# lmxyy/sige

Measured on AMD Instinct MI355X. Metric: DDPM-256 U-Net sparse (SIGE) forwards/s, higher is better.
Workload: dtype f32; 1 GPU; DDPM 256x256 church U-Net (ch128, mult 1-1-2-2-4-4, 113.7M params, random init), 1.2% square edit, one edited image per GPU, hipGraph replay, NHWC activations, in-place scatter ...; batch_per_gpu=1, resolution=256, parallelism=dp1

## Files before the change

### include/sige_hip.h

```cpp
#ifndef SIGE_HIP_H
#define SIGE_HIP_H

#include <stddef.h>
#include <stdint.h>

#ifdef __cplusplus
extern "C" {
#endif

#define SIGE_HIP_VERSION 310

enum {
    SIGE_HIP_OK = 0,
    SIGE_HIP_EINVAL = -1,
    SIGE_HIP_EUNSUPPORTED = -2,
    SIGE_HIP_ELAUNCH = -3,
    SIGE_HIP_ENODEVICE = -4
};

enum { SIGE_HIP_ACT_IDENTITY = 0, SIGE_HIP_ACT_SWISH = 1,
       SIGE_HIP_ACT_RELU = 2, SIGE_HIP_ACT_LEAKY = 3 , SIGE_HIP_ACT_TANH = 4 };

enum {
    SIGE_HIP_TUNE_CONV_TILE_MT = 0,
// ... 92 lines not shown

int sige_hip_change_tiles_i32(const int32_t *indices, const int32_t *count, int capacity, int bH, int bW,
                              int strideH, int strideW, int offsetH, int offsetW, int outH, int outW,
                              int Hp, int Wp, int tileH, int tileW, int padH, int padW, int depth,
                              int32_t *lists, int32_t *counts, void *stream);

size_t sige_hip_block_conv_packed_size(int Cout, int Cin, int kH, int kW, int R, int S,
                                       int strideH, int strideW, int groups);
int sige_hip_block_conv_pack_f32(const float *w, int Cout, int Cin, int kH, int kW,
                                 float *packed, void *stream);
int sige_hip_block_conv_f32(const float *x, int T, int Cin, int R, int S,
                            const float *packed, const float *bias, int Cout, int kH, int kW,
                            int strideH, int strideW, float *out, void *stream);
int sige_hip_block_conv_direct_f32(const float *x, int T, int Cin, int R, int S,
                                   const float *w, const float *bias, int Cout, int kH, int kW,
                                   int strideH, int strideW, int dilationH, int dilationW, int groups,
                                   float *out, void *stream);
int sige_hip_spade_modulate_nhwc_f32(
        const float *x_full, const float *x_tiles, const int32_t *map_x, int Nx, int Rx, int Sx,
        const float *scale, int scaleB, int scaleC, const float *shift, int shiftB, int shiftC,
        const float *gb_tiles, const float *gb_full, const int32_t *map_g, int Ng, int Rg, int Sg,
        int B, int C, int H, int W, int bH, int bW, const int32_t *active_indices, int N,
        int leaky, float slope, float *out, void *stream);

size_t sige_hip_block_conv_packed_size_f16c(int Cout, int Cin, int kH, int kW, int R, int S,
                                            int strideH, int strideW, int groups);
int sige_hip_block_conv_pack_f16c(const float *w, int Cout, int Cin, int kH, int kW,
                                  float *packed, void *stream);

int sige_hip_conv_pair_begin(void);
int sige_hip_conv_pair_end(void);
int64_t sige_hip_conv_pairs_fused(void);
int sige_hip_conv_side_begin(int max_side_workgroups_per_host);
int sige_hip_conv_side_flush(void);
int64_t sige_hip_conv_side_workgroups(int flushed);
int sige_hip_release_graph_tickets(void);

int sige_hip_gather_conv_f32(const float *x, int B, int Cin, int H, int W, int bH, int bW,
                             const int32_t *active_indices, int N,
                             const float *scale, int scaleB, int scaleC, int scaleH, int scaleW,
                             const float *shift, int shiftB, int shiftC, int shiftH, int shiftW,
                             int activation,
                             const float *packed, const float *bias, int Cout, int kH, int kW,
                             int strideH, int strideW, float *out, void *stream);
int sige_hip_scatter_gather_conv_f32(const float *x, const float *y, int B, int Cin, int H, int W,
                                     int Rx, int Sx, int bH, int bW,
                                     const int32_t *active_indices, int N, const int32_t *scatter_map,
                                     const float *scale, int scaleB, int scaleC, int scaleH, int scaleW,
                                     const float *shift, int shiftB, int shiftC, int shiftH, int shiftW,
                                     int activation,
                                     const float *packed, const float *bias, int Cout, int kH, int kW,
                                     int strideH, int strideW, float *out, void *stream);

int sige_hip_gather_conv_nchw_f32(const float *x, const float *x2, int B, int C1, int C2, int H, int W,
                                  int bH, int bW, const int32_t *active_indices, int N,
                                  const float *scale, int scaleB, int scaleC,
                                  const float *shift, int shiftB, int shiftC,
                                  int activation,
                                  const float *packed, const float *bias, int Cout, int kH, int kW,
                                  int strideH, int strideW, int offsetH, int offsetW,
                                  const float *residual, int Ho, int Wo, float *out, void *stream);

int sige_hip_block_conv_nhwc(int compute, const float *x, int T, int Cin, int R, int S,
                             const float *packed, const float *bias, int Cout, int kH, int kW,
                             int strideH, int strideW, float *out, void *stream);
int sige_hip_block_conv_nhwc_keyed(int compute, const float *x, const int32_t *count_key, int B, int N, int Cin, int R, int S,
                                   const float *packed, const float *bias, int Cout, int kH, int kW,
                                   int strideH, int strideW, float *out, void *stream);
int sige_hip_gather_conv_nhwc(int compute, const float *x, const float *x2, int B, int C1, int C2, int H, int W,
                              int bH, int bW, const int32_t *active_indices, int N,
                              const float *scale, int scaleB, int scaleC,
                              const float *shift, int shiftB, int shiftC,
                              int activation,
                              const float *packed, const float *bias, int Cout, int kH, int kW,
                              int strideH, int strideW,
                              int to_full, int offsetH, int offsetW, const float *residual, int Ho, int Wo,
                              float *workspace, size_t workspace_floats,
                              const float *out_scale, const float *out_shift, int out_activation,
                              int upsample2x,
                              float *twin0, const float *twin0_scale, const float *twin0_shift,
                              float *twin1, const float *twin1_scale, const float *twin1_shift,
                              const float *packed_tile3, int min_blocks,
                              float *out, void *stream);
int sige_hip_conv_ksplit_hint(int T, int Cin, int Cout, int kH, int kW, int strideH, int strideW);
int sige_hip_scatter_gather_conv_nhwc(int compute, const float *x, const void *y, int y_f16, int B, int Cin, int H, int W,
                                      int Rx, int Sx, int bH, int bW,
                                      const int32_t *active_indices, int N, const int32_t *scatter_map,
                                      const float *scale, int scaleB, int scaleC,
                                      const float *shift, int shiftB, int shiftC,
                                      int activation,
                                      const float *packed, const float *bias, int Cout, int kH, int kW,
                                      int strideH, int strideW, float *out, void *stream);

int sige_hip_scatter_gather_conv_scatter_nhwc(
        int compute, const float *x, const void *y, int y_f16, int B, int Cin, int H, int W, int Rx, int Sx, int bH, int bW,
        const int32_t *active_indices, int N, const int32_t *scatter_map,
        const float *scale, int scaleB, int scaleC, const float *shift, int shiftB, int shiftC, int activation,
        const float *packed, const float *bias, int Cout, int kH, int kW,
        int offsetH, int offsetW, const void *residual, int residual_f16,
        const float *x1, const int32_t *table1, int gH1, int gW1, int N1, int R1, int S1,
        float *twin0, const float *twin0_scale, const float *twin0_shift,
        float *twin1, const float *twin1_scale, const float *twin1_shift,
        const float *packed_tile3, int min_blocks,
        float *out, void *stream);

int sige_hip_gather_nhwc_f32(const float *x, int B, int C, int H, int W, int bH, int bW,
                             const int32_t *active_indices, int N,
                             const float *scale, int scaleB, int scaleC,
                             const float *shift, int shiftB, int shiftC,
                             int activation, float *out, void *stream);
int sige_hip_scatter_gather_nhwc_f32(const float *x, const float *y, int B, int C, int H, int W,
                                     int Rx, int Sx, int bH, int bW,
                                     const int32_t *active_indices, int N, const int32_t *scatter_map,
                                     const float *scale, int scaleB, int scaleC,
                                     const float *shift, int shiftB, int shiftC,
                                     int activation, float *out, void *stream);
int sige_hip_scatter_nhwc_f32(const float *x, const float *y, int B, int C, int H, int W, int R, int S,
                              int offsetH, int offsetW, int strideH, int strideW,
                              const int32_t *active_indices, const int32_t *table, int gH, int gW, int N,
                              const float *residual, int in_place, float *out, void *stream);
int sige_hip_scatter_with_block_residual_nhwc_f32(
        const float *x0, const float *y0, const float *x1, const float *y1,
        int B, int C, int H, int W, int R0, int S0, int R1, int S1,
        int offsetH, int offsetW, int strideH, int strideW,
        const int32_t *active_indices0, const int32_t *table0, int gH0, int gW0, int N0,
        const int32_t *active_indices1, const int32_t *table1, int gH1, int gW1, int N1,
        int in_place, float *out, void *stream);

enum { SIGE_HIP_RESAMPLE_DOWN = 0, SIGE_HIP_RESAMPLE_UP = 1 };
int sige_hip_resample_tiles_nhwc_f32(const float *x, int B, int C, int H, int W, int mode,
                                     const int32_t *active_indices, int N, int bH, int bW,
                                     const float *scale, const float *shift, float *tiles,
                                     int offsetH, int offsetW, int strideH, int strideW, int rH, int rW,
                                     float *res, void *stream);

int sige_hip_tile_conv3_supported(int C1, int C2, int Cout);
int sige_hip_tile_conv3_nhwc(
        int compute, int source, const float *x, const void *x2, int y_f16, int B, int C1, int C2, int H, int W, int upsample2x,
        const int32_t *active_indices, int N, const int32_t *scatter_map, int Rx, int Sx,
        const float *scale, const float *shift, int affineB, int activation,
        const float *packed, const float *bias, int Cout,
        int to_full, int offsetH, int offsetW, int Ho, int Wo, const void *residual, int residual_f16,
        const float *x1, const int32_t *table1, int gH1, int gW1, int N1, int R1, int S1,
        const float *out_scale, const float *out_shift, int out_activation,
        float *twin0, const float *twin_scale0, const float *twin_shift0,
        float *twin1, const float *twin_scale1, const float *twin_shift1,
        float *out, void *stream);

int sige_hip_add_layer_norm_tokens_f32(const float *x, const float *delta, const float *bias, const float *gamma,
                                       const float *beta, int64_t T, int C, float eps, float *sum_out, float *out, void *stream);
int sige_hip_geglu_tokens_f32(const float *x, int64_t T, int D, float *out, void *stream);
int sige_hip_add_bias_tokens_f32(const float *x, const float *delta, const float *bias, int64_t T, int C, float *out, void *stream);

size_t sige_hip_token_linear_packed_size(int N, int K, int geglu);
int sige_hip_token_linear_supported(int64_t M, int N, int K, int layer_norm, int geglu, int parts);
int sige_hip_token_linear_pack(const float *w, int N, int K, int geglu, float *packed, void *stream);
int sige_hip_token_linear_f32(const float *x, int64_t M, int K, const float *ln_gamma, const float *ln_beta, float ln_eps,
                              const float *packed, const float *bias, int N, int geglu, const float *residual, int parts,
                              float *out0, float *out1, float *out2, void *stream);

int sige_hip_conv3x3_small_cout_nhwc_f32(const float *x, int B, int C, int H, int W,
                                         const float *scale, int scaleB, int scaleC,
                                         const float *shift, int shiftB, int shiftC, int activation,
                                         const float *weight, const float *bias, int Cout,
                                         float *out, void *stream);

// ... 158 lines not shown
```

### sige_amd/build.py

```python
import os
import subprocess
import sys

PKG = os.path.dirname(os.path.abspath(__file__))
REPO = os.path.dirname(PKG)
CSRC = os.path.join(PKG, "csrc")
LIB_DIR = os.path.join(PKG, "lib")
LIB = os.path.join(LIB_DIR, "libsige_hip.so")
SOURCES = ["api.hip", "plan.hip", "gather.hip", "scatter.hip", "reduce_mask.hip", "mask_pipeline.hip", "block_conv.hip", "conv_k3s1.hip", "conv_k1.hip",
           "conv_k3s2.hip", "conv_k3s1_nhwc.hip", "conv_k1_nhwc.hip", "conv_k3s2_nhwc.hip", "conv_k3s1_nhwc_w8.hip", "conv_k1_nhwc_w8.hip", "conv_k3s1_nhwc_h.hip", "conv_k1_nhwc_h.hip", "conv_k3s1_nhwc_x.hip", "conv_k1_nhwc_x.hip", "conv_k3s1_nhwc_c16.hip", "conv_k3s1_nhwc_h_c16.hip", "conv_k3s1_nhwc_x_c16.hip", "conv_pair_nhwc_x_t4.hip", "conv_pair_nhwc_x_f4.hip",
           "conv_pair_nhwc_t4.hip", "conv_pair_nhwc_t8.hip", "conv_pair_nhwc_f4.hip", "conv_pair_nhwc_f8.hip", "conv_pair_nhwc_h_t4.hip", "conv_pair_nhwc_h_f4.hip", "conv_wide.hip", "conv_wide_k3_p8.hip", "conv_wide_k3_f32.hip", "conv_wide_k1_p8.hip", "conv_wide_pair_f32.hip", "conv_wide_pair_x3.hip", "conv_wide_pair_f16.hip", "group_norm.hip", "attention.hip", "attention_fused.hip", "attention_tokens.hip", "nhwc_ops.hip", "conv_out.hip", "conv_in.hip", "spade_ops.hip", "conv_tile3.hip", "conv_tile3_f32.hip", "token_ops.hip", "conv_tile3_f16.hip", "token_linear.hip", "resample_tiles.hip", "attention_wide.hip", "conv_side_nhwc_f4.hip", "conv_latent_head.hip", "spade_separable.hip"]
FLAGS = ["--offload-arch=gfx950", "-O3", "-std=c++17", "-fPIC", "-ffp-contract=off", "-Wno-unused-result"]


def source_hash() -> str:
    import hashlib

    h = hashlib.sha256(" ".join(FLAGS).encode())
    for f in sorted(os.listdir(CSRC)):
        if f.endswith((".hip", ".hpp", ".h")):
            h.update(f.encode())
            h.update(open(os.path.join(CSRC, f), "rb").read())
    h.update(open(os.path.join(REPO, "include", "sige_hip.h"), "rb").read())
    return h.hexdigest()[:16]


def _hipcc() -> str:
    for cand in (os.environ.get("HIPCC"), "/opt/rocm/bin/hipcc", "hipcc"):
        if cand and (os.path.isabs(cand) and os.path.isfile(cand) or not os.path.isabs(cand)):
            return cand
    return "hipcc"


def needs_build() -> bool:
    if not os.path.isfile(LIB):
        return True
    t = os.path.getmtime(LIB)
    deps = [os.path.join(CSRC, f) for f in os.listdir(CSRC)] + [os.path.join(REPO, "include", "sige_hip.h")]
    return any(os.path.getmtime(d) > t for d in deps)


def _stale(obj: str, src: str, headers) -> bool:
    if not os.path.isfile(obj):
        return True
    t = os.path.getmtime(obj)
    return any(os.path.getmtime(d) > t for d in [src, *headers])


TUNING_UNITS = ("api.hip", "block_conv.hip", "gather.hip", "conv_wide.hip", "attention_tokens.hip", "conv_out.hip", "conv_tile3.hip", "token_linear.hip")
TUNING_LIB = os.path.join(LIB_DIR, "libsige_hip_tuning.so")


def _compile_cmd(src: str, obj: str, defs=()):
    return [_hipcc(), *FLAGS, "-DSIGE_TU_ID=%d" % SOURCES.index(src), *defs, "-I" + os.path.join(REPO, "include"), "-I" + CSRC, "-c",
            os.path.join(CSRC, src), "-o", obj]


def _headers():
    headers = [os.path.join(CSRC, f) for f in os.listdir(CSRC) if f.endswith((".hpp", ".h"))]
    headers.append(os.path.join(REPO, "include", "sige_hip.h"))
    return headers


def _headers_of(src: str, headers):
    return (headers if src.startswith("conv_wide") else [h for h in headers if not h.endswith("conv_wide.hpp")] if src.startswith(("conv_k", "conv_pair", "conv_side", "conv_tile3", "block_conv", "token_linear"))
            else [h for h in headers if not h.endswith(("conv_mfma.hpp", "conv_wide.hpp", "conv_tile3.hpp"))])


def _run_all(procs):
    for cmd, p in procs:
        if p.wait() != 0:
            raise RuntimeError("hipcc failed: " + " ".join(cmd))


def build_tuning(force: bool = False, verbose: bool = True) -> str:
    build(force=force, verbose=verbose)
    if not force and os.path.isfile(TUNING_LIB):
        t = os.path.getmtime(TUNING_LIB)
        deps = [os.path.join(CSRC, f) for f in os.listdir(CSRC)] + [os.path.join(REPO, "include", "sige_hip.h"), LIB]
        if all(os.path.getmtime(d) <= t for d in deps):
            return TUNING_LIB
    tdir = os.path.join(LIB_DIR, "tuning")
    os.makedirs(tdir, exist_ok=True)
    headers = _headers()
    objs, procs = [], []
    for src in SOURCES:
        if src in TUNING_UNITS:
            obj = os.path.join(tdir, src.replace(".hip", ".o"))
            if force or _stale(obj, os.path.join(CSRC, src), _headers_of(src, headers)):
                cmd = _compile_cmd(src, obj, ["-DSIGE_HIP_TUNING"])
                if verbose:
                    print(" ".join(cmd), flush=True)
                procs.append((cmd, subprocess.Popen(cmd)))
        else:
# ... 71 lines not shown
```

### sige_amd/csrc/block_conv.hip

```cpp
#include <deque>
#include <mutex>

#include "conv_mfma.hpp"
#include "conv_tile3.hpp"

namespace sige {

template <int KK, int MT>
__global__ void pack_weights_kernel(const float *__restrict__ w, int Cout, int Cin, float *__restrict__ packed,
                                    long total) {
    constexpr int NL = 64 / MT, CW = (KK == 1 ? 16 : 4) * NL, CC = 4 * CW, L = (CW / NL) * KK, F = L / 4;
    const int nchunks = ((Cin + CC - 1) / CC + 1) & ~1;
    for (long i = (long)blockIdx.x * blockDim.x + threadIdx.x; i < total; i += (long)gridDim.x * blockDim.x) {
        long r = i;
        const int e = r % 4; r /= 4;
        const int j = r % MT; r /= MT;
        const int kq = r % NL; r /= NL;
        const int f = r % F; r /= F;
        const int wave = r % 4; r /= 4;
        const int chunk = r % nchunks; r /= nchunks;
        const int ng = (int)r;
        const int u = 4 * f + e, q = u / KK, tap = u % KK;
        const int ci = chunk * CC + wave * CW + NL * q + kq;
        const int co = MT * ng + j;
// ... 93 lines not shown
        const int g = co / cog;
        float acc = bias ? bias[co] : 0.0f;
        for (int ci = 0; ci < cig; ++ci) {
            const float *xp = x + (((size_t)t * Cin + g * cig + ci) * R + oy * strH) * S + ox * strW;
            const float *wq = w + ((size_t)co * cig + ci) * kH * kW;
            for (int ky = 0; ky < kH; ++ky)
                for (int kx = 0; kx < kW; ++kx) acc = fmaf(xp[ky * dilH * S + kx * dilW], wq[ky * kW + kx], acc);
        }
        out[i] = acc;
    }
}

static int mfma_kind(int kH, int kW, int R, int S, int strH, int strW, int groups) {
    if (groups != 1 || kH != kW || R != S || strH != strW) return 0;
    if (kH == 3 && strH == 1 && R == 6) return 1;
    if (kH == 1 && strH == 1 && R == 4) return 2;
    if (kH == 3 && strH == 2 && R == 5) return 3;
    return 0;
}

#define SIGE_CONV_DECLARE(G, NB, LAY, W)                                                                 \
    template <> void launch_conv_geo<G, NB, SRC_TILES, DST_TILES, LAY, W>(ConvArgs, int, hipStream_t);          \
    template <> void launch_conv_geo<G, NB, SRC_GATHER, DST_TILES, LAY, W>(ConvArgs, int, hipStream_t);         \
    template <> void launch_conv_geo<G, NB, SRC_GATHER, DST_NCHW, LAY, W>(ConvArgs, int, hipStream_t);          \
    template <> void launch_conv_geo<G, NB, SRC_SCATTER_GATHER, DST_TILES, LAY, W>(ConvArgs, int, hipStream_t);
#define SIGE_CONV_DECLARE_LAYOUTS(G, NB) SIGE_CONV_DECLARE(G, NB, LAYOUT_NCHW, 4) SIGE_CONV_DECLARE(G, NB, LAYOUT_NHWC, 4)
using K31_16 = ConvGeo<3, 1, 6, 16>;
using K31_32 = ConvGeo<3, 1, 6, 32>;
using K11_16 = ConvGeo<1, 1, 4, 16>;
using K11_32 = ConvGeo<1, 1, 4, 32>;
using K32_16 = ConvGeo<3, 2, 5, 16>;
using K32_32 = ConvGeo<3, 2, 5, 32>;
SIGE_CONV_DECLARE_LAYOUTS(K31_16, 1)
SIGE_CONV_DECLARE_LAYOUTS(K31_16, 2)
SIGE_CONV_DECLARE_LAYOUTS(K31_32, 1)
SIGE_CONV_DECLARE_LAYOUTS(K31_32, 2)
SIGE_CONV_DECLARE_LAYOUTS(K11_16, 1)
SIGE_CONV_DECLARE_LAYOUTS(K11_16, 2)
SIGE_CONV_DECLARE_LAYOUTS(K11_32, 1)
SIGE_CONV_DECLARE_LAYOUTS(K11_32, 2)
SIGE_CONV_DECLARE_LAYOUTS(K32_16, 1)
SIGE_CONV_DECLARE_LAYOUTS(K32_32, 1)
#define SIGE_CONV_DECLARE_SG_FULL(G, NB, W) \
    template <> void launch_conv_geo<G, NB, SRC_SCATTER_GATHER, DST_NCHW, LAYOUT_NHWC, W>(ConvArgs, int, hipStream_t);
SIGE_CONV_DECLARE_SG_FULL(K31_16, 1, 4) SIGE_CONV_DECLARE_SG_FULL(K31_16, 2, 4)
SIGE_CONV_DECLARE_SG_FULL(K31_32, 1, 4) SIGE_CONV_DECLARE_SG_FULL(K31_32, 2, 4)
SIGE_CONV_DECLARE_SG_FULL(K31_16, 1, 8) SIGE_CONV_DECLARE_SG_FULL(K31_16, 2, 8)
SIGE_CONV_DECLARE_SG_FULL(K31_32, 1, 8) SIGE_CONV_DECLARE_SG_FULL(K31_32, 2, 8)
SIGE_CONV_DECLARE(K31_16, 1, LAYOUT_NHWC, 8)
SIGE_CONV_DECLARE(K31_16, 2, LAYOUT_NHWC, 8)
SIGE_CONV_DECLARE(K31_32, 1, LAYOUT_NHWC, 8)
SIGE_CONV_DECLARE(K31_32, 2, LAYOUT_NHWC, 8)
SIGE_CONV_DECLARE(K11_16, 1, LAYOUT_NHWC, 8)
SIGE_CONV_DECLARE(K11_16, 2, LAYOUT_NHWC, 8)
SIGE_CONV_DECLARE(K11_32, 1, LAYOUT_NHWC, 8)
SIGE_CONV_DECLARE(K11_32, 2, LAYOUT_NHWC, 8)

using H31_16 = ConvGeoH<3, 1, 6, 16>;
using H31_32 = ConvGeoH<3, 1, 6, 32>;
using H11_16 = ConvGeoH<1, 1, 4, 16>;
using H11_32 = ConvGeoH<1, 1, 4, 32>;
SIGE_CONV_DECLARE(H31_16, 1, LAYOUT_NHWC, 4) SIGE_CONV_DECLARE(H31_16, 2, LAYOUT_NHWC, 4)
SIGE_CONV_DECLARE(H31_32, 1, LAYOUT_NHWC, 4) SIGE_CONV_DECLARE(H31_32, 2, LAYOUT_NHWC, 4)
SIGE_CONV_DECLARE(H11_16, 1, LAYOUT_NHWC, 4) SIGE_CONV_DECLARE(H11_16, 2, LAYOUT_NHWC, 4)
SIGE_CONV_DECLARE(H11_32, 1, LAYOUT_NHWC, 4) SIGE_CONV_DECLARE(H11_32, 2, LAYOUT_NHWC, 4)
SIGE_CONV_DECLARE_SG_FULL(H31_16, 1, 4) SIGE_CONV_DECLARE_SG_FULL(H31_16, 2, 4)
SIGE_CONV_DECLARE_SG_FULL(H31_32, 1, 4) SIGE_CONV_DECLARE_SG_FULL(H31_32, 2, 4)

using X31_16 = ConvGeoX<3, 1, 6, 16>;
using X31_32 = ConvGeoX<3, 1, 6, 32>;
using X11_16 = ConvGeoX<1, 1, 4, 16>;
using X11_32 = ConvGeoX<1, 1, 4, 32>;
SIGE_CONV_DECLARE(X31_16, 1, LAYOUT_NHWC, 4) SIGE_CONV_DECLARE(X31_32, 1, LAYOUT_NHWC, 4)
SIGE_CONV_DECLARE(X11_16, 1, LAYOUT_NHWC, 4) SIGE_CONV_DECLARE(X11_32, 1, LAYOUT_NHWC, 4)
SIGE_CONV_DECLARE_SG_FULL(X31_16, 1, 4) SIGE_CONV_DECLARE_SG_FULL(X31_32, 1, 4)

#define SIGE_CONV_DECLARE_C16(G, NB)                                                        \
    template <> void launch_conv_c16<G, NB, DST_TILES>(ConvArgs, int, hipStream_t);         \
    template <> void launch_conv_c16<G, NB, DST_NCHW>(ConvArgs, int, hipStream_t);
SIGE_CONV_DECLARE_C16(K31_16, 1) SIGE_CONV_DECLARE_C16(K31_16, 2) SIGE_CONV_DECLARE_C16(K31_32, 1) SIGE_CONV_DECLARE_C16(K31_32, 2)
SIGE_CONV_DECLARE_C16(H31_16, 1) SIGE_CONV_DECLARE_C16(H31_16, 2) SIGE_CONV_DECLARE_C16(H31_32, 1) SIGE_CONV_DECLARE_C16(H31_32, 2)
SIGE_CONV_DECLARE_C16(X31_16, 1) SIGE_CONV_DECLARE_C16(X31_32, 1)

__global__ __launch_bounds__(256) void splitk_reduce_nhwc_kernel(const float *__restrict__ ws, int S, size_t stride, size_t n4, int C,
                                                                const float *__restrict__ bias, const float *__restrict__ residual,
                                                                const float *__restrict__ oscale, const float *__restrict__ oshift, int oact,
                                                                float *__restrict__ out) {
    for (size_t i = (size_t)blockIdx.x * 256 + threadIdx.x; i < n4; i += (size_t)gridDim.x * 256) {
        const float4 zero = make_float4(0.f, 0.f, 0.f, 0.f);
        const int c = (int)((4 * i) % C);
        float4 b = zero, r = zero, os = zero, oh = zero;
        if (bias) b = *reinterpret_cast<const float4 *>(bias + c);
        if (residual) r = *reinterpret_cast<const float4 *>(residual + 4 * i);
        if (oscale) {
            os = *reinterpret_cast<const float4 *>(oscale + c);
            oh = *reinterpret_cast<const float4 *>(oshift + c);
        }
        float4 p[8];
#pragma unroll
        for (int s = 0; s < 8; ++s) p[s] = *reinterpret_cast<const float4 *>(ws + (size_t)(s < S ? s : S - 1) * stride + 4 * i);
        float4 v = p[0];
#pragma unroll
        for (int s = 1; s < 8; ++s)
            if (s < S) { v.x += p[s].x; v.y += p[s].y; v.z += p[s].z; v.w += p[s].w; }
        if (bias) { v.x += b.x; v.y += b.y; v.z += b.z; v.w += b.w; }
        if (residual) { v.x += r.x; v.y += r.y; v.z += r.z; v.w += r.w; }
        if (oscale) {
            v.x = os.x * v.x; v.y = os.y * v.y; v.z = os.z * v.z; v.w = os.w * v.w;
            v.x = oh.x + v.x; v.y = oh.y + v.y; v.z = oh.z + v.z; v.w = oh.w + v.w;
            if (oact == SIGE_HIP_ACT_SWISH) { v.x = swish(v.x); v.y = swish(v.y); v.z = swish(v.z); v.w = swish(v.w); }
        }
        *reinterpret_cast<float4 *>(out + 4 * i) = v;
    }
}

static int ksplit_for(long blocks, int nchunks, int cap) {
    const int force = tuning(SIGE_HIP_TUNE_CONV_KSPLIT);
    if (cap <= 1 || (blocks >= 224 && !force)) return 1;
    int s = force ? force : (int)((224 + blocks - 1) / blocks);
    s = s < nchunks / 2 ? s : nchunks / 2;
    s = s < 8 ? s : 8;
    s = s < cap ? s : cap;
    return s < 1 ? 1 : s;
}

__device__ int32_t g_zero_idx[2] = {0, 0};

#ifdef SIGE_CONV_PROBE
static unsigned long long *g_probe_buf = nullptr;
static unsigned long long *conv_probe_buffer() {
    if (!g_probe_buf && hipMalloc(&g_probe_buf, 8 * 4096 * sizeof(unsigned long long)) != hipSuccess) g_probe_buf = nullptr;
    return g_probe_buf;
}
extern "C" int sige_hip_conv_probe_read(unsigned long long *host, int workgroups) {
    if (!g_probe_buf || workgroups > 4096) return SIGE_HIP_EINVAL;
    return hipMemcpy(host, g_probe_buf, (size_t)workgroups * 8 * sizeof(unsigned long long), hipMemcpyDeviceToHost) == hipSuccess
               ? SIGE_HIP_OK : SIGE_HIP_ELAUNCH;
}
extern "C" int sige_hip_conv_probe_clear(void) {
    if (!conv_probe_buffer()) return SIGE_HIP_ELAUNCH;
    return hipMemset(g_probe_buf, 0, 8 * 4096 * sizeof(unsigned long long)) == hipSuccess ? SIGE_HIP_OK : SIGE_HIP_ELAUNCH;
}
#endif

struct HeldConv {
    bool active = false;
    ConvArgs a;
    int mode = 0, dst = 0, prec = 0;
    hipStream_t st = nullptr;
    int (*launch)(ConvArgs, int, hipStream_t) = nullptr;
};
static thread_local HeldConv g_held;
static thread_local bool g_pairing = false;
static std::atomic<long> g_pairs_fused{0};

static int flush_held() {
    if (!g_held.active) return SIGE_HIP_OK;
    const HeldConv h = g_held;
    g_held.active = false;
    const bool p = g_pairing;
    g_pairing = false;
    const int rc = h.launch(h.a, h.mode, h.st);
    note_launches(1);
    g_pairing = p;
    return rc;
}
// ... 305 lines not shown
            if (rc1 != SIGE_HIP_OK) {
                const int rc = flush_held();
                return rc != SIGE_HIP_OK ? rc : SIGE_HIP_EUNSUPPORTED;
            }
        }
    }
    if (a.ksplit > 1) {
        a.out = a.ws;
        a.fout = final_out;
    }
    const int mt = p.mt, nb = p.nb, waves = p.waves;
    bool done = false;
    if constexpr (kPairFirst) {
        if (may_pair) {
            done = launch_pair<DST, PREC>(a, p, mode, g_held.a, st);
            if (done) g_held.active = false;
            else {
                const int rc = flush_held();
                if (rc != SIGE_HIP_OK) return rc;
            }
        }
    }
    if constexpr (kSideGeo) {
        if (!done && !g_side.empty() && mt == 16 && nb == 1 && waves == 4 && a.ksplit == 1 && (mode == MODE_RAW || mode == MODE_AFFINE_SWISH)) {
            SideConv &sc = g_side.front();
            const int na = conv_grid_x(a);
            int take = sc.total - sc.next;
            take = take < sc.budget ? take : sc.budget;
            take = take < kSideChipWorkgroups - na ? take : kSideChipWorkgroups - na;
            if (take > 0) {
                if (sc.nb == 2) launch_conv_side<K31_16, 1, K31_16, 2, DST_NCHW, 4>(a, sc.a, mode, na, sc.next, take, st);
                else launch_conv_side<K31_16, 1, K31_16, 1, DST_NCHW, 4>(a, sc.a, mode, na, sc.next, take, st);
                sc.next += take;
                g_side_hosted.fetch_add(take, std::memory_order_relaxed);
                if (sc.next >= sc.total) g_side.pop_front();
                done = true;
            }
        }
    }
    if constexpr (SRC == SRC_SCATTER_GATHER && LAY == LAYOUT_NHWC && KH == 3 && STR == 1) {
        if (!done && a.y_f16) {
            if (waves != 4) return SIGE_HIP_EUNSUPPORTED;
            if constexpr (kHasNB2) {
                if (mt == 32 && nb == 2) { launch_conv_c16<G32, 2, DST>(a, mode, st); done = true; }
                else if (nb == 2) { launch_conv_c16<G16, 2, DST>(a, mode, st); done = true; }
            }
            if (!done) {
                if (mt == 32) launch_conv_c16<G32, 1, DST>(a, mode, st);
                else launch_conv_c16<G16, 1, DST>(a, mode, st);
                done = true;
            }
        }
    } else {
        if (a.y_f16) return SIGE_HIP_EUNSUPPORTED;
    }
    constexpr bool kHasW8 = LAY == LAYOUT_NHWC && STR == 1 && PREC == 0;
    if constexpr (kHasW8) {
        if (!done && waves == 8) {
            if (mt == 32 && nb == 2) launch_conv_geo<G32, 2, SRC, DST, LAY, 8>(a, mode, st);
            else if (mt == 32) launch_conv_geo<G32, 1, SRC, DST, LAY, 8>(a, mode, st);
            else if (nb == 2) launch_conv_geo<G16, 2, SRC, DST, LAY, 8>(a, mode, st);
            else launch_conv_geo<G16, 1, SRC, DST, LAY, 8>(a, mode, st);
            done = true;
        }
    }
    if constexpr (kHasNB2) {
        if (!done && mt == 32 && nb == 2) { launch_conv_geo<G32, 2, SRC, DST, LAY, 4>(a, mode, st); done = true; }
        else if (!done && nb == 2) { launch_conv_geo<G16, 2, SRC, DST, LAY, 4>(a, mode, st); done = true; }
    }
    if (!done) {
        if (mt == 32) launch_conv_geo<G32, 1, SRC, DST, LAY, 4>(a, mode, st);
        else launch_conv_geo<G16, 1, SRC, DST, LAY, 4>(a, mode, st);
    }
    if (a.ksplit > 1 && !a.counters) {
        const size_t n4 = a.split_stride / 4;
        const int grid = (int)((n4 + 255) / 256 < 2048 ? (n4 + 255) / 256 : 2048);
        splitk_reduce_nhwc_kernel<<<grid, 256, 0, st>>>(a.ws, a.ksplit, a.split_stride, n4, a.Cout, a.bias, a.residual,
                                                       a.oscale, a.oshift, a.oact, final_out);
        note_launches(1);
    }
    return SIGE_HIP_OK;
}

template <int SRC, int DST = DST_TILES, int LAY = LAYOUT_NCHW, int PREC = 0>
static int launch_conv(const ConvArgs &a, int mode, int kH, int kW, int R, int S, int strH, int strW, hipStream_t st) {
    int rc;
    switch (mfma_kind(kH, kW, R, S, strH, strW, 1)) {
        case 1: rc = launch_kind<3, 1, 6, SRC, DST, LAY, PREC>(a, mode, st); break;
        case 2: rc = launch_kind<1, 1, 4, SRC, DST, LAY, PREC>(a, mode, st); break;
        case 3:
            if constexpr (PREC != 0) return SIGE_HIP_EUNSUPPORTED;
            else rc = launch_kind<3, 2, 5, SRC, DST, LAY, PREC>(a, mode, st);
            break;
        default: return SIGE_HIP_EUNSUPPORTED;
    }
    return rc != SIGE_HIP_OK ? rc : launch_status();
}

static int staging_mode(const float *scale, int sB, int sC, const float *shift, int tB, int tC, int activation,
                        int B, int C, int *aff_sb, int *aff_sc) {
    *aff_sb = *aff_sc = 0;
    if (!scale && !shift) return activation == SIGE_HIP_ACT_IDENTITY ? MODE_RAW : -1;
    if (!scale || !shift || sB != tB || sC != tC) return -1;
    if (!((sB == 1 || sB == B) && (sC == 1 || sC == C))) return -1;
    *aff_sb = sB > 1 ? sC : 0;
    *aff_sc = sC > 1 ? 1 : 0;
    return activation == SIGE_HIP_ACT_SWISH ? MODE_AFFINE_SWISH : MODE_AFFINE;
}

}

using namespace sige;

extern "C" int sige_hip_conv_pair_begin(void) {
    SIGE_PLAN_HOOK0(sige_hip_conv_pair_begin);
    const int rc = flush_held();
    g_pairing = true;
    return rc;
}

extern "C" int sige_hip_conv_pair_end(void) {
    SIGE_PLAN_HOOK0(sige_hip_conv_pair_end);
    g_pairing = false;
    g_side_armed = 0;
    const int rc = flush_held();
    if (rc != SIGE_HIP_OK) (void)flush_side();
    return rc != SIGE_HIP_OK ? rc : launch_status(0);
}

extern "C" int64_t sige_hip_conv_pairs_fused(void) { return (int64_t)g_pairs_fused.load(std::memory_order_relaxed); }

extern "C" int sige_hip_conv_side_begin(int max_side_workgroups_per_host) {
    SIGE_PLAN_HOOK_NOSTREAM(sige_hip_conv_side_begin, max_side_workgroups_per_host);
    if (max_side_workgroups_per_host <= 0) return SIGE_HIP_EINVAL;
    g_side_armed = max_side_workgroups_per_host;
    return SIGE_HIP_OK;
}

extern "C" int sige_hip_conv_side_flush(void) {
    SIGE_PLAN_HOOK0(sige_hip_conv_side_flush);
    g_side_armed = 0;
    return flush_side();
}

extern "C" int64_t sige_hip_conv_side_workgroups(int flushed) {
    return (int64_t)(flushed ? g_side_flushed : g_side_hosted).load(std::memory_order_relaxed);
}

extern "C" size_t sige_hip_block_conv_packed_size(int Cout, int Cin, int kH, int kW, int R, int S,
                                                  int strideH, int strideW, int groups) {
    if (Cout <= 0 || Cin <= 0) return 0;
    if (!mfma_kind(kH, kW, R, S, strideH, strideW, groups)) return 0;
    return packed_floats(Cout, Cin, kH * kW, 32) + packed_floats(Cout, Cin, kH * kW, 16);
}

extern "C" int sige_hip_block_conv_pack_f32(const float *w, int Cout, int Cin, int kH, int kW,
                                            float *packed, void *stream) {
    if (!w || !packed || Cout <= 0 || Cin <= 0) return SIGE_HIP_EINVAL;
    if (kH != kW || (kH != 1 && kH != 3)) return SIGE_HIP_EUNSUPPORTED;
    const int KK = kH * kW;
    hipStream_t st = as_stream(stream);
    const long n32 = (long)packed_floats(Cout, Cin, KK, 32), n16 = (long)packed_floats(Cout, Cin, KK, 16);
    auto blocks = [](long n) { return (int)((n + 255) / 256 < 4096 ? (n + 255) / 256 : 4096); };
    if (KK == 9) {
        pack_weights_kernel<9, 32><<<blocks(n32), 256, 0, st>>>(w, Cout, Cin, packed, n32);
        pack_weights_kernel<9, 16><<<blocks(n16), 256, 0, st>>>(w, Cout, Cin, packed + n32, n16);
    } else {
        pack_weights_kernel<1, 32><<<blocks(n32), 256, 0, st>>>(w, Cout, Cin, packed, n32);
        pack_weights_kernel<1, 16><<<blocks(n16), 256, 0, st>>>(w, Cout, Cin, packed + n32, n16);
    }
    return launch_status(2);
}

extern "C" size_t sige_hip_block_conv_packed_size_f16c(int Cout, int Cin, int kH, int kW, int R, int S,
                                                       int strideH, int strideW, int groups) {
    if (Cout <= 0 || Cin <= 0) return 0;
    const int kind = mfma_kind(kH, kW, R, S, strideH, strideW, groups);
    if (kind != 1 && kind != 2) return 0;
    return packed_units_h(Cout, Cin, kH * kW, 32) + packed_units_h(Cout, Cin, kH * kW, 16);
}

extern "C" int sige_hip_block_conv_pack_f16c(const float *w, int Cout, int Cin, int kH, int kW,
                                             float *packed, void *stream) {
    if (!w || !packed || Cout <= 0 || Cin <= 0) return SIGE_HIP_EINVAL;
    if (kH != kW || (kH != 1 && kH != 3)) return SIGE_HIP_EUNSUPPORTED;
    const int KK = kH * kW;
    hipStream_t st = as_stream(stream);
    const long n32 = 2 * (long)packed_units_h(Cout, Cin, KK, 32), n16 = 2 * (long)packed_units_h(Cout, Cin, KK, 16);
    auto blocks = [](long n) { return (int)((n + 255) / 256 < 4096 ? (n + 255) / 256 : 4096); };
    _Float16 *ph = reinterpret_cast<_Float16 *>(packed);
    if (KK == 9) {
        pack_weights_h_kernel<9, 32><<<blocks(n32), 256, 0, st>>>(w, Cout, Cin, ph, n32);
        pack_weights_h_kernel<9, 16><<<blocks(n16), 256, 0, st>>>(w, Cout, Cin, ph + n32, n16);
    } else {
        pack_weights_h_kernel<1, 32><<<blocks(n32), 256, 0, st>>>(w, Cout, Cin, ph, n32);
        pack_weights_h_kernel<1, 16><<<blocks(n16), 256, 0, st>>>(w, Cout, Cin, ph + n32, n16);
    }
    return launch_status(2);
}

extern "C" size_t sige_hip_block_conv_packed_size_f16x3(int Cout, int Cin, int kH, int kW, int R, int S,
                                                        int strideH, int strideW, int groups) {
    if (Cout <= 0 || Cin <= 0) return 0;
    const int kind = mfma_kind(kH, kW, R, S, strideH, strideW, groups);
    if (kind != 1 && kind != 2) return 0;
    return packed_units_x(Cout, Cin, kH * kW, 32) + packed_units_x(Cout, Cin, kH * kW, 16) + kX3Header;
}

extern "C" int sige_hip_block_conv_pack_f16x3(const float *w, int Cout, int Cin, int kH, int kW,
                                              float *packed, void *stream) {
    if (!w || !packed || Cout <= 0 || Cin <= 0) return SIGE_HIP_EINVAL;
    if (kH != kW || (kH != 1 && kH != 3)) return SIGE_HIP_EUNSUPPORTED;
    const int KK = kH * kW;
    hipStream_t st = as_stream(stream);
    const size_t u32 = packed_units_x(Cout, Cin, KK, 32), u16 = packed_units_x(Cout, Cin, KK, 16);
    const long n32 = 2 * (long)u32, n16 = 2 * (long)u16;
    float *header = packed + u32 + u16;
    if (hipMemsetAsync(header, 0, kX3Header * sizeof(float), st) != hipSuccess) return SIGE_HIP_ELAUNCH;
    const long nw = (long)Cout * Cin * KK;
    wmax_bits_kernel<<<(int)((nw + 255) / 256 < 1024 ? (nw + 255) / 256 : 1024), 256, 0, st>>>(w, nw, reinterpret_cast<unsigned *>(header));
    auto blocks = [](long n) { return (int)((n + 255) / 256 < 4096 ? (n + 255) / 256 : 4096); };
    _Float16 *ph = reinterpret_cast<_Float16 *>(packed);
    if (KK == 9) {
        pack_weights_x_kernel<9, 32><<<blocks(n32), 256, 0, st>>>(w, Cout, Cin, ph, n32, header);
        pack_weights_x_kernel<9, 16><<<blocks(n16), 256, 0, st>>>(w, Cout, Cin, ph + n32, n16, header);
    } else {
        pack_weights_x_kernel<1, 32><<<blocks(n32), 256, 0, st>>>(w, Cout, Cin, ph, n32, header);
        pack_weights_x_kernel<1, 16><<<blocks(n16), 256, 0, st>>>(w, Cout, Cin, ph + n32, n16, header);
    }
    return launch_status(3);
}

extern "C" int sige_hip_block_conv_f32(const float *x, int T, int Cin, int R, int S,
                                       const float *packed, const float *bias, int Cout, int kH, int kW,
                                       int strideH, int strideW, float *out, void *stream) {
    SIGE_PLAN_HOOK_FIXED(sige_hip_block_conv_f32, x, T, Cin, R, S, packed, bias, Cout, kH, kW, strideH, strideW, out, stream);
    if (T < 0 || Cin <= 0 || Cout <= 0) return SIGE_HIP_EINVAL;
    if (T == 0) return SIGE_HIP_OK;
    if (!x || !packed || !out) return SIGE_HIP_EINVAL;
    if (reinterpret_cast<uintptr_t>(out) & 15 || reinterpret_cast<uintptr_t>(packed) & 15) return SIGE_HIP_EINVAL;
    if ((long)T * Cin * R * S >= (1L << 29)) return SIGE_HIP_EUNSUPPORTED;
    ConvArgs a{};
    a.x = x; a.packed = packed; a.bias = bias; a.out = out;
    a.T = T; a.Cin = Cin; a.Cout = Cout;
    if (reinterpret_cast<uintptr_t>(x) & 15 || ((long)Cin * R * S) % 4) {
        void *zero_idx = nullptr;
        if (hipGetSymbolAddress(&zero_idx, HIP_SYMBOL(g_zero_idx)) != hipSuccess) return SIGE_HIP_ELAUNCH;
        a.x2 = x; a.Csplit = Cin; a.idx = static_cast<const int32_t *>(zero_idx);
        a.B = T; a.N = 1; a.H = R; a.W = S;
        return launch_conv<SRC_GATHER>(a, MODE_RAW, kH, kW, R, S, strideH, strideW, as_stream(stream));
    }
    return launch_conv<SRC_TILES>(a, 0, kH, kW, R, S, strideH, strideW, as_stream(stream));
}

// ... 77 lines not shown
        !channel_affine(shift, shiftB, shiftC, shiftH, shiftW, B, Cin))
        return SIGE_HIP_EUNSUPPORTED;
    if ((long)B * Cin * H * W >= (1L << 29) || (long)B * N * Cin * Rx * Sx >= (1L << 29)) return SIGE_HIP_EUNSUPPORTED;
    if ((long)B * N == 0) return SIGE_HIP_OK;
    if (!x || !y || !packed || !out || !active_indices || !scatter_map) return SIGE_HIP_EINVAL;
    if (reinterpret_cast<uintptr_t>(out) & 15 || reinterpret_cast<uintptr_t>(packed) & 15) return SIGE_HIP_EINVAL;
    ConvArgs a{};
    a.x = x; a.y = y; a.idx = active_indices; a.map = scatter_map; a.packed = packed; a.bias = bias; a.out = out;
    a.T = B * N; a.Cin = Cin; a.Cout = Cout; a.B = B; a.N = N; a.H = H; a.W = W;
    if (stacked_shift(H) != 0) return SIGE_HIP_EUNSUPPORTED;
    a.RxSx = Rx * Sx; a.Sx = Sx;
    a.scale = scale; a.shift = shift;
    const int mode = staging_mode(scale, scaleB, scaleC, shift, shiftB, shiftC, activation, B, Cin, &a.aff_sb, &a.aff_sc);
    if (mode < 0) return SIGE_HIP_EUNSUPPORTED;
    return launch_conv<SRC_SCATTER_GATHER>(a, mode, kH, kW, bH, bW, strideH, strideW, as_stream(stream));
}

static bool nhwc_ok(int Cin, int C1, int Cout, const void *p0, const void *p1, const void *p2, const void *p3) {
    auto al = [](const void *p) { return (reinterpret_cast<uintptr_t>(p) & 15) == 0; };
    return Cin % 4 == 0 && C1 % 4 == 0 && Cout % 4 == 0 && al(p0) && al(p1) && al(p2) && al(p3);
}

extern "C" int sige_hip_conv_ksplit_hint(int T, int Cin, int Cout, int kH, int kW, int strideH, int strideW) {
    if (T <= 0 || Cin <= 0 || Cout <= 0) return 1;
    const int px = (kH == 3 && strideH == 2) ? 4 : 16;
    const long blocks16 = (long)ceil_div(T, 16 / px) * ceil_div(Cout, 16);
    if (blocks16 >= 224 && !tuning(SIGE_HIP_TUNE_CONV_KSPLIT)) return 1;
    return 8;
}

#define SIGE_BY_COMPUTE(compute, impl, ...)         \
    ((compute) == 0   ? impl<0>(__VA_ARGS__)        \
     : (compute) == 1 ? impl<1>(__VA_ARGS__)        \
     : (compute) == 2 ? impl<2>(__VA_ARGS__)        \
                      : SIGE_HIP_EINVAL)

template <int PREC>
static int block_conv_nhwc_impl(const float *x, int T, int Cin, int R, int S,
                                const float *packed, const float *bias, int Cout, int kH, int kW,
                                int strideH, int strideW, float *out, void *stream) {
    if (T < 0 || Cin <= 0 || Cout <= 0) return SIGE_HIP_EINVAL;
    if (T == 0) return SIGE_HIP_OK;
    if (!x || !packed || !out) return SIGE_HIP_EINVAL;
    if (!nhwc_ok(Cin, Cin, Cout, x, packed, out, bias)) return SIGE_HIP_EUNSUPPORTED;
    if ((long)T * Cin * R * S >= (1L << 29)) return SIGE_HIP_EUNSUPPORTED;
    ConvArgs a{};
    a.x = x; a.packed = packed; a.bias = bias; a.out = out;
    a.T = T; a.Cin = Cin; a.Cout = Cout;
    return launch_conv<SRC_TILES, DST_TILES, LAYOUT_NHWC, PREC>(a, 0, kH, kW, R, S, strideH, strideW, as_stream(stream));
}

extern "C" int sige_hip_block_conv_nhwc(int compute, const float *x, int T, int Cin, int R, int S,
                                        const float *packed, const float *bias, int Cout, int kH, int kW,
                                        int strideH, int strideW, float *out, void *stream) {
    SIGE_PLAN_HOOK_FIXED(sige_hip_block_conv_nhwc, compute, x, T, Cin, R, S, packed, bias, Cout, kH, kW, strideH, strideW, out, stream);
    return SIGE_BY_COMPUTE(compute, block_conv_nhwc_impl, x, T, Cin, R, S, packed, bias, Cout, kH, kW, strideH, strideW, out, stream);
}

extern "C" int sige_hip_block_conv_nhwc_keyed(int compute, const float *x, const int32_t *count_key, int B, int N, int Cin, int R, int S,
                                              const float *packed, const float *bias, int Cout, int kH, int kW,
                                              int strideH, int strideW, float *out, void *stream) {
    SIGE_PLAN_HOOK_N(sige_hip_block_conv_nhwc_keyed, (sige::CountOf<2, 4>), compute, x, count_key, B, N, Cin, R, S, packed, bias, Cout, kH, kW, strideH, strideW, out, stream);
    if (B < 0 || N < 0 || !count_key || (long)B * N > 0x7fffffffL) return SIGE_HIP_EINVAL;
    const int T = B * N;
    return SIGE_BY_COMPUTE(compute, block_conv_nhwc_impl, x, T, Cin, R, S, packed, bias, Cout, kH, kW, strideH, strideW, out, stream);
}

template <int PREC>
static int gather_conv_nhwc_impl(const float *x, const float *x2, int B, int C1, int C2, int H, int W,
                                             int bH, int bW, const int32_t *active_indices, int N,
                                             const float *scale, int scaleB, int scaleC,
                                             const float *shift, int shiftB, int shiftC,
                                             int activation,
                                             const float *packed, const float *bias, int Cout, int kH, int kW,
                                             int strideH, int strideW,
                                             int to_full, int offsetH, int offsetW, const float *residual, int Ho, int Wo,
                                             float *workspace, size_t workspace_floats,
                                             const float *out_scale, const float *out_shift, int out_activation,
                                             int upsample2x,
                                             float *twin0, const float *twin0_scale, const float *twin0_shift,
                                             float *twin1, const float *twin1_scale, const float *twin1_shift,
                                             float *out, void *stream) {
    const int Cin = C1 + C2;
    if (upsample2x && ((H | W) & 1)) return SIGE_HIP_EINVAL;
    if (B < 0 || C1 <= 0 || C2 < 0 || Cout <= 0 || H <= 0 || W <= 0 || N < 0) return SIGE_HIP_EINVAL;
    if (to_full && (Ho <= 0 || Wo <= 0)) return SIGE_HIP_EINVAL;
    if (activation != SIGE_HIP_ACT_IDENTITY && activation != SIGE_HIP_ACT_SWISH) return SIGE_HIP_EUNSUPPORTED;
    if ((long)B * Cin * H * W >= (1L << 29)) return SIGE_HIP_EUNSUPPORTED;
    if ((long)B * N == 0) return SIGE_HIP_OK;
    if (!x || (C2 && !x2) || !packed || !out || !active_indices) return SIGE_HIP_EINVAL;
    if (C2 && B != 1) return SIGE_HIP_EUNSUPPORTED;
    if (!nhwc_ok(Cin, C1, Cout, x, C2 ? x2 : x, out, bias) || (reinterpret_cast<uintptr_t>(packed) & 15) ||
        (reinterpret_cast<uintptr_t>(residual) & 15))
        return SIGE_HIP_EUNSUPPORTED;
    ConvArgs a{};
    a.x = x; a.x2 = C2 ? x2 : x; a.Csplit = C1; a.idx = active_indices; a.packed = packed; a.bias = bias; a.out = out;
    a.T = B * N; a.Cin = Cin; a.Cout = Cout; a.B = B; a.N = N; a.H = H; a.W = W;
    a.hp_shift = stacked_shift(H);
    if (a.hp_shift < 0 || (a.hp_shift && B != 1)) return SIGE_HIP_EUNSUPPORTED;
    a.scale = scale; a.shift = shift;
    const int mode = staging_mode(scale, scaleB, scaleC, shift, shiftB, shiftC, activation, B, Cin, &a.aff_sb, &a.aff_sc);
    if (mode < 0) return SIGE_HIP_EUNSUPPORTED;
    if ((out_scale == nullptr) != (out_shift == nullptr)) return SIGE_HIP_EINVAL;
    if (out_activation != SIGE_HIP_ACT_IDENTITY && out_activation != SIGE_HIP_ACT_SWISH) return SIGE_HIP_EUNSUPPORTED;
    if ((reinterpret_cast<uintptr_t>(out_scale) | reinterpret_cast<uintptr_t>(out_shift)) & 15) return SIGE_HIP_EUNSUPPORTED;
    a.oscale = out_scale; a.oshift = out_shift; a.oact = out_activation;
    a.up = upsample2x ? 1 : 0;
    {
        const int Ro = (bH - kH) / strideH + 1, So = (bW - kW) / strideW + 1;
        a.split_stride = to_full ? (size_t)B * Ho * Wo * Cout : (size_t)B * N * Ro * So * Cout;
        a.ws = workspace;
        a.ksplit_max = (workspace && a.split_stride && !(reinterpret_cast<uintptr_t>(workspace) & 15))
                           ? (int)(workspace_floats / a.split_stride < 8 ? workspace_floats / a.split_stride : 8) : 1;
        if (to_full && (long)N * Ro * So < (long)Ho * Wo) a.ksplit_max = 1;
    }
    if ((twin0 || twin1) && !to_full) return SIGE_HIP_EINVAL;
    if ((twin0 && (!twin0_scale || !twin0_shift)) || (twin1 && (!twin1_scale || !twin1_shift))) return SIGE_HIP_EINVAL;
    if ((reinterpret_cast<uintptr_t>(twin0) | reinterpret_cast<uintptr_t>(twin1) | reinterpret_cast<uintptr_t>(twin0_scale) |
         reinterpret_cast<uintptr_t>(twin0_shift) | reinterpret_cast<uintptr_t>(twin1_scale) | reinterpret_cast<uintptr_t>(twin1_shift)) & 15)
        return SIGE_HIP_EUNSUPPORTED;
    a.twin0 = twin0; a.tscale0 = twin0_scale; a.tshift0 = twin0_shift;
    a.twin1 = twin1; a.tscale1 = twin1_scale; a.tshift1 = twin1_shift;
    if (to_full) {
        a.residual = residual; a.Ho = Ho; a.Wo = Wo; a.offH = offsetH; a.offW = offsetW; a.strH = strideH; a.strW = strideW;
        return launch_conv<SRC_GATHER, DST_NCHW, LAYOUT_NHWC, PREC>(a, mode, kH, kW, bH, bW, strideH, strideW, as_stream(stream));
    }
    return launch_conv<SRC_GATHER, DST_TILES, LAYOUT_NHWC, PREC>(a, mode, kH, kW, bH, bW, strideH, strideW, as_stream(stream));
}

constexpr int kTile3F16PairMin = 256;

constexpr int kTile3F16SparseMin = 128;

static bool tile3_takes(const float *packed_tile3, int min_blocks, int B, int N, int C1, int C2, int Cout, int kH, int kW, int bH, int bW,
                        int strideH, int strideW, hipStream_t st, bool f16 = false, int H = 0, int W = 0) {
    if (!packed_tile3 || min_blocks <= 0) return false;
    if (kH != 3 || kW != 3 || bH != 6 || bW != 6 || strideH != 1 || strideW != 1) return false;
    if (!sige_hip_tile_conv3_supported(C1, C2, Cout)) return false;
    const long blocks = (long)((B * (long)N + 1) / 2) * (Cout / 64);
    int need = min_blocks;
    if (f16 && H > 0 && (long)N * 16 < (long)H * W) {
        int sm = tuning(SIGE_HIP_TUNE_TILE3_F16_SPARSE_MIN);
        if (sm < 0) sm = kTile3F16SparseMin;
        if (sm > 0 && sm < need) need = sm;
    }
    if (blocks < need) return false;
    if (g_held.active && g_held.st == st) {
        if (!f16) return false;
        int pm = tuning(SIGE_HIP_TUNE_TILE3_F16_PAIR_MIN);
        if (pm < 0) pm = kTile3F16PairMin;
        if (pm == 0 || blocks < pm) return false;
    }
    return true;
}

extern "C" int sige_hip_gather_conv_nhwc(int compute, const float *x, const float *x2, int B, int C1, int C2, int H, int W,
                                         int bH, int bW, const int32_t *active_indices, int N,
                                         const float *scale, int scaleB, int scaleC,
                                         const float *shift, int shiftB, int shiftC,
                                         int activation,
                                         const float *packed, const float *bias, int Cout, int kH, int kW,
                                         int strideH, int strideW,
                                         int to_full, int offsetH, int offsetW, const float *residual, int Ho, int Wo,
                                         float *workspace, size_t workspace_floats,
                                         const float *out_scale, const float *out_shift, int out_activation,
                                         int upsample2x,
                                         float *twin0, const float *twin0_scale, const float *twin0_shift,
                                         float *twin1, const float *twin1_scale, const float *twin1_shift,
                                         const float *packed_tile3, int min_blocks,
                                         float *out, void *stream) {
    SIGE_PLAN_HOOK_N(sige_hip_gather_conv_nhwc, (sige::CountOf<10, 11>), compute, x, x2, B, C1, C2, H, W, bH, bW, active_indices, N, scale, scaleB, scaleC, shift, shiftB, shiftC, activation, packed, bias, Cout, kH, kW, strideH, strideW, to_full, offsetH, offsetW, residual, Ho, Wo, workspace, workspace_floats, out_scale, out_shift, out_activation, upsample2x, twin0, twin0_scale, twin0_shift, twin1, twin1_scale, twin1_shift, packed_tile3, min_blocks, out, stream);
    const int Cin = C1 + C2;
    const bool f16 = compute == 1;
    const bool aff_ok = (!scale && !shift) || (scale && shift && scaleC == Cin && shiftC == Cin && scaleB == shiftB && (scaleB == 1 || scaleB == B));
    if ((compute == 0 || f16) && B > 0 && N > 0 && aff_ok && !(g_side_armed > 0 && compute == 0 && to_full) &&
        tile3_takes(packed_tile3, min_blocks, B, N, C1, C2, Cout, kH, kW, bH, bW, strideH, strideW, as_stream(stream), f16, f16 ? H : 0, f16 ? W : 0)) {
        const int rc = tile_conv3_launch(T3_GATHER, x, x2, B, C1, C2, H, W, upsample2x, active_indices, N, nullptr, 0, 0, scale, shift,
                                         scale ? scaleB : 0, activation, packed_tile3, bias, Cout, to_full, offsetH, offsetW, Ho, Wo,
                                         to_full ? residual : nullptr, nullptr, nullptr, 0, 0, 0, 0, 0, out_scale, out_shift, out_activation,
                                         twin0, twin0_scale, twin0_shift, twin1, twin1_scale, twin1_shift, out, stream, f16 ? WIDE_F16 : WIDE_F32, 0, 0);
        if (rc != SIGE_HIP_EUNSUPPORTED) { g_side_armed = 0; return rc; }
    }
    const int rc = SIGE_BY_COMPUTE(compute, gather_conv_nhwc_impl, x, x2, B, C1, C2, H, W, bH, bW, active_indices, N, scale, scaleB, scaleC, shift, shiftB,
                                   shiftC, activation, packed, bias, Cout, kH, kW, strideH, strideW, to_full, offsetH, offsetW, residual, Ho, Wo,
                                   workspace, workspace_floats, out_scale, out_shift, out_activation, upsample2x, twin0, twin0_scale, twin0_shift,
                                   twin1, twin1_scale, twin1_shift, out, stream);
    g_side_armed = 0;
    return rc;
}

template <int PREC>
static int scatter_gather_conv_nhwc_impl(const float *x, const void *y, int y_f16, int B, int Cin, int H, int W,
                                                     int Rx, int Sx, int bH, int bW,
                                                     const int32_t *active_indices, int N, const int32_t *scatter_map,
                                                     const float *scale, int scaleB, int scaleC,
                                                     const float *shift, int shiftB, int shiftC,
                                                     int activation,
                                                     const float *packed, const float *bias, int Cout, int kH, int kW,
                                                     int strideH, int strideW, float *out, void *stream) {
    if (B < 0 || Cin <= 0 || Cout <= 0 || H <= 0 || W <= 0 || N < 0 || Rx <= 0 || Sx <= 0) return SIGE_HIP_EINVAL;
    if (activation != SIGE_HIP_ACT_IDENTITY && activation != SIGE_HIP_ACT_SWISH) return SIGE_HIP_EUNSUPPORTED;
    if ((long)B * Cin * H * W >= (1L << 29) || (long)B * N * Cin * Rx * Sx >= (1L << 29)) return SIGE_HIP_EUNSUPPORTED;
    if ((long)B * N == 0) return SIGE_HIP_OK;
    if (!x || !y || !packed || !out || !active_indices || !scatter_map) return SIGE_HIP_EINVAL;
    if (!nhwc_ok(Cin, Cin, Cout, x, y, out, bias) || (reinterpret_cast<uintptr_t>(packed) & 15)) return SIGE_HIP_EUNSUPPORTED;
    if (y_f16 && (kH != 3 || kW != 3 || strideH != 1 || strideW != 1)) return SIGE_HIP_EUNSUPPORTED;
    ConvArgs a{};
    a.y_f16 = y_f16 ? 1 : 0;
    a.x = x; a.y = static_cast<const float *>(y); a.idx = active_indices; a.map = scatter_map; a.packed = packed; a.bias = bias; a.out = out;
    a.T = B * N; a.Cin = Cin; a.Cout = Cout; a.B = B; a.N = N; a.H = H; a.W = W;
    a.hp_shift = stacked_shift(H);
    if (a.hp_shift < 0 || (a.hp_shift && B != 1)) return SIGE_HIP_EUNSUPPORTED;
    a.RxSx = Rx * Sx; a.Sx = Sx;
    a.scale = scale; a.shift = shift;
    const int mode = staging_mode(scale, scaleB, scaleC, shift, shiftB, shiftC, activation, B, Cin, &a.aff_sb, &a.aff_sc);
    if (mode < 0) return SIGE_HIP_EUNSUPPORTED;
    return launch_conv<SRC_SCATTER_GATHER, DST_TILES, LAYOUT_NHWC, PREC>(a, mode, kH, kW, bH, bW, strideH, strideW, as_stream(stream));
}

extern "C" int sige_hip_scatter_gather_conv_nhwc(int compute, const float *x, const void *y, int y_f16, int B, int Cin, int H, int W,
                                                 int Rx, int Sx, int bH, int bW,
                                                 const int32_t *active_indices, int N, const int32_t *scatter_map,
                                                 const float *scale, int scaleB, int scaleC,
                                                 const float *shift, int shiftB, int shiftC,
                                                 int activation,
                                                 const float *packed, const float *bias, int Cout, int kH, int kW,
                                                 int strideH, int strideW, float *out, void *stream) {
    SIGE_PLAN_HOOK_N(sige_hip_scatter_gather_conv_nhwc, (sige::CountOf<12, 13>), compute, x, y, y_f16, B, Cin, H, W, Rx, Sx, bH, bW, active_indices, N, scatter_map, scale, scaleB, scaleC, shift, shiftB, shiftC, activation, packed, bias, Cout, kH, kW, strideH, strideW, out, stream);
    return SIGE_BY_COMPUTE(compute, scatter_gather_conv_nhwc_impl, x, y, y_f16, B, Cin, H, W, Rx, Sx, bH, bW, active_indices, N, scatter_map, scale, scaleB,
                           scaleC, shift, shiftB, shiftC, activation, packed, bias, Cout, kH, kW, strideH, strideW, out, stream);
}

template <int PREC>
static int scatter_gather_conv_scatter_nhwc_impl(
        const float *x, const void *y, int y_f16, int B, int Cin, int H, int W, int Rx, int Sx, int bH, int bW,
        const int32_t *active_indices, int N, const int32_t *scatter_map,
        const float *scale, int scaleB, int scaleC, const float *shift, int shiftB, int shiftC, int activation,
        const float *packed, const float *bias, int Cout, int kH, int kW,
        int offsetH, int offsetW, const void *residual, int residual_f16,
        const float *x1, const int32_t *table1, int gH1, int gW1, int N1, int R1, int S1,
        float *twin0, const float *twin0_scale, const float *twin0_shift,
        float *twin1, const float *twin1_scale, const float *twin1_shift,
        float *out, void *stream) {
    if (B < 0 || Cin <= 0 || Cout <= 0 || H <= 0 || W <= 0 || N < 0 || Rx <= 0 || Sx <= 0) return SIGE_HIP_EINVAL;
    if (kH != 3 || kW != 3 || bH != 6 || bW != 6) return SIGE_HIP_EUNSUPPORTED;
    if (activation != SIGE_HIP_ACT_IDENTITY && activation != SIGE_HIP_ACT_SWISH) return SIGE_HIP_EUNSUPPORTED;
    if ((long)B * Cin * H * W >= (1L << 29) || (long)B * N * Cin * Rx * Sx >= (1L << 29)) return SIGE_HIP_EUNSUPPORTED;
    if ((long)B * N == 0) return SIGE_HIP_OK;
    if (!x || !y || !packed || !out || !active_indices || !scatter_map) return SIGE_HIP_EINVAL;
    if (x1 && (!residual || !table1 || R1 <= 0 || S1 <= 0 || gH1 < (H + R1 - 1) / R1 || gW1 < (W + S1 - 1) / S1)) return SIGE_HIP_EINVAL;
    if (!nhwc_ok(Cin, Cin, Cout, x, y, out, bias) || (reinterpret_cast<uintptr_t>(packed) & 15) ||
        (reinterpret_cast<uintptr_t>(residual) & 15) || (reinterpret_cast<uintptr_t>(x1) & 15))
        return SIGE_HIP_EUNSUPPORTED;
    if (residual_f16 && !residual) return SIGE_HIP_EINVAL;
    ConvArgs a{};
    a.y_f16 = y_f16 ? 1 : 0; a.res_f16 = residual_f16 ? 1 : 0;
    a.x = x; a.y = static_cast<const float *>(y); a.idx = active_indices; a.map = scatter_map; a.packed = packed; a.bias = bias; a.out = out;
    a.T = B * N; a.Cin = Cin; a.Cout = Cout; a.B = B; a.N = N; a.H = H; a.W = W;
// ... 71 lines not shown
```

### sige_amd/csrc/conv_mfma.hpp

```cpp
#pragma once
#include <type_traits>

#include "common.hpp"

namespace sige {

typedef float f32x16 __attribute__((ext_vector_type(16)));
typedef float f32x4 __attribute__((ext_vector_type(4)));
typedef _Float16 f16x8 __attribute__((ext_vector_type(8)));
typedef _Float16 f16x4 __attribute__((ext_vector_type(4)));

enum { SRC_TILES = 0, SRC_GATHER = 1, SRC_SCATTER_GATHER = 2 };
enum { DST_TILES = 0, DST_NCHW = 1 };

template <int MT_> struct Mfma;
template <> struct Mfma<32> {
    using acc_t = f32x16;
    static constexpr int REGS = 16;
    __device__ static __forceinline__ acc_t op(float a, float b, acc_t c) {
        return __builtin_amdgcn_mfma_f32_32x32x2f32(a, b, c, 0, 0, 0);
    }
};
template <> struct Mfma<16> {
    using acc_t = f32x4;
// ... 35 lines not shown
    static constexpr int F = L / 4;
    static constexpr int TILE_FLOATS = CC * RS;
    static constexpr int BUF = TPB * TILE_FLOATS;
    static constexpr int RED = MT_ + 4;
    static_assert(L % 4 == 0, "wave slice must be a whole number of float4 weight loads");
    static_assert(MT_ % PX == 0 && TPB >= 1, "tile pixels must divide the M block");
};

template <int KH, int STR, int R_, int MT_>
struct ConvGeoH {
    static constexpr bool F16 = true, X3 = false;
    static constexpr int K = KH, S = STR, R = R_, MT = MT_;
    static constexpr int KK = KH * KH;
    static constexpr int RS = R_ * R_;
    static constexpr int RO = (R_ - KH) / STR + 1;
    static constexpr int PX = RO * RO;
    static constexpr int NL = 64 / MT_;
    static constexpr int KP = 8;
    static constexpr int SLAB = NL * KP;
    static constexpr int NSLAB = KK == 1 ? 2 : 1;
    static constexpr int TPB = MT_ / PX;
    static constexpr int CW = NSLAB * SLAB;
    static constexpr int CC = 4 * CW;
    static constexpr int L = NSLAB * KK;
    static constexpr int F = L;
    static constexpr int TILE_FLOATS = CC * RS;
    static constexpr int BUF = TPB * TILE_FLOATS;
    static constexpr int RED = MT_ + 4;
    static_assert(MT_ % PX == 0 && TPB >= 1, "tile pixels must divide the M block");
};

template <int KH, int STR, int R_, int MT_>
struct ConvGeoX : ConvGeoH<KH, STR, R_, MT_> {
    static constexpr bool X3 = true;
    static constexpr int F = 2 * ConvGeoH<KH, STR, R_, MT_>::L;
};

__host__ __device__ constexpr int cmax(int a, int b) { return a > b ? a : b; }

template <int I, int N, typename F>
__device__ __forceinline__ void static_for(F &&f) {
    if constexpr (I < N) {
        f(std::integral_constant<int, I>{});
        static_for<I + 1, N>(f);
    }
}

struct ConvArgs {
    const float *x;
    const float *y;
    const int32_t *idx;
    const int32_t *map;
    const float *packed;
    const float *bias;
    float *out;
    int T, Cin, Cout, nchunks;
    int nblk;
    int B, N, H, W;
    int RxSx, Sx;
    const float *scale, *shift;
    int aff_sb, aff_sc;
    const float *x2;
    int Csplit;
    const float *residual;
    int Ho, Wo, offH, offW, strH, strW;
    int mbk, ngk, ng_fast;
    int ksplit, chunks_per_split;
    size_t split_stride;
    const float *oscale, *oshift;
    int oact;
    const float *x1;
    const int32_t *table1;
    int gW1, N1, R1, S1;
    int up;
    float *ws;
    int ksplit_max;
    int32_t *counters;
    float *fout;
    float *twin0, *twin1;
    const float *tscale0, *tshift0, *tscale1, *tshift1;
    const float *wscale_ptr;
    int y_f16, res_f16;
    int hp_shift;
#ifdef SIGE_CONV_PROBE
    unsigned long long *probe;
#endif
};

#ifdef SIGE_CONV_PROBE
#define SIGE_PROBE(k)                                                                                       \
    do {                                                                                                    \
        if (a.probe && threadIdx.x == 0 && blockIdx.y == 0 && blockIdx.x < 4096)                            \
            a.probe[blockIdx.x * 8 + (k)] = __builtin_amdgcn_s_memtime();                                   \
    } while (0)
#else
#define SIGE_PROBE(k)
#endif
#if defined(SIGE_CONV_PROBE) && defined(SIGE_ABL)
#define SIGE_ABL_HAS(bit) (((SIGE_ABL) & (bit)) != 0)
#else
#define SIGE_ABL_HAS(bit) false
#endif

__device__ __forceinline__ float swish_fast(float z) {
    const float e = __builtin_amdgcn_exp2f(z * -1.44269504088896341f);
    return z * __builtin_amdgcn_rcpf(1.0f + e);
}

enum { MODE_RAW = 0, MODE_AFFINE_SWISH = 1, MODE_AFFINE = 2 };

using rsrc_t = __amdgpu_buffer_rsrc_t;
constexpr unsigned kOOB = 0x80000000u;

__device__ __forceinline__ rsrc_t make_rsrc(const float *base, long elem_off, long total_elems) {
    const int off = __builtin_amdgcn_readfirstlane((int)elem_off);
    int bytes = __builtin_amdgcn_readfirstlane((int)((total_elems - elem_off) * 4));
    bytes = bytes < 0 ? 0 : bytes;
    return __builtin_amdgcn_make_buffer_rsrc(const_cast<float *>(base) + off, 0, bytes, 0x00020000);
}
__device__ __forceinline__ float buf_f32(rsrc_t r, unsigned byte_off) {
    return __builtin_bit_cast(float, __builtin_amdgcn_raw_buffer_load_b32(r, (int)byte_off, 0, 0));
}
__device__ __forceinline__ float4 buf_f32x4(rsrc_t r, unsigned byte_off, int soff) {
    const f32x4 v = __builtin_bit_cast(f32x4, __builtin_amdgcn_raw_buffer_load_b128(r, (int)byte_off, soff, 0));
    return make_float4(v[0], v[1], v[2], v[3]);
}

__device__ __forceinline__ rsrc_t make_rsrc_h(const float *base_as_halves, long elem_off, long total_elems) {
    const int off = __builtin_amdgcn_readfirstlane((int)elem_off);
    int bytes = __builtin_amdgcn_readfirstlane((int)((total_elems - elem_off) * 2));
    bytes = bytes < 0 ? 0 : bytes;
    return __builtin_amdgcn_make_buffer_rsrc(reinterpret_cast<_Float16 *>(const_cast<float *>(base_as_halves)) + off, 0, bytes, 0x00020000);
}
typedef unsigned u32x2 __attribute__((ext_vector_type(2)));
__device__ __forceinline__ float4 buf_h4(rsrc_t r, unsigned byte_off, int soff) {
    const f16x4 h = __builtin_bit_cast(f16x4, __builtin_amdgcn_raw_buffer_load_b64(r, (int)byte_off, soff, 0));
    return make_float4((float)h[0], (float)h[1], (float)h[2], (float)h[3]);
}
__device__ __forceinline__ float4 ld_f32x4_or_h4(const float *base, size_t elem, bool halves) {
    if (halves) {
        const f16x4 h = *reinterpret_cast<const f16x4 *>(reinterpret_cast<const _Float16 *>(base) + elem);
        return make_float4((float)h[0], (float)h[1], (float)h[2], (float)h[3]);
    }
    return *reinterpret_cast<const float4 *>(base + elem);
}

__device__ __forceinline__ float4 ld_raw_f32x4_or_h4(const float *base, size_t elem, bool halves) {
    if (halves) {
        const float2 h = *reinterpret_cast<const float2 *>(reinterpret_cast<const _Float16 *>(base) + elem);
        return make_float4(h.x, h.y, 0.f, 0.f);
    }
    return *reinterpret_cast<const float4 *>(base + elem);
}
__device__ __forceinline__ float4 cvt_raw_f32x4_or_h4(float4 raw, bool halves) {
    if (halves) {
        const float2 r2 = make_float2(raw.x, raw.y);
        const f16x4 h = __builtin_bit_cast(f16x4, r2);
        return make_float4((float)h[0], (float)h[1], (float)h[2], (float)h[3]);
    }
    return raw;
}

enum { LAYOUT_NCHW = 0, LAYOUT_NHWC = 1 };

__device__ __forceinline__ void coherent_store(float *p, float4 v) {
    unsigned long long *q = reinterpret_cast<unsigned long long *>(p);
    const unsigned long long lo = (unsigned long long)__builtin_bit_cast(unsigned, v.x) | ((unsigned long long)__builtin_bit_cast(unsigned, v.y) << 32);
    const unsigned long long hi = (unsigned long long)__builtin_bit_cast(unsigned, v.z) | ((unsigned long long)__builtin_bit_cast(unsigned, v.w) << 32);
    __hip_atomic_store(q, lo, __ATOMIC_RELAXED, __HIP_MEMORY_SCOPE_AGENT);
    __hip_atomic_store(q + 1, hi, __ATOMIC_RELAXED, __HIP_MEMORY_SCOPE_AGENT);
}
__device__ __forceinline__ float4 coherent_load(const float *p) {
    unsigned long long *q = reinterpret_cast<unsigned long long *>(const_cast<float *>(p));
    const unsigned long long lo = __hip_atomic_load(q, __ATOMIC_RELAXED, __HIP_MEMORY_SCOPE_AGENT);
    const unsigned long long hi = __hip_atomic_load(q + 1, __ATOMIC_RELAXED, __HIP_MEMORY_SCOPE_AGENT);
    return make_float4(__builtin_bit_cast(float, (unsigned)lo), __builtin_bit_cast(float, (unsigned)(lo >> 32)),
                       __builtin_bit_cast(float, (unsigned)hi), __builtin_bit_cast(float, (unsigned)(hi >> 32)));
}

template <typename G, int NB, int MODE, int LAYOUT, int W>
__host__ __device__ constexpr int conv_lds_floats() {
    constexpr int CCk = W * G::CW;
    constexpr bool NHWC = LAYOUT == LAYOUT_NHWC;
    constexpr int LDC = G::F16 ? (G::X3 ? 2 * CCk + 8 : CCk + 8) : CCk + 4;
    constexpr int STAGE = NHWC ? (G::F16 ? G::TPB * G::RS * LDC / 2 : G::TPB * G::RS * LDC) : G::TPB * CCk * G::RS;
    constexpr int TABF = MODE != MODE_RAW ? 2 * (CCk + 4) : 0;
    return cmax(2 * STAGE + 2 * TABF, W * NB * G::MT * (G::MT + 4));
}

template <typename G, int NB, int SRC, int MODE, int DST, int LAYOUT, int W, bool Y16 = false>
__device__ __forceinline__ void conv_mfma_body(const ConvArgs &a, const int bx, const int by, float *const smem) {
    static_assert(!Y16 || (SRC == SRC_SCATTER_GATHER && LAYOUT == LAYOUT_NHWC), "fp16-stored cache: the channels-last scatter_gather source");
    constexpr unsigned YB = Y16 ? 2u : 4u;
    constexpr bool F16 = G::F16;
    using M = std::conditional_t<F16, MfmaH<G::MT>, Mfma<G::MT>>;
    static_assert(!F16 || LAYOUT == LAYOUT_NHWC, "the f16-compute kernels are channels-last");
    constexpr int NT = 64 * W;
    constexpr int CCk = W * G::CW;
    constexpr int TILEF = CCk * G::RS;
    constexpr int BUFk = G::TPB * TILEF;
    constexpr bool NHWC = LAYOUT == LAYOUT_NHWC;
    constexpr bool VEC = NHWC || SRC == SRC_TILES;
#ifndef SIGE_CONV_NACC32
#define SIGE_CONV_NACC32 1
#endif
    constexpr int NACC = NB == 1 ? ((G::MT == 16 || F16) ? 2 : SIGE_CONV_NACC32) : 1;
    constexpr bool AFF = MODE != MODE_RAW;
    constexpr bool X3 = G::X3;
    constexpr int LDC = F16 ? (X3 ? 2 * CCk + 8 : CCk + 8) : CCk + 4;
    constexpr int STAGE = NHWC ? (F16 ? G::TPB * G::RS * LDC / 2 : G::TPB * G::RS * LDC) : BUFk;
    constexpr int TROW = CCk + 4;
    constexpr int TABF = AFF ? 2 * TROW : 0;
    constexpr int RP = G::MT + 4;
    constexpr int LDS_FLOATS = cmax(2 * STAGE + 2 * TABF, W * NB * G::MT * RP);
    static_assert(LDS_FLOATS == conv_lds_floats<G, NB, MODE, LAYOUT, W>(), "conv_lds_floats() out of step with the body");
    float *const tab = smem + 2 * STAGE;

    SIGE_PROBE(0);
    const int tid = threadIdx.x;
    const int wave = __builtin_amdgcn_readfirstlane(tid >> 6);
    const int lane = tid & 63;
    const int kq = lane / G::MT, j = lane % G::MT;
    int mb, ng;
    if (a.ng_fast == 1) { ng = bx % a.ngk; mb = bx / a.ngk; }
    else if (a.ng_fast == 2) {
        const int jj = bx >> 3;
        mb = (bx & 7) + 8 * (jj / a.ngk);
        ng = jj % a.ngk;
        if (mb >= a.mbk) return;
    } else { mb = bx % a.mbk; ng = bx / a.mbk; }
    SIGE_PROBE(6);
    const int Cin = a.Cin;
    const int HW = (SRC == SRC_GATHER) ? (a.H >> a.up) * (a.W >> a.up) : a.H * a.W;
    const int split = by;
    const int first = split * a.chunks_per_split;
    const int last = min(a.nchunks, first + a.chunks_per_split) - 1;

    const int ngtot = (a.Cout + G::MT - 1) / G::MT;
    const long packed_floats_total = (long)ngtot * a.nblk * G::F * 64 * 4;
    int gsel[NB];
#pragma unroll
    for (int nb = 0; nb < NB; ++nb) gsel[nb] = min(ng * NB + nb, ngtot - 1);
    rsrc_t r_b[NB];
    auto set_b_chunk = [&](int chunk) {
#pragma unroll
        for (int nb = 0; nb < NB; ++nb)
            r_b[nb] = make_rsrc(a.packed, ((long)gsel[nb] * a.nblk + chunk * W + wave) * G::F * 64 * 4, packed_floats_total);
    };
    float4 bset[2][NB][G::F];
    auto b_load = [&](float4 &dst, int nb, int f) { dst = buf_f32x4(r_b[nb], lane * 16, f * 1024); };

    auto b_prologue = [&]() {
        set_b_chunk(first);
#pragma unroll
        for (int nb = 0; nb < NB; ++nb)
#pragma unroll
            for (int f = 0; f < G::F; ++f) b_load(bset[0][nb][f], nb, f);
        set_b_chunk(min(first + 1, last));
#pragma unroll
        for (int nb = 0; nb < NB; ++nb)
#pragma unroll
            for (int f = 0; f < G::F; ++f) b_load(bset[1][nb][f], nb, f);
    };
    if (!NHWC) b_prologue();

    constexpr int UNITS = VEC ? (NHWC ? G::TPB * G::RS * CCk / 4 : BUFk / 4) : BUFk;
    constexpr int NS = (UNITS + NT - 1) / NT;
    constexpr bool TWO = SRC == SRC_SCATTER_GATHER || (NHWC && SRC == SRC_GATHER);
    float st_z[2][VEC ? 1 : NS], st_z2[2][(!VEC && TWO) ? NS : 1];
    float4 st_q[2][VEC ? NS : 1], st_q2[2][(VEC && SRC == SRC_SCATTER_GATHER) ? NS : 1];
    unsigned s_off[NS], s_off2[TWO ? NS : 1];
    int s_tab[AFF ? NS : 1];
    int s_dst[NS];
    int s_cl[VEC ? NS : 1];

    const int trow = tid % CCk;
    const int tab_b0 = AFF ? ((mb * G::TPB) / a.N) * a.aff_sb : 0;
    auto tab_fetch = [&](int chunk, float &sc, float &sh) {
        const int c = chunk * CCk + trow;
        const int cc = c < Cin ? c : 0;
        const float vs = a.scale[tab_b0 + cc * a.aff_sc], vh = a.shift[tab_b0 + cc * a.aff_sc];
        sc = c < Cin ? vs : 0.f;
        sh = c < Cin ? vh : 0.f;
    };
    float t_sc = 0.f, t_sh = 0.f, t_sc1 = 0.f, t_sh1 = 0.f;

    constexpr int UNITS_NB = G::MT * G::MT / 4;
    constexpr int OUT_UNITS = NB * UNITS_NB;
    constexpr int EU = (OUT_UNITS + NT - 1) / NT;
    constexpr bool EPRE = NHWC && DST != DST_TILES && (W == 4 || NB == 1);
    int e_h[EPRE ? EU : 1], e_w[EPRE ? EU : 1];
    size_t e_q[EPRE ? EU : 1];
    bool e_in[EPRE ? EU : 1];
    float4 e_res[EPRE ? EU : 1];
    constexpr bool EPV = NHWC && (W == 4 || NB == 1);
    float4 e_bias[EPV ? EU : 1], e_os[EPV ? EU : 1], e_oh[EPV ? EU : 1];
    const bool e_first_pass = a.ksplit <= 1 || a.counters != nullptr;
    float wsc = 1.0f;
    if constexpr (X3) wsc = *a.wscale_ptr;

    auto epre_setup = [&]() {
        if constexpr (EPRE)
            static_for<0, EU>([&](auto k_tag) {
                constexpr int k = decltype(k_tag)::value;
                const int o = tid + k * NT;
                const int nb = o / UNITS_NB, o1 = o - nb * UNITS_NB;
                const int n4 = o1 % (G::MT / 4), m = o1 / (G::MT / 4);
                const int pxo = m % G::PX;
                const int t = mb * G::TPB + m / G::PX, co = (ng * NB + nb) * G::MT + 4 * n4;
                const int b = min(t, a.T - 1) / a.N;
                const int h = (a.offH + e_h[k]) / a.strH + pxo / G::RO, w = (a.offW + e_w[k]) / a.strW + pxo % G::RO;
                const bool in = o < OUT_UNITS && t < a.T && co < a.Cout && h >= 0 && h < a.Ho && w >= 0 && w < a.Wo;
                e_h[k] = h; e_w[k] = w; e_in[k] = in;
                e_q[k] = in ? (((size_t)b * a.Ho + h) * a.Wo + w) * a.Cout + co : 0;
                e_res[k] = make_float4(0.f, 0.f, 0.f, 0.f);
                if (e_first_pass && a.residual) e_res[k] = ld_raw_f32x4_or_h4(a.residual, e_q[k], a.res_f16 != 0);
            });
    };
    if constexpr (NHWC) {
        constexpr int UPT = G::RS * CCk / 4, UPP = CCk / 4;
        int z_t[NS], z_p[NS], z_c[NS], z_h[NS], z_w[NS], z_b[NS];
        bool z_live[NS];
        static_for<0, NS>([&](auto i_tag) {
            constexpr int i = decltype(i_tag)::value;
            const int v = tid + NT * i;
            const int t_l = v / UPT;
            const int p = (v - t_l * UPT) / UPP;
            const int c_l = ((v - t_l * UPT) - p * UPP) * 4;
            s_dst[i] = (t_l * G::RS + p) * LDC + c_l;
            s_cl[i] = c_l;
            z_c[i] = c_l; z_p[i] = p;
            z_t[i] = mb * G::TPB + t_l;
            z_live[i] = v < UNITS && z_t[i] < a.T;
        });
        if (SRC != SRC_TILES) {
            static_for<0, NS>([&](auto i_tag) {
                constexpr int i = decltype(i_tag)::value;
                const int tt = min(z_t[i], a.T - 1);
                const int b = tt / a.N, n = tt - b * a.N;
                const int2 o = *reinterpret_cast<const int2 *>(a.idx + 2 * n);
                z_b[i] = b; z_h[i] = o.x + z_p[i] / G::R; z_w[i] = o.y + z_p[i] % G::R;
            });
        }
        if constexpr (EPRE) {
            static_for<0, EU>([&](auto k_tag) {
                constexpr int k = decltype(k_tag)::value;
                const int o = tid + k * NT;
                const int nb = o / UNITS_NB, o1 = o - nb * UNITS_NB;
                const int m = o1 / (G::MT / 4);
                const int tt = min(mb * G::TPB + m / G::PX, a.T - 1);
                const int n = tt - (tt / a.N) * a.N;
                const int2 og = *reinterpret_cast<const int2 *>(a.idx + 2 * n);
                e_h[k] = og.x; e_w[k] = og.y;
            });
        }
        if constexpr (EPV) static_for<0, EU>([&](auto k_tag) {
            constexpr int k = decltype(k_tag)::value;
            const int o = tid + k * NT;
            const int nb = o / UNITS_NB, o1 = o - nb * UNITS_NB;
            const int co = (ng * NB + nb) * G::MT + 4 * (o1 % (G::MT / 4));
            const int cs = (o < OUT_UNITS && co < a.Cout) ? co : 0;
            e_bias[k] = e_os[k] = e_oh[k] = make_float4(0.f, 0.f, 0.f, 0.f);
            if (e_first_pass) {
                if (a.bias) e_bias[k] = *reinterpret_cast<const float4 *>(a.bias + cs);
                if (a.oscale) {
                    e_os[k] = *reinterpret_cast<const float4 *>(a.oscale + cs);
                    e_oh[k] = *reinterpret_cast<const float4 *>(a.oshift + cs);
                }
            }
        });
        if (AFF) {
            tab_fetch(first, t_sc, t_sh);
            tab_fetch(min(first + 1, last), t_sc1, t_sh1);
        }
        SIGE_PROBE(7);
        b_prologue();
        int z_hw[NS], z_m0[NS], z_m1[NS], z_m2[NS];
        static_for<0, NS>([&](auto i_tag) {
            constexpr int i = decltype(i_tag)::value;
            unsigned off = kOOB, off2 = kOOB;
            const int t = z_t[i], c_l = z_c[i];
            if (SRC == SRC_TILES) {
                off = z_live[i] ? (unsigned)((t * G::RS + z_p[i]) * Cin + c_l) * 4u : kOOB;
            } else {
                const int h = z_h[i], w = z_w[i], b = z_b[i];
                int hlo = 0, hhi = a.H;
                if (a.hp_shift) {
                    hlo = ((h - z_p[i] / G::R + 2) >> a.hp_shift) << a.hp_shift;
                    hhi = hlo + (1 << a.hp_shift);
                }
                const bool in = z_live[i] && h >= hlo && h < hhi && w >= 0 && w < a.W;
                z_live[i] = in;
                const int hw = (SRC == SRC_GATHER) ? (h >> a.up) * (a.W >> a.up) + (w >> a.up) : h * a.W + w;
                if (SRC == SRC_GATHER) {
                    off = in ? (unsigned)((b * HW + hw) * a.Csplit + c_l) * 4u : kOOB;
                    off2 = in ? (unsigned)(hw * (Cin - a.Csplit) + c_l) * 4u : kOOB;
                } else {
                    const int hwc = in ? hw : 0;
                    z_hw[i] = hwc;
                    const int32_t *m = a.map + 3 * (size_t)hwc;
                    z_m0[i] = m[0]; z_m1[i] = m[1]; z_m2[i] = m[2];
                }
            }
            if (SRC != SRC_SCATTER_GATHER) {
                s_off[i] = off;
                if (TWO) s_off2[i] = (off == kOOB ? 0u : off2 - off);
                if (AFF) s_tab[i] = (off != kOOB || off2 != kOOB) ? c_l : CCk;
            }
        });
        if constexpr (SRC == SRC_SCATTER_GATHER) {
            static_for<0, NS>([&](auto i_tag) {
                constexpr int i = decltype(i_tag)::value;
                const int blk = z_m0[i], c_l = z_c[i], b = z_b[i];
                const bool in = z_live[i];
                const unsigned off = (in && blk >= 0)
                    ? (unsigned)(((b * a.N + blk) * a.RxSx + z_m1[i] * a.Sx + z_m2[i]) * Cin + c_l) * 4u : kOOB;
                const unsigned off2 = (in && blk < 0) ? (unsigned)((b * HW + z_hw[i]) * Cin + c_l) * YB : kOOB;
                s_off[i] = off;
                s_off2[i] = off2;
                if (AFF) s_tab[i] = in ? c_l : CCk;
            });
        }
    } else {
    static_for<0, NS>([&](auto i_tag) {
        constexpr int i = decltype(i_tag)::value;
        const int v = tid + NT * i;
        int t_l, c_l, p;
        if (NHWC) {
            constexpr int UPT = G::RS * CCk / 4, UPP = CCk / 4;
            t_l = v / UPT;
            p = (v - t_l * UPT) / UPP;
            c_l = ((v - t_l * UPT) - p * UPP) * 4;
            s_dst[i] = (t_l * G::RS + p) * LDC + c_l;
        } else if (VEC) {
            constexpr int U4 = TILEF / 4;
            t_l = v / U4;
            const int e = (v - t_l * U4) * 4;
            c_l = e / G::RS; p = e - c_l * G::RS;
            s_dst[i] = 4 * v;
        } else {
            t_l = v / TILEF;
            c_l = (v - t_l * TILEF) / G::RS;
            p = (v - t_l * TILEF) - c_l * G::RS;
            s_dst[i] = v;
        }
        if (VEC) s_cl[i] = c_l;
        const int t = mb * G::TPB + t_l;
        unsigned off = kOOB, off2 = kOOB;
        if (v < UNITS && t < a.T) {
            if (SRC == SRC_TILES) {
                off = NHWC ? (unsigned)((t * G::RS + p) * Cin + c_l) * 4u : (unsigned)(t * Cin * G::RS + (v % (TILEF / 4)) * 4) * 4u;
            } else {
                const int b = t / a.N;
                const int n = t - b * a.N;
                const int h = a.idx[2 * n] + p / G::R, w = a.idx[2 * n + 1] + p % G::R;
                if (h >= 0 && h < a.H && w >= 0 && w < a.W) {
                    const int hw = (SRC == SRC_GATHER) ? (h >> a.up) * (a.W >> a.up) + (w >> a.up) : h * a.W + w;
                    if (SRC == SRC_GATHER) {
                        if (NHWC) {
                            off = (unsigned)((b * HW + hw) * a.Csplit + c_l) * 4u;
                            off2 = (unsigned)(hw * (Cin - a.Csplit) + c_l) * 4u;
                        } else {
                            off = (unsigned)((b * Cin + c_l) * HW + hw) * 4u;
                        }
                    } else {
                        const int32_t *m = a.map + 3 * (size_t)hw;
                        const int blk = m[0];
                        if (NHWC) {
                            if (blk >= 0) off = (unsigned)(((b * a.N + blk) * a.RxSx + m[1] * a.Sx + m[2]) * Cin + c_l) * 4u;
                            else off2 = (unsigned)((b * HW + hw) * Cin + c_l) * 4u;
                        } else {
                            if (blk >= 0) off = (unsigned)(((b * a.N + blk) * Cin + c_l) * a.RxSx + m[1] * a.Sx + m[2]) * 4u;
                            else off2 = (unsigned)((b * Cin + c_l) * HW + hw) * 4u;
                        }
                    }
                }
// ... 364 lines not shown
                        pv[sidx] = coherent_load(a.out + (size_t)(sidx < a.ksplit ? sidx : a.ksplit - 1) * a.split_stride + u.addr);
                    float4 s = pv[0];
#pragma unroll
                    for (int sidx = 1; sidx < 8; ++sidx)
                        if (sidx < a.ksplit) { s.x += pv[sidx].x; s.y += pv[sidx].y; s.z += pv[sidx].z; s.w += pv[sidx].w; }
                    emit(k_tag, u, s, a.fout);
                });
            }
        }
        SIGE_PROBE(5);
        return;
    }
    const float *const biasp = split_k ? nullptr : a.bias;
    const float *const resp = split_k ? nullptr : a.residual;
    constexpr int P4 = G::PX / 4;
#pragma unroll
    for (int o = tid; o < OUT_UNITS; o += NT) {
        const int nb = o / UNITS_NB, o1 = o - nb * UNITS_NB;
        const int p4 = o1 % P4;
        const int co_l = (o1 / P4) % G::MT;
        const int t_l = o1 / (P4 * G::MT);
        const int rrow = t_l * G::PX + p4 * 4;
        const float *r0 = red + (nb * G::MT + co_l) * RP + rrow;
        float4 s = *reinterpret_cast<const float4 *>(r0);
#pragma unroll
        for (int w = 1; w < W; ++w) {
            const float4 v = *reinterpret_cast<const float4 *>(r0 + w * NB * G::MT * RP);
            s.x += v.x; s.y += v.y; s.z += v.z; s.w += v.w;
        }
        const int t = mb * G::TPB + t_l, co = (ng * NB + nb) * G::MT + co_l;
        if (t < a.T && co < a.Cout) {
            const float bb = biasp ? biasp[co] : 0.0f;
            s.x += bb; s.y += bb; s.z += bb; s.w += bb;
            if (DST == DST_TILES) {
                *reinterpret_cast<float4 *>(outp + ((size_t)t * a.Cout + co) * G::PX + p4 * 4) = s;
            } else {
                const int b = t / a.N, n = t - b * a.N;
                const int h0 = (a.offH + a.idx[2 * n]) / a.strH, w0 = (a.offW + a.idx[2 * n + 1]) / a.strW;
                const size_t plane = ((size_t)b * a.Cout + co) * a.Ho * a.Wo;
                const float sv[4] = {s.x, s.y, s.z, s.w};
                if (G::RO == 4) {
                    const int h = h0 + p4;
                    if (h >= 0 && h < a.Ho) {
                        const size_t q = plane + (size_t)h * a.Wo + w0;
                        if (w0 >= 0 && w0 + 3 < a.Wo && ((q & 3) == 0)) {
                            float4 ov = s;
                            if (resp) {
                                const float4 rr = *reinterpret_cast<const float4 *>(resp + q);
                                ov.x += rr.x; ov.y += rr.y; ov.z += rr.z; ov.w += rr.w;
                            }
                            *reinterpret_cast<float4 *>(outp + q) = ov;
                        } else {
#pragma unroll
                            for (int i = 0; i < 4; ++i)
                                if (w0 + i >= 0 && w0 + i < a.Wo)
                                    outp[q + i] = sv[i] + (resp ? resp[q + i] : 0.0f);
                        }
                    }
                } else {
#pragma unroll
                    for (int i = 0; i < 4; ++i) {
                        const int pp = p4 * 4 + i;
                        const int h = h0 + pp / G::RO, w = w0 + pp % G::RO;
                        if (h >= 0 && h < a.Ho && w >= 0 && w < a.Wo) {
                            const size_t q = plane + (size_t)h * a.Wo + w;
                            outp[q] = sv[i] + (resp ? resp[q] : 0.0f);
                        }
                    }
                }
            }
        }
    }
}

inline int conv_grid_x(const ConvArgs &a) { return a.ng_fast == 2 ? 8 * ((a.mbk + 7) / 8) * a.ngk : a.mbk * a.ngk; }

template <typename G, int NB, int SRC, int MODE, int DST, int LAYOUT = LAYOUT_NCHW, int W = 4, bool Y16 = false>
__global__ __launch_bounds__(64 * W) void conv_mfma_kernel(const ConvArgs a) {
    kernarg_touch<sizeof(ConvArgs)>();
    __shared__ __attribute__((aligned(16))) float smem[conv_lds_floats<G, NB, MODE, LAYOUT, W>()];
    conv_mfma_body<G, NB, SRC, MODE, DST, LAYOUT, W, Y16>(a, blockIdx.x, blockIdx.y, smem);
}

template <typename GA, int NBA, typename GB, int DST, int W, int MODEA>
__global__ __launch_bounds__(64 * W) void conv_pair_kernel(const ConvArgs a, const ConvArgs b, const int na) {
    kernarg_touch<2 * sizeof(ConvArgs)>();
    constexpr int LA = conv_lds_floats<GA, NBA, MODEA, LAYOUT_NHWC, W>();
    constexpr int LB = conv_lds_floats<GB, 1, MODE_RAW, LAYOUT_NHWC, W>();
    __shared__ __attribute__((aligned(16))) float smem[cmax(LA, LB)];
    if ((int)blockIdx.x < na)
        conv_mfma_body<GA, NBA, SRC_GATHER, MODEA, DST, LAYOUT_NHWC, W>(a, blockIdx.x, blockIdx.y, smem);
    else if (blockIdx.y == 0)
        conv_mfma_body<GB, 1, SRC_GATHER, MODE_RAW, DST, LAYOUT_NHWC, W>(b, blockIdx.x - na, 0, smem);
}

template <typename GA, int NBA, typename GB, int DST, int W>
void launch_conv_pair(ConvArgs a, ConvArgs b, int mode_a, hipStream_t st);

#define SIGE_CONV_PAIR_INSTANTIATE(GA, NBA, GB, DST, W)                                                   \
    template <> void launch_conv_pair<GA, NBA, GB, DST, W>(ConvArgs a, ConvArgs b, int mode_a, hipStream_t st) { \
        const int na = conv_grid_x(a);                                                                    \
        const dim3 grid(na + conv_grid_x(b), a.ksplit);                                                   \
        if (mode_a == MODE_RAW) conv_pair_kernel<GA, NBA, GB, DST, W, MODE_RAW><<<grid, 64 * W, 0, st>>>(a, b, na); \
        else conv_pair_kernel<GA, NBA, GB, DST, W, MODE_AFFINE_SWISH><<<grid, 64 * W, 0, st>>>(a, b, na);  \
    }


template <typename GA, int NBA, typename GB, int NBB, int DST, int W, int MODEA>
__global__ __launch_bounds__(64 * W) void conv_side_kernel(const ConvArgs a, const ConvArgs b, const int na, const int b_off) {
    kernarg_touch<2 * sizeof(ConvArgs)>();
    constexpr int LA = conv_lds_floats<GA, NBA, MODEA, LAYOUT_NHWC, W>();
    constexpr int LB = conv_lds_floats<GB, NBB, MODE_RAW, LAYOUT_NHWC, W>();
    __shared__ __attribute__((aligned(16))) float smem[cmax(LA, LB)];
    if ((int)blockIdx.x < na)
        conv_mfma_body<GA, NBA, SRC_GATHER, MODEA, DST, LAYOUT_NHWC, W>(a, blockIdx.x, blockIdx.y, smem);
    else if (blockIdx.y == 0)
        conv_mfma_body<GB, NBB, SRC_GATHER, MODE_RAW, DST, LAYOUT_NHWC, W>(b, b_off + (int)blockIdx.x - na, 0, smem);
}

template <typename GA, int NBA, typename GB, int NBB, int DST, int W>
void launch_conv_side(ConvArgs a, ConvArgs b, int mode_a, int na, int b_off, int nb_blocks, hipStream_t st);

#define SIGE_CONV_SIDE_INSTANTIATE(GA, NBA, GB, NBB, DST, W)                                              \
    template <> void launch_conv_side<GA, NBA, GB, NBB, DST, W>(ConvArgs a, ConvArgs b, int mode_a, int na, int b_off, \
                                                                int nb_blocks, hipStream_t st) {          \
        const dim3 grid(na + nb_blocks, na ? a.ksplit : 1);                                               \
        if (mode_a == MODE_RAW) conv_side_kernel<GA, NBA, GB, NBB, DST, W, MODE_RAW><<<grid, 64 * W, 0, st>>>(a, b, na, b_off); \
        else conv_side_kernel<GA, NBA, GB, NBB, DST, W, MODE_AFFINE_SWISH><<<grid, 64 * W, 0, st>>>(a, b, na, b_off); \
    }

template <typename G, int NB, int SRC, int DST, int LAYOUT, int W>
void launch_conv_geo(ConvArgs a, int mode, hipStream_t st);

#define SIGE_CONV_LAUNCH3(G, NB, SRC, DST, LAY, W)                                                        \
    template <> void launch_conv_geo<G, NB, SRC, DST, LAY, W>(ConvArgs a, int mode, hipStream_t st) {     \
        const dim3 grid(conv_grid_x(a), a.ksplit);                                                        \
        if (mode == MODE_AFFINE_SWISH) conv_mfma_kernel<G, NB, SRC, MODE_AFFINE_SWISH, DST, LAY, W><<<grid, 64 * W, 0, st>>>(a); \
        else if (mode == MODE_AFFINE) conv_mfma_kernel<G, NB, SRC, MODE_AFFINE, DST, LAY, W><<<grid, 64 * W, 0, st>>>(a);        \
        else conv_mfma_kernel<G, NB, SRC, MODE_RAW, DST, LAY, W><<<grid, 64 * W, 0, st>>>(a);             \
    }

#define SIGE_CONV_INSTANTIATE(G, NB, LAY, W)                                                              \
    template <> void launch_conv_geo<G, NB, SRC_TILES, DST_TILES, LAY, W>(ConvArgs a, int, hipStream_t st) { \
        conv_mfma_kernel<G, NB, SRC_TILES, MODE_RAW, DST_TILES, LAY, W><<<dim3(conv_grid_x(a), a.ksplit), 64 * W, 0, st>>>(a); \
    }                                                                                                     \
    SIGE_CONV_LAUNCH3(G, NB, SRC_GATHER, DST_TILES, LAY, W)                                               \
    SIGE_CONV_LAUNCH3(G, NB, SRC_GATHER, DST_NCHW, LAY, W)                                                \
    SIGE_CONV_LAUNCH3(G, NB, SRC_SCATTER_GATHER, DST_TILES, LAY, W)

template <typename G, int NB, int DST>
void launch_conv_c16(ConvArgs a, int mode, hipStream_t st);
#define SIGE_CONV_INSTANTIATE_C16_DST(G, NB, DST)                                                         \
    template <> void launch_conv_c16<G, NB, DST>(ConvArgs a, int mode, hipStream_t st) {                  \
        const dim3 grid(conv_grid_x(a), a.ksplit);                                                        \
        if (mode == MODE_AFFINE_SWISH) conv_mfma_kernel<G, NB, SRC_SCATTER_GATHER, MODE_AFFINE_SWISH, DST, LAYOUT_NHWC, 4, true><<<grid, 256, 0, st>>>(a); \
        else if (mode == MODE_AFFINE) conv_mfma_kernel<G, NB, SRC_SCATTER_GATHER, MODE_AFFINE, DST, LAYOUT_NHWC, 4, true><<<grid, 256, 0, st>>>(a);        \
        else conv_mfma_kernel<G, NB, SRC_SCATTER_GATHER, MODE_RAW, DST, LAYOUT_NHWC, 4, true><<<grid, 256, 0, st>>>(a);             \
    }
#define SIGE_CONV_INSTANTIATE_C16(G, NB) SIGE_CONV_INSTANTIATE_C16_DST(G, NB, DST_TILES) SIGE_CONV_INSTANTIATE_C16_DST(G, NB, DST_NCHW)

#define SIGE_CONV_INSTANTIATE_SG_FULL(G, NB, LAY, W) SIGE_CONV_LAUNCH3(G, NB, SRC_SCATTER_GATHER, DST_NCHW, LAY, W)

}
```

### sige_amd/hip.py

```python
import ctypes
import os
import threading
from typing import Optional, Tuple

import torch

_PKG = os.path.dirname(os.path.abspath(__file__))
LIB_PATH = os.environ.get("SIGE_HIP_LIB", os.path.join(_PKG, "lib", "libsige_hip.so"))

ACT = {"identity": 0, "swish": 1}
ACT_EXT = {"identity": 0, "relu": 2, "leaky": 3, "tanh": 4}

_c_int, _c_vp, _c_sz = ctypes.c_int, ctypes.c_void_p, ctypes.c_size_t
_lib = None

_BC = [_c_vp, _c_int, _c_int, _c_int, _c_int]

_SIGNATURES = {
    "sige_hip_version": (_c_int, []),
    "sige_hip_error_string": (ctypes.c_char_p, [_c_int]),
    "sige_hip_device_arch": (ctypes.c_char_p, []),
    "sige_hip_launch_count": (ctypes.c_int64, []),
    "sige_hip_last_launch_device": (_c_int, []),
    "sige_hip_preload": (_c_int, []),
    "sige_hip_gather_f32": (_c_int, [_c_vp] + [_c_int] * 6 + [_c_vp, _c_int] + _BC + _BC + [_c_int, _c_int, _c_vp, _c_vp]),
    "sige_hip_scatter_f32": (_c_int, [_c_vp, _c_vp] + [_c_int] * 10 + [_c_vp, _c_int] + _BC + [_c_vp, _c_vp]),
    "sige_hip_scatter_with_block_residual_f32": (
        _c_int, [_c_vp] * 4 + [_c_int] * 12 + [_c_vp, _c_int, _c_vp, _c_int, _c_vp, _c_vp]),
    "sige_hip_tile_table_i32": (_c_int, [_c_vp] + [_c_int] * 9 + [_c_vp, _c_vp]),
    "sige_hip_scatter_fused_f32": (_c_int, [_c_vp, _c_vp] + [_c_int] * 6 + [_c_vp, _c_int, _c_int, _c_int] + _BC + [_c_vp, _c_vp]),
    "sige_hip_scatter_with_block_residual_fused_f32": (
        _c_int, [_c_vp] * 4 + [_c_int] * 8 + [_c_vp, _c_int, _c_int, _c_int] * 2 + [_c_vp, _c_vp]),
    "sige_hip_scatter_map_i32": (_c_int, [_c_int] * 10 + [_c_vp, _c_int, _c_vp, _c_vp]),
    "sige_hip_scatter_gather_f32": (
        _c_int, [_c_vp, _c_vp] + [_c_int] * 8 + [_c_vp, _c_int, _c_vp] + _BC + _BC + [_c_int, _c_int, _c_vp, _c_vp]),
    "sige_hip_difference_mask_u8": (_c_int, [_c_vp, _c_vp] + [_c_int] * 3 + [ctypes.c_int64] * 3 + [ctypes.c_float, _c_vp, _c_vp]),
    "sige_hip_dilate_mask_u8": (_c_int, [_c_vp] + [_c_int] * 4 + [_c_vp, _c_vp]),
    "sige_hip_mask_pyramid_levels": (_c_int, [_c_int] * 4 + [_c_vp, _c_vp, _c_int]),
    "sige_hip_mask_pyramid_u8": (_c_int, [_c_vp] + [_c_int] * 6 + [ctypes.c_float] * 2 + [_c_vp, _c_sz, _c_vp, _c_vp]),
    "sige_hip_reduce_mask_capacity": (_c_int, [_c_int] * 6),
    "sige_hip_reduce_mask_i32": (_c_int, [_c_vp] + [_c_int] * 8 + [_c_vp, _c_int, _c_vp, _c_vp]),
    "sige_hip_demand_tiles_capacity": (_c_int, [_c_int] * 4),
    "sige_hip_demand_tiles_i32": (_c_int, [_c_vp, _c_vp] + [_c_int] * 13 + [_c_vp, _c_vp, _c_vp]),
    "sige_hip_change_tiles_i32": (_c_int, [_c_vp, _c_vp] + [_c_int] * 16 + [_c_vp, _c_vp, _c_vp]),
    "sige_hip_block_conv_packed_size": (_c_sz, [_c_int] * 9),
    "sige_hip_block_conv_packed_size_f16c": (_c_sz, [_c_int] * 9),
    "sige_hip_block_conv_pack_f16c": (_c_int, [_c_vp] + [_c_int] * 4 + [_c_vp, _c_vp]),
    "sige_hip_block_conv_pack_f32": (_c_int, [_c_vp] + [_c_int] * 4 + [_c_vp, _c_vp]),
    "sige_hip_block_conv_f32": (_c_int, [_c_vp] + [_c_int] * 4 + [_c_vp, _c_vp] + [_c_int] * 5 + [_c_vp, _c_vp]),
    "sige_hip_gather_conv_f32": (
        _c_int, [_c_vp] + [_c_int] * 6 + [_c_vp, _c_int] + _BC + _BC + [_c_int, _c_vp, _c_vp] + [_c_int] * 5 + [_c_vp, _c_vp]),
    "sige_hip_scatter_gather_conv_f32": (
        _c_int, [_c_vp, _c_vp] + [_c_int] * 8 + [_c_vp, _c_int, _c_vp] + _BC + _BC + [_c_int, _c_vp, _c_vp]
        + [_c_int] * 5 + [_c_vp, _c_vp]),
    "sige_hip_gather_conv_nchw_f32": (
        _c_int, [_c_vp, _c_vp] + [_c_int] * 7 + [_c_vp, _c_int] + [_c_vp, _c_int, _c_int] * 2 + [_c_int, _c_vp, _c_vp]
        + [_c_int] * 7 + [_c_vp, _c_int, _c_int, _c_vp, _c_vp]),
    "sige_hip_group_norm_affine_workspace": (_c_sz, [_c_int] * 5),
    "sige_hip_group_norm_affine_f32": (_c_int, [_c_vp] + [_c_int] * 5 + [ctypes.c_float] + [_c_vp] * 6),
    "sige_hip_block_conv_direct_f32": (_c_int, [_c_vp] + [_c_int] * 4 + [_c_vp, _c_vp] + [_c_int] * 8 + [_c_vp, _c_vp]),
    "sige_hip_conv_pair_begin": (_c_int, []),
    "sige_hip_conv_pair_end": (_c_int, []),
    "sige_hip_conv_pairs_fused": (ctypes.c_int64, []),
    "sige_hip_conv_side_begin": (_c_int, [_c_int]),
    "sige_hip_conv_side_flush": (_c_int, []),
    "sige_hip_conv_side_workgroups": (ctypes.c_int64, [_c_int]),
    "sige_hip_attention_workspace": (_c_sz, [_c_int] * 3),
    "sige_hip_attention_f32": (_c_int, [_c_vp, _c_int, _c_int, _c_int, ctypes.c_float, _c_vp, _c_vp, _c_vp]),
    "sige_hip_copy_f32": (_c_int, [_c_vp, _c_vp, _c_sz, _c_vp]),
    "sige_hip_block_conv_nhwc": (_c_int, [_c_int, _c_vp] + [_c_int] * 4 + [_c_vp, _c_vp] + [_c_int] * 5 + [_c_vp, _c_vp]),
    "sige_hip_block_conv_nhwc_keyed": (_c_int, [_c_int, _c_vp, _c_vp] + [_c_int] * 5 + [_c_vp, _c_vp] + [_c_int] * 5 + [_c_vp, _c_vp]),
    "sige_hip_gather_conv_nhwc": (
        _c_int, [_c_int, _c_vp, _c_vp] + [_c_int] * 7 + [_c_vp, _c_int] + [_c_vp, _c_int, _c_int] * 2 + [_c_int, _c_vp, _c_vp]
        + [_c_int] * 5 + [_c_int, _c_int, _c_int, _c_vp, _c_int, _c_int, _c_vp, _c_sz, _c_vp, _c_vp, _c_int, _c_int] + [_c_vp] * 6
        + [_c_vp, _c_int] + [_c_vp, _c_vp]),
    "sige_hip_scatter_gather_conv_nhwc": (
        _c_int, [_c_int, _c_vp, _c_vp, _c_int] + [_c_int] * 8 + [_c_vp, _c_int, _c_vp] + [_c_vp, _c_int, _c_int] * 2 + [_c_int, _c_vp, _c_vp]
        + [_c_int] * 5 + [_c_vp, _c_vp]),
    "sige_hip_scatter_gather_conv_scatter_nhwc": (
        _c_int, [_c_int, _c_vp, _c_vp, _c_int] + [_c_int] * 8 + [_c_vp, _c_int, _c_vp] + [_c_vp, _c_int, _c_int] * 2 + [_c_int, _c_vp, _c_vp]
        + [_c_int] * 3 + [_c_int, _c_int, _c_vp, _c_int] + [_c_vp, _c_vp] + [_c_int] * 5 + [_c_vp] * 6 + [_c_vp, _c_int] + [_c_vp, _c_vp]),
    "sige_hip_tile_conv3_nhwc": (
        _c_int, [_c_int, _c_int, _c_vp, _c_vp, _c_int] + [_c_int] * 6 + [_c_vp, _c_int, _c_vp, _c_int, _c_int] + [_c_vp, _c_vp, _c_int, _c_int]
        + [_c_vp, _c_vp, _c_int] + [_c_int] * 5 + [_c_vp, _c_int] + [_c_vp, _c_vp] + [_c_int] * 5 + [_c_vp, _c_vp, _c_int] + [_c_vp] * 6 + [_c_vp, _c_vp]),
    "sige_hip_conv_ksplit_hint": (_c_int, [_c_int] * 7),
    "sige_hip_gather_nhwc_f32": (
        _c_int, [_c_vp] + [_c_int] * 6 + [_c_vp, _c_int] + [_c_vp, _c_int, _c_int] * 2 + [_c_int, _c_vp, _c_vp]),
    "sige_hip_scatter_gather_nhwc_f32": (
        _c_int, [_c_vp, _c_vp] + [_c_int] * 8 + [_c_vp, _c_int, _c_vp] + [_c_vp, _c_int, _c_int] * 2 + [_c_int, _c_vp, _c_vp]),
    "sige_hip_resample_tiles_nhwc_f32": (
        _c_int, [_c_vp] + [_c_int] * 5 + [_c_vp, _c_int, _c_int, _c_int] + [_c_vp] * 3 + [_c_int] * 6 + [_c_vp, _c_vp]),
    "sige_hip_spade_modulate_nhwc_f32": (
        _c_int, [_c_vp, _c_vp, _c_vp, _c_int, _c_int, _c_int] + [_c_vp, _c_int, _c_int] * 2 + [_c_vp, _c_vp, _c_vp, _c_int, _c_int, _c_int]
        + [_c_int] * 6 + [_c_vp, _c_int, _c_int, ctypes.c_float, _c_vp, _c_vp]),
    "sige_hip_scatter_nhwc_f32": (
        _c_int, [_c_vp, _c_vp] + [_c_int] * 10 + [_c_vp, _c_vp, _c_int, _c_int, _c_int, _c_vp, _c_int, _c_vp, _c_vp]),
    "sige_hip_scatter_with_block_residual_nhwc_f32": (
        _c_int, [_c_vp] * 4 + [_c_int] * 12 + [_c_vp, _c_vp, _c_int, _c_int, _c_int] * 2 + [_c_int, _c_vp, _c_vp]),
    "sige_hip_group_norm_affine_nhwc_workspace": (_c_sz, [_c_int] * 5),
    "sige_hip_group_norm_affine_nhwc_f32": (_c_int, [_c_vp] + [_c_int] * 5 + [ctypes.c_float] + [_c_vp] * 6),
    "sige_hip_group_norm_affine_nhwc_bias_f32": (_c_int, [_c_vp] + [_c_int] * 5 + [ctypes.c_float] + [_c_vp] * 7),
    "sige_hip_conv3x3_small_cout_nhwc_f32": (
        _c_int, [_c_vp] + [_c_int] * 4 + [_c_vp, _c_int, _c_int] * 2 + [_c_int, _c_vp, _c_vp, _c_int, _c_vp, _c_vp]),
    "sige_hip_conv3x3_small_cin_nhwc_f32": (
        _c_int, [_c_vp] + [ctypes.c_int64] * 4 + [_c_int] * 4 + [_c_vp, _c_vp, _c_int, _c_vp, _c_vp]),
    "sige_hip_conv3x3_small_cin_tiles_nhwc_f32": (
        _c_int, [_c_vp] + [ctypes.c_int64] * 4 + [_c_int] * 4 + [_c_vp, _c_vp, _c_int, _c_vp, _c_int, _c_int, _c_int, _c_vp, _c_vp]),
    "sige_hip_attention_nhwc_f32": (_c_int, [_c_vp, _c_int, _c_int, _c_int, ctypes.c_float, _c_vp, _c_vp, _c_vp]),
    "sige_hip_attention_residual_nhwc_f32": (_c_int, [_c_vp, _c_int, _c_int, _c_int, ctypes.c_float, _c_vp] + [_c_vp] * 10),
    "sige_hip_attention_residual_qv_nhwc_f32": (_c_int, [_c_vp, _c_vp, _c_vp, _c_int, _c_int, _c_int, _c_int, ctypes.c_float, _c_vp] + [_c_vp] * 10),
    "sige_hip_attention_fused_workspace": (_c_sz, [_c_int] * 3),
    "sige_hip_attention_fused_nhwc_f32": (_c_int, [_c_vp, _c_int, _c_int, _c_int, ctypes.c_float, _c_vp, _c_vp, _c_vp]),
    "sige_hip_block_conv_packed_size_f16x3": (_c_sz, [_c_int] * 9),
    "sige_hip_block_conv_pack_f16x3": (_c_int, [_c_vp] + [_c_int] * 4 + [_c_vp, _c_vp]),
    "sige_hip_affine_act_nhwc_f32": (_c_int, [_c_vp] + [_c_int] * 4 + [_c_vp, _c_vp, _c_int, _c_int, _c_vp, _c_vp]),
    "sige_hip_wide_conv_supported": (_c_int, [_c_int] * 5),
    "sige_hip_wide_conv_packed_size": (_c_sz, [_c_int] * 5),
    "sige_hip_wide_conv_pack": (_c_int, [_c_vp] + [_c_int] * 6 + [_c_vp, _c_vp]),
    "sige_hip_wide_conv_workspace": (_c_sz, [_c_int] * 8),
    "sige_hip_wide_conv_nhwc": (
        _c_int, [_c_vp, _c_vp] + [_c_int] * 6 + [_c_vp, _c_vp, _c_int, _c_int] + [_c_vp, _c_int, _c_int, _c_vp, _c_int, _c_int, _c_int]
        + [_c_vp, _c_vp, _c_vp, _c_int] + [_c_vp] * 6 + [_c_vp, _c_sz, _c_vp, _c_vp, _c_vp]),
    "sige_hip_release_graph_tickets": (_c_int, []),
    "sige_hip_channel_stats_tiles": (_c_int, [_c_int, _c_int]),
    "sige_hip_channel_stats_nhwc_f32": (_c_int, [_c_vp] + [_c_int] * 4 + [_c_vp, _c_vp]),
    "sige_hip_group_norm_affine_from_stats_f32": (
        _c_int, [_c_vp, _c_int, _c_int, _c_int, _c_vp, _c_int, _c_int, _c_int, _c_int, _c_int, ctypes.c_float] + [_c_vp] * 6),
    "sige_hip_attention_tokens_supported": (_c_int, [_c_int] * 4),
    "sige_hip_attention_tokens_f32": (_c_int, [_c_vp] * 3 + [_c_int] * 5 + [ctypes.c_float, _c_vp, _c_vp]),
    "sige_hip_attention_wide_supported": (_c_int, [_c_int] * 4),
    "sige_hip_attention_wide_f32": (_c_int, [_c_vp, _c_int] * 3 + [_c_int] * 5 + [ctypes.c_float, _c_vp, _c_int, _c_vp]),
# ... 567 lines not shown
    m = _mask_u8(mask)
    H, W = m.shape
    out = torch.empty_like(m)
    _check(lib().sige_hip_dilate_mask_u8(m.data_ptr(), H, W, max(0, dilation[0]), max(0, dilation[1]), out.data_ptr(),
                                         _stream(m)), "dilate_mask")
    _plan_keep(out, m)
    return out.view(torch.bool)


def mask_pyramid(mask: torch.Tensor, min_res: Tuple[int, int], dilation: Tuple[int, int], threshold: float, eps: float):
    m = _mask_u8(mask)
    H, W = m.shape
    E = get_edit_batch()
    if H % E:
        raise RuntimeError("mask_pyramid: the mask's height is not a multiple of the edit batch %d" % E)
    Hp = H // E
    n = lib().sige_hip_mask_pyramid_levels(Hp, W, min_res[0], min_res[1], None, None, 0)
    hs, ws = (ctypes.c_int * n)(), (ctypes.c_int * n)()
    lib().sige_hip_mask_pyramid_levels(Hp, W, min_res[0], min_res[1], hs, ws, n)
    sizes = [(E * int(hs[i]), int(ws[i])) for i in range(n)]
    out = torch.empty(sum(h * w for h, w in sizes), dtype=torch.uint8, device=m.device)
    n_scratch = E * ((Hp // 2) * (W // 2) + (Hp // 4) * (W // 4) + (Hp * W + 3) // 4 + 8)
    scratch = torch.empty(n_scratch, dtype=torch.float32, device=m.device)
    _check(lib().sige_hip_mask_pyramid_u8(m.data_ptr(), H, W, min_res[0], min_res[1], max(0, dilation[0]), max(0, dilation[1]),
                                          float(threshold), float(eps), scratch.data_ptr(), n_scratch, out.data_ptr(),
                                          _stream(m)), "mask_pyramid")
    _plan_keep(out, scratch, m)
    pyramid, off = {}, 0
    for h, w in sizes:
        pyramid[(h, w)] = out[off:off + h * w].view(h, w).view(torch.bool)
        off += h * w
    return pyramid


def conv_packed_size(Cout, Cin, kH, kW, R, S, strH, strW, groups=1) -> int:
    return int(lib().sige_hip_block_conv_packed_size(Cout, Cin, kH, kW, R, S, strH, strW, groups))


class PackedWeights(torch.Tensor):
    compute = "f32"
    wshift = 0

    @classmethod
    def __torch_function__(cls, func, types, args=(), kwargs=None):
        out = super().__torch_function__(func, types, args, kwargs or {})
        if isinstance(out, PackedWeights):
            src = next((a for a in args if isinstance(a, PackedWeights)), None)
            if src is not None and src is not out:
                out.compute = src.__dict__.get("compute", "f32")
                out.wshift = src.__dict__.get("wshift", 0)
        return out


def conv_pack_weights(weight: torch.Tensor, R: int, S: int, stride: Tuple[int, int], compute: str = "f32") -> Optional[torch.Tensor]:
    w = _req(weight.detach(), torch.float32, "weight")
    Cout, Cin, kH, kW = w.shape
    if compute not in ("f32", "f16", "f16x3"):
        raise ValueError("compute must be 'f32', 'f16' or 'f16x3'")
    n = 0
    if compute == "f16":
        n = int(lib().sige_hip_block_conv_packed_size_f16c(Cout, Cin, kH, kW, R, S, stride[0], stride[1], 1))
        if n == 0:
            compute = "f32"
    if compute == "f16x3":
        n = int(lib().sige_hip_block_conv_packed_size_f16x3(Cout, Cin, kH, kW, R, S, stride[0], stride[1], 1))
        if n == 0:
            compute = "f32"
    if compute == "f32":
        n = conv_packed_size(Cout, Cin, kH, kW, R, S, stride[0], stride[1], 1)
    if n == 0:
        return None
    packed = torch.empty((n,), dtype=torch.float32, device=w.device).as_subclass(PackedWeights)
    packed.compute = compute
    fn = {"f16": lib().sige_hip_block_conv_pack_f16c, "f16x3": lib().sige_hip_block_conv_pack_f16x3,
          "f32": lib().sige_hip_block_conv_pack_f32}[compute]
    _check(fn(w.data_ptr(), Cout, Cin, kH, kW, packed.data_ptr(), _stream(w)), "conv_pack_weights")
    if compute in ("f32", "f16") and (kH, kW) == (3, 3) and (R, S) == (6, 6) and tuple(stride) == (1, 1) and Cin % 64 == 0 and Cout % 64 == 0:
        packed._tile3_src = w
        if TILE3 is not False and TILE3_MIN_BLOCKS is not None:
            _tile3_pack_now(packed)
    return packed


COMPUTE_DTYPES = ("f32", "f16", "f16x3")


_COMPUTE_ID = {"f32": 0, "f16": 1, "f16x3": 2}
_WIDE_PREC = {"f16": 0, "f16x3": 1, "f32": 2}


def _compute_id(packed) -> int:
    return _COMPUTE_ID[getattr(packed, "compute", "f32")]


def wide_conv_supported(C1: int, C2: int, Cout: int, kernel: Tuple[int, int]) -> bool:
    return bool(lib().sige_hip_wide_conv_supported(C1, C2, Cout, kernel[0], kernel[1]))


def wide_conv_pack_weights(weight: torch.Tensor, compute: str) -> Optional[torch.Tensor]:
    if compute not in _WIDE_PREC:
        raise ValueError("compute must be 'f16', 'f16x3' or 'f32'")
    w = _req(weight.detach(), torch.float32, "weight")
    Cout, Cin, kH, kW = w.shape
    prec = _WIDE_PREC[compute]
    x3 = compute == "f16x3"
    n = int(lib().sige_hip_wide_conv_packed_size(Cout, Cin, kH, kW, prec))
    if n == 0:
        return None
    wshift = 0
    if x3:
        import math

        m = float(w.abs().max())
        if m > 0 and math.isfinite(m):
            wshift = max(-40, min(40, 13 - math.frexp(m)[1] + 1))
    packed = torch.empty((n,), dtype=torch.float32, device=w.device).as_subclass(PackedWeights)
    packed.compute = compute + "w"
    packed.wshift = wshift
    _check(lib().sige_hip_wide_conv_pack(w.data_ptr(), Cout, Cin, kH, kW, prec, wshift, packed.data_ptr(), _stream(w)),
           "wide_conv_pack_weights")
    return packed


def wide_conv_force_ksplit(ksplit: int = 0):
    tuning_set("wide_ksplit", ksplit)


def wide_conv_cl(x, x2, scale, shift, activationName: str, packed, bias, Cout: int, kernel: Tuple[int, int],
                 residual=None, out_affine: Optional[tuple] = None, twins=None, upsample2x: bool = False,
                 out: Optional[torch.Tensor] = None, stats: bool = False):
    compute = getattr(packed, "compute", "f32")
    if compute not in ("f16w", "f16x3w", "f32w"):
        raise NotImplementedError("wide_conv_cl: weights must be packed with wide_conv_pack_weights")
    bias_keep = _vec(bias, "bias")
    x = _req_cl(x, "x")
    B, C1, H, W = x.shape
    if upsample2x:
        H, W = 2 * H, 2 * W
    C2 = 0
    if x2 is not None:
        x2 = _req_cl(x2, "x2")
        C2 = x2.shape[1]
        if tuple(x2.shape[2:]) != tuple(x.shape[2:]) or x2.shape[0] != B:
            raise RuntimeError("wide_conv_cl: x2 must match x in batch and resolution")
    if not wide_conv_supported(C1, C2, Cout, kernel):
        return None
    (sa, s_keep), (ta, t_keep) = _cvec(scale, "scale"), _cvec(shift, "shift")
    if (s_keep is None) != (t_keep is None):
        return None
    if s_keep is not None and (sa[1] != ta[1] or sa[2] != C1 + C2 or ta[2] != C1 + C2 or sa[1] not in (1, B)):
        return None
    if s_keep is None and activationName != "identity":
        return None
    if out is None:
        out = _empty_cl((B, Cout, H, W), x.device)
    elif tuple(out.shape) != (B, Cout, H, W) or not out.is_contiguous(memory_format=CL):
        raise RuntimeError("wide_conv_cl: `out` must be a channels-last [B,Cout,H,W] tensor")
    r = None
    if residual is not None:
        r = _req_cl(residual, "residual")
        if tuple(r.shape) != tuple(out.shape):
            raise RuntimeError("wide_conv_cl: residual %s != output %s" % (tuple(r.shape), tuple(out.shape)))
    if out_affine is not None:
        os_, oh_, oact = out_affine
        os_, oh_ = _req(os_.reshape(-1), torch.float32, "out_scale", 1), _req(oh_.reshape(-1), torch.float32, "out_shift", 1)
        if os_.numel() != Cout or oh_.numel() != Cout:
# ... 485 lines not shown
    if status == UNSUPPORTED:
        return None
    _check(status, "block_conv_cl")
    return tag_tiles(out, idx, B) if keyed else out


TILE3 = None
TILE3_MIN_BLOCKS = 512
TILE3_MIN_BLOCKS_F16 = 256


def _tile3_min_blocks(packed) -> int:
    return int(TILE3_MIN_BLOCKS_F16 if getattr(packed, "compute", "f32") == "f16" else TILE3_MIN_BLOCKS)


def _tile3_pack_now(packed):
    t3 = wide_conv_pack_weights(packed._tile3_src, "f16" if getattr(packed, "compute", "f32") == "f16" else "f32")
    packed.tile3 = False if t3 is None else t3
    packed._tile3_src = None
    return t3


def _tile3_packed(packed):
    if TILE3 is False or (TILE3 is None and TILE3_MIN_BLOCKS is None):
        return None
    t3 = getattr(packed, "tile3", None)
    if t3 is False:
        return None
    if t3 is None:
        src = getattr(packed, "_tile3_src", None)
        if src is None or torch.cuda.is_current_stream_capturing():
            return None
        t3 = _tile3_pack_now(packed)
    return t3


def _tile3_args(packed, t3r):
    return (None, 0) if t3r is None else (t3r.data_ptr(), _tile3_min_blocks(packed))


def _tile3_route(packed, T: int, C1: int, C2: int, Cout: int, kernel, stride, block):
    if TILE3 is not True:
        return None
    if tuple(kernel) != (3, 3) or tuple(stride) != (1, 1) or tuple(block) != (6, 6) or C1 % 64 or C2 % 64 or Cout % 64:
        return None
    return _tile3_packed(packed)


def tile_conv3_cl(source: int, x, x2, B, C1, C2, H, W, up, idx, smap, rx_sx, scale, shift, activationName, t3, bias, Cout,
                  full, residual, bargs, out_affine, targs, out, compute: int = 0):
    bias_keep = _vec(bias, "bias")
    sc = sh = None
    affB = 0
    if scale is not None:
        (sa, s_keep), (ta, t_keep) = _cvec(scale, "scale"), _cvec(shift, "shift")
        if sa[2] != C1 + C2 or ta[2] != C1 + C2 or sa[1] != ta[1]:
            return None
        sc, sh, affB = sa[0], ta[0], sa[1]
    if out_affine is not None:
        os_, oh_, oact = out_affine
        os_, oh_ = _req(os_.reshape(-1), torch.float32, "out_scale", 1), _req(oh_.reshape(-1), torch.float32, "out_shift", 1)
        if os_.numel() != Cout or oh_.numel() != Cout:
            raise RuntimeError("tile_conv3_cl: out_affine must have one entry per output channel")
        oargs = (os_.data_ptr(), oh_.data_ptr(), _act(oact))
    else:
        oargs = (None, None, 0)
    fargs = (0, 0, 0, 0, 0) if full is None else (1, *full)
    y16 = int(x2 is not None and x2.dtype == torch.float16)
    r16 = int(residual is not None and residual.dtype == torch.float16)
    status = lib().sige_hip_tile_conv3_nhwc(
        compute, source, x.data_ptr(), None if x2 is None else x2.data_ptr(), y16, B, C1, C2, H, W, int(bool(up)), idx.data_ptr(), idx.shape[0],
        None if smap is None else smap.data_ptr(), rx_sx[0], rx_sx[1], sc, sh, affB, _act(activationName),
        t3.data_ptr(), _p(bias_keep), Cout, *fargs, None if residual is None else residual.data_ptr(), r16, *bargs, *oargs, *targs,
        out.data_ptr(), _stream(x))
    if status == UNSUPPORTED:
        return None
    _check(status, "tile_conv3_cl")
    return out


def gather_conv_cl(x, x2, block: Tuple[int, int], activeIndices, scale, shift, activationName: str,
                   packed, bias, Cout: int, kernel: Tuple[int, int], stride: Tuple[int, int],
                   full: Optional[dict] = None, out_affine: Optional[tuple] = None, upsample2x: bool = False,
                   out: Optional[torch.Tensor] = None, twins=None):
    bias_keep = _vec(bias, "bias")
    x = _req_cl(x, "x")
    B, C1, H, W = x.shape
    if upsample2x:
        H, W = 2 * H, 2 * W
    C2 = 0
    if x2 is not None:
        x2 = _req_cl(x2, "x2")
        C2 = x2.shape[1]
    idx = _req(activeIndices, torch.int32, "activeIndices", 2)
    (sa, s_keep), (ta, t_keep) = _cvec(scale, "scale"), _cvec(shift, "shift")
    N = idx.shape[0]
    if full is None:
        Ro, So = (block[0] - kernel[0]) // stride[0] + 1, (block[1] - kernel[1]) // stride[1] + 1
        out = _empty_tiles_cl(B, idx, Cout, Ro, So, x.device)
        fargs = (0, 0, 0, None, 0, 0)
    else:
        Ho, Wo = full["out_res"]
        if out is None:
            out = _empty_cl((B, Cout, Ho, Wo), x.device)
        elif tuple(out.shape) != (B, Cout, Ho, Wo) or not out.is_contiguous(memory_format=CL):
            raise RuntimeError("gather_conv_cl: `out` must be a channels-last [B,Cout,Ho,Wo] tensor")
        r = full.get("residual")
        if r is not None:
            r = _req_cl(r, "residual")
            if tuple(r.shape) != tuple(out.shape):
                raise RuntimeError("gather_conv_cl: residual %s != output %s" % (tuple(r.shape), tuple(out.shape)))
        fargs = (1, full["offset"][0], full["offset"][1], None if r is None else r.data_ptr(), Ho, Wo)
    compute = _compute_id(packed)
    t3 = _tile3_route(packed, B * N, C1, C2, Cout, kernel, stride, block)
    if getattr(_side_state, "armed", False):
        t3 = None
    if t3 is not None and N > 0:
        if twins and full is None:
            raise RuntimeError("gather_conv_cl: twins need a full-tensor destination")
        targs3, twin_keep3 = _twin_args(twins if twins else None, out, Cout, "gather_conv_cl")
        got = tile_conv3_cl(1, x, x2, B, C1, C2, H, W, upsample2x, idx, None, (0, 0), scale, shift, activationName, t3, bias, Cout,
                            None if full is None else (full["offset"][0], full["offset"][1], Ho, Wo),
                            None if full is None else r, (None, None, 0, 0, 0, 0, 0), out_affine, targs3, out, compute=compute)
        if got is not None:
            return got if full is not None else tag_tiles(got, idx, B)
    ws, ws_n = None, 0
    ks = lib().sige_hip_conv_ksplit_hint(B * N, C1 + C2, Cout, kernel[0], kernel[1], stride[0], stride[1])
    if full is not None and N * ((block[0] - kernel[0]) // stride[0] + 1) * ((block[1] - kernel[1]) // stride[1] + 1) < Ho * Wo:
        ks = 1
    cap = _tile_capacity(idx)
    if cap is not None and full is None and KSPLIT:
        px = ((block[0] - kernel[0]) // stride[0] + 1) * ((block[1] - kernel[1]) // stride[1] + 1)
        t_split = min(B * cap, max(1, 16 // px) * (224 // max(1, -(-Cout // 16)) + 1))
        ws_n = 8 * t_split * px * Cout
        ws = torch.empty(ws_n, dtype=torch.float32, device=x.device)
    elif ks > 1 and KSPLIT:
        ws_n = ks * out.numel()
        ws = torch.empty(ws_n, dtype=torch.float32, device=x.device)
    fargs = fargs + (None if ws is None else ws.data_ptr(), ws_n)
    if out_affine is not None:
        os_, oh_, oact = out_affine
        os_, oh_ = _req(os_.reshape(-1), torch.float32, "out_scale", 1), _req(oh_.reshape(-1), torch.float32, "out_shift", 1)
        if os_.numel() != Cout or oh_.numel() != Cout:
            raise RuntimeError("gather_conv_cl: out_affine must have one entry per output channel")
        fargs = fargs + (os_.data_ptr(), oh_.data_ptr(), _act(oact))
    else:
        fargs = fargs + (None, None, 0)
    if twins and full is None:
        raise RuntimeError("gather_conv_cl: twins need a full-tensor destination")
    targs, twin_keep = _twin_args(twins if twins else None, out, Cout, "gather_conv_cl")
    fargs = fargs + (int(bool(upsample2x)), *targs)
    t3r = _tile3_packed(packed) if (TILE3 is None and compute in (0, 1)) else None
    status = lib().sige_hip_gather_conv_nhwc(
        compute, x.data_ptr(), None if x2 is None else x2.data_ptr(), B, C1, C2, H, W, block[0], block[1], idx.data_ptr(), N,
        *sa, *ta, _act(activationName), packed.data_ptr(), _p(bias_keep), Cout, kernel[0], kernel[1],
        stride[0], stride[1], *fargs, *_tile3_args(packed, t3r), out.data_ptr(), _stream(x))
    if status == UNSUPPORTED:
        return None
    _check(status, "gather_conv_cl")
    keep = getattr(_pair_state, "keep", None)
    if keep is not None:
        keep.append((x, x2, idx, s_keep, t_keep, packed, bias_keep, out, ws, out_affine, full, twin_keep))
    if getattr(_side_state, "armed", False):
        _side_state.armed = False
        _side_state.keep.append((x, x2, idx, s_keep, t_keep, packed, bias_keep, out, ws, out_affine, full, twin_keep))
    return out


def scatter_gather_conv_cl(x, y, block: Tuple[int, int], activeIndices, scatterMap, scale, shift, activationName: str,
                           packed, bias, Cout: int, kernel: Tuple[int, int], stride: Tuple[int, int]):
    bias_keep = _vec(bias, "bias")
    x, y = _req_cl(x, "x"), _req_cl_cache(y, "y")
    idx = _req(activeIndices, torch.int32, "activeIndices", 2)
    smap = _req(scatterMap, torch.int32, "scatterMap", 3)
    (sa, s_keep), (ta, t_keep) = _cvec(scale, "scale"), _cvec(shift, "shift")
    B, C, H, W = y.shape
    N = idx.shape[0]
    Ro, So = (block[0] - kernel[0]) // stride[0] + 1, (block[1] - kernel[1]) // stride[1] + 1
    out = _empty_tiles_cl(B, idx, Cout, Ro, So, y.device)
    status = lib().sige_hip_scatter_gather_conv_nhwc(
        _compute_id(packed), x.data_ptr(), y.data_ptr(), int(y.dtype == torch.float16), B, C, H, W, x.shape[2], x.shape[3],
        block[0], block[1], idx.data_ptr(), N, smap.data_ptr(), *sa, *ta, _act(activationName), packed.data_ptr(), _p(bias_keep),
        Cout, kernel[0], kernel[1], stride[0], stride[1], out.data_ptr(), _stream(y))
    if status == UNSUPPORTED:
        return None
    _check(status, "scatter_gather_conv_cl")
    return out


def scatter_gather_conv_scatter_cl(x, y, block, activeIndices, scatterMap, scale, shift, activationName: str,
                                   packed, bias, Cout: int, kernel, offset, out: torch.Tensor, residual=None,
                                   x1=None, table1=None, twins=None):
    bias_keep = _vec(bias, "bias")
    x, y = _req_cl(x, "x"), _req_cl_cache(y, "y")
    idx = _req(activeIndices, torch.int32, "activeIndices", 2)
    smap = _req(scatterMap, torch.int32, "scatterMap", 3)
    (sa, s_keep), (ta, t_keep) = _cvec(scale, "scale"), _cvec(shift, "shift")
    B, C, H, W = y.shape
    if tuple(out.shape) != (B, Cout, H, W) or not out.is_contiguous(memory_format=CL):
        raise RuntimeError("scatter_gather_conv_scatter_cl: `out` must be a channels-last [B,Cout,H,W] tensor")
    r = None if residual is None else (_req_cl_cache(residual, "residual") if x1 is not None else _req_cl(residual, "residual"))
    if r is not None and r.dtype == torch.float16 and y.dtype != torch.float16:
        return None
    if r is not None and tuple(r.shape) != tuple(out.shape):
        raise RuntimeError("scatter_gather_conv_scatter_cl: residual must be full size")
    if x1 is not None:
        x1 = _req_cl(x1, "x1")
        t1 = _req(table1, torch.int32, "table1", 2)
        bargs = (x1.data_ptr(), t1.data_ptr(), t1.shape[0], t1.shape[1], x1.shape[0] // B, x1.shape[2], x1.shape[3])
    else:
        bargs = (None, None, 0, 0, 0, 0, 0)
    targs, twin_keep = _twin_args(twins if twins else None, out, Cout, "scatter_gather_conv_scatter_cl")
    compute = _compute_id(packed)
    t3 = _tile3_route(packed, B * idx.shape[0], C, 0, Cout, kernel, (1, 1), block)
    f16c = compute == 1
    if (t3 is not None and idx.shape[0] > 0 and (f16c or (y.dtype == torch.float32 and (r is None or r.dtype == torch.float32)))
            and ((scale is None and shift is None and activationName == "identity") or (scale is not None and shift is not None))):
        got = tile_conv3_cl(2, x, y, B, C, 0, H, W, False, idx, smap, (x.shape[2], x.shape[3]), scale, shift, activationName, t3, bias, Cout,
                            (offset[0], offset[1], H, W), r, bargs, None, targs, out, compute=compute)
        if got is not None:
            return got
    t3r = _tile3_packed(packed) if (TILE3 is None and ((compute == 0 and y.dtype == torch.float32) or f16c)) else None
    status = lib().sige_hip_scatter_gather_conv_scatter_nhwc(
        compute, x.data_ptr(), y.data_ptr(), int(y.dtype == torch.float16), B, C, H, W, x.shape[2], x.shape[3], block[0], block[1],
        idx.data_ptr(), idx.shape[0], smap.data_ptr(), *sa, *ta, _act(activationName), packed.data_ptr(), _p(bias_keep), Cout,
        kernel[0], kernel[1], offset[0], offset[1], None if r is None else r.data_ptr(), int(r is not None and r.dtype == torch.float16),
        *bargs, *targs, *_tile3_args(packed, t3r), out.data_ptr(), _stream(y))
    if status == UNSUPPORTED:
        return None
    _check(status, "scatter_gather_conv_scatter_cl")
    return out


def gather_cl(x, bSizeH, bSizeW, activeIndices, scale=None, shift=None, activationName="identity"):
    x = _req_cl_cache(x, "x")
    idx = _req(activeIndices, torch.int32, "activeIndices", 2)
    (sa, s_keep), (ta, t_keep) = _cvec(scale, "scale"), _cvec(shift, "shift")
    B, C, H, W = x.shape
    N = idx.shape[0]
    out = _empty_tiles_cl(B, idx, C, bSizeH, bSizeW, x.device)
    fn = lib().sige_hip_gather_nhwc_f16 if x.dtype == torch.float16 else lib().sige_hip_gather_nhwc_f32
    _check(fn(x.data_ptr(), B, C, H, W, bSizeH, bSizeW, idx.data_ptr(), N, *sa, *ta, _act(activationName), out.data_ptr(), _stream(x)),
           "gather_cl")
    return tag_tiles(out, idx, B)

# ... 585 lines not shown
```

### sige_amd/nn/base.py

```python
from typing import Dict, List, Optional, Tuple

import torch
from torch import nn
from torch.nn import functional as F

from .. import runtime as _runtime
from . import deferred

MODES = ("full", "sparse", "profile")


class _RuntimeTable(dict):

    def __init__(self, function_name: str):
        super().__init__()
        self.function_name = function_name

    def __missing__(self, device_type: str):
        fn = _runtime.resolve(device_type, self.function_name)
        if fn is not None:
            self[device_type] = fn
        return fn


class SIGEModule(nn.Module):
    def __init__(self, call_super: bool = True):
        if call_super:
            super(SIGEModule, self).__init__()
        self.devices: List[str] = ["cpu", "cuda", "mps"]
        self.supported_dtypes = [torch.float32]
        self.mode: str = "full"
        self.runtime: Dict = {}
        self.mask: Optional[torch.Tensor] = None
        self.timestamp = None
        self.cache_id = 0
        self.sparse_update = False
        self.cache_dtype = "f32"

    def set_mask(self, masks: Dict, cache: Dict, timestamp: int):
        self.timestamp = timestamp

    def set_cache_id(self, cache_id: int):
        self.cache_id = cache_id

    def clear_cache(self):
        pass

    def set_sparse_update(self, sparse_update: bool):
        self.sparse_update = sparse_update

    def set_mode(self, mode: str):
        self.mode = mode

    def load_runtime(self, function_name: str, runtime_dict: Dict = None):
        table = _RuntimeTable(function_name)
        if runtime_dict is None:
            self.runtime = table
        return table

    def native(self, table: Dict, x: torch.Tensor):
        fn = table[x.device.type]
        if fn is None:
            raise RuntimeError(
                "[%s] no native backend for device type '%s': the sparse path runs on MI355X "
                "(torch-ROCm 'cuda' tensors) through libsige_hip.so only." % (type(self).__name__, x.device.type))
        return fn

    def check_dtype(self, *args):
        for x in args:
            if x is not None:
                assert isinstance(x, torch.Tensor)
                if x.dtype not in self.supported_dtypes:
                    raise NotImplementedError(
                        "[%s] does not support dtype [%s]!!! "
                        "Currently supported dtype %s." % (self.__class__.__name__, x.dtype, str(self.supported_dtypes))
                    )

    def check_dim(self, *args):
        for x in args:
            if x is not None:
                assert isinstance(x, torch.Tensor)
                if x.dim() != 4:
                    raise NotImplementedError(
                        "[%s] does not support input with dim [%d]!!!" % (self.__class__.__name__, x.dim())
                    )


class SIGEModuleWrapper:

    def __init__(self, module: SIGEModule):
        self.module = module


class SIGEConv2d(nn.Conv2d, SIGEModule):

    def __init__(self, *args, **kwargs):
        nn.Conv2d.__init__(self, *args, **kwargs)
        SIGEModule.__init__(self, call_super=False)
        self._packed = {}
        self._tiles_runtime = self.load_runtime("conv2d_tiles", {})
        self.compute_dtype = "f32"

    def _packed_weights(self, x: torch.Tensor, channels_last: bool = True):
        from .. import hip

        from .dense import TILE_X3_MIN_FLOP, _tile_compute

        compute = _tile_compute(self.compute_dtype) if channels_last else "f32"
        if compute == "f16x3":
            ro, so = (x.shape[2] - self.kernel_size[0]) // self.stride[0] + 1, (x.shape[3] - self.kernel_size[1]) // self.stride[1] + 1
            flop = 2.0 * x.shape[0] * ro * so * self.out_channels * self.in_channels * self.kernel_size[0] * self.kernel_size[1]
            if flop * (9 if tuple(self.kernel_size) == (1, 1) else 1) < TILE_X3_MIN_FLOP:
                compute = "f32"
        w = self.weight
        key = (w.data_ptr(), w._version, tuple(w.shape), x.shape[2], x.shape[3], w.device)
        entry = self._packed.get(compute)
        if entry is None or entry[0] != key:
            entry = (key, hip.conv_pack_weights(w, x.shape[2], x.shape[3], self.stride, compute))
            self._packed[compute] = entry
        return entry[1]

    def _block_conv(self, x: torch.Tensor, out_affine=None) -> torch.Tensor:
        from .. import hip

        if out_affine is not None:
            spec = x.spec if isinstance(x, deferred.DeferredTiles) else None
            packed = self._packed_weights(x) if self.groups == 1 and tuple(self.dilation) == (1, 1) else None
            if (packed is not None and spec is not None and spec["kind"] == "gather" and spec.get("cl", False)
                    and self.out_channels % 4 == 0):
                out = hip.gather_conv_cl(spec["x"], spec.get("x2"), spec["block"], spec["idx"], spec["scale"], spec["shift"],
                                         spec["act"], packed, self.bias, self.out_channels, self.kernel_size, self.stride,
                                         out_affine=out_affine, upsample2x=spec.get("up", False))
                if out is not None:
                    return out
            out = self._block_conv(x)
            os_, oh_, oact = out_affine
            out = out * os_.reshape(1, -1, 1, 1) + oh_.reshape(1, -1, 1, 1)
            return F.silu(out) if oact == "swish" else out

        plain = tuple(self.dilation) == (1, 1)
        spec = x.spec if isinstance(x, deferred.DeferredTiles) else None
        mfma = self.groups == 1 and plain
        if mfma and spec is not None:
            cl = spec.get("cl", False) and self.out_channels % 4 == 0
            packed = self._packed_weights(x, cl)
        if mfma and spec is not None and packed is not None:
            common = (packed, self.bias, self.out_channels, self.kernel_size, self.stride)
            if spec["kind"] == "gather":
                if cl:
                    out = hip.gather_conv_cl(spec["x"], spec.get("x2"), spec["block"], spec["idx"], spec["scale"],
                                             spec["shift"], spec["act"], *common, upsample2x=spec.get("up", False))
                elif spec.get("x2") is None and not spec.get("up", False):
                    out = hip.gather_conv(spec["x"], spec["block"], spec["idx"], spec["scale"], spec["shift"],
                                          spec["act"], *common)
                else:
                    out = None
            else:
                f = hip.scatter_gather_conv_cl if cl else hip.scatter_gather_conv
                out = f(spec["x"], spec["y"], spec["block"], spec["idx"], spec["map"], spec["scale"], spec["shift"],
                        spec["act"], *common)
            if out is not None:
                return out
        x = deferred.resolve(x)
        if mfma:
            if hip.is_cl(x) and x.shape[1] % 4 == 0 and self.out_channels % 4 == 0:
                packed = self._packed_weights(x, True)
                out = None if packed is None else hip.block_conv_cl(x, packed, self.bias, self.out_channels, self.kernel_size,
                                                                    self.stride)
                if out is not None:
                    return out
            packed = self._packed_weights(x, False)
            if packed is not None:
                return hip.block_conv(x, packed, self.bias, self.out_channels, self.kernel_size, self.stride)
        return hip.block_conv_direct(x, self.weight, self.bias, self.stride, self.groups, self.dilation)

    def forward(self, x: torch.Tensor, out_affine=None) -> torch.Tensor:
        if self.mode == "full":
            if x.is_cuda and self.compute_dtype != "f32":
                from .dense import full_conv2d

                output = full_conv2d(self, x)
            else:
                output = super(SIGEConv2d, self).forward(x)
        elif self.mode == "sparse":
            self.check_dtype(x)
            if x.is_cuda:
                output = self._block_conv(x, out_affine)
            else:
                conv = self.native(self._tiles_runtime, x)
                output = conv(deferred.resolve(x), self.weight, self.bias, self.stride, self.dilation, self.groups)
                if out_affine is not None:
                    os_, oh_, oact = out_affine
                    output = output * os_.reshape(1, -1, 1, 1) + oh_.reshape(1, -1, 1, 1)
                    output = F.silu(output) if oact == "swish" else output
        elif self.mode == "profile":
            output = F.conv2d(x, self.weight, self.bias, self.stride, (0, 0), self.dilation, self.groups)
        else:
            raise NotImplementedError("Unknown mode: %s" % self.mode)
        return output


class SIGEModel(nn.Module):
    def __init__(self, call_super: bool = True):
# ... 125 lines not shown
```

### sige_amd/nn/gather.py

```python
import warnings
from typing import Dict, Optional, Tuple, Union

import torch
from torch import nn

from ..utils import reduce_mask
from . import deferred
from .base import SIGEModule
from .utils import activation


class Gather(SIGEModule):
    def __init__(
        self,
        conv: nn.Conv2d,
        block_size: Union[int, Tuple[int, int]],
        offset: Optional[Union[int, Tuple[int, int]]] = None,
        activation_name: str = "identity",
        activation_first: bool = False,
        verbose: bool = False,
    ):
        super(Gather, self).__init__()
        if isinstance(block_size, int):
            block_size = (block_size, block_size)
        k, s = conv.kernel_size, conv.stride
        out_tile = tuple(max(block_size[i] - k[i], 0) // s[i] + 1 for i in (0, 1))
        fitted = tuple((out_tile[i] - 1) * s[i] + k[i] for i in (0, 1))
        if fitted != tuple(block_size):
            warnings.warn("Change the block size from (%d, %d) to (%d, %d)" % (*block_size, *fitted))

        self.model_stride = conv.stride
        self.kernel_size = conv.kernel_size
        self.block_size = fitted
        self.block_stride = (out_tile[0] * s[0], out_tile[1] * s[1])
        self.out_tile = out_tile
        if offset is None:
            self.offset = conv.padding
        else:
            self.offset = (offset, offset) if isinstance(offset, int) else offset
        self.activation_name = activation_name
        self.activation_first = activation_first
        self.verbose = verbose

        self.load_runtime("gather")

        self.input_res: Optional[Tuple[int, int]] = None
        self.active_indices: Optional[torch.Tensor] = None
        self._tables: Dict = {}

    def note_full_input(self, res):
        self.input_res = torch.Size(tuple(res))

    def forward(
        self, x: torch.Tensor, scale: Optional[torch.Tensor] = None, shift: Optional[torch.Tensor] = None,
        upsample2x: bool = False, preactivated: bool = False
    ) -> torch.Tensor:
        self.check_dtype(x, scale, shift)
        self.check_dim(x, scale, shift)
        if upsample2x:
            x = deferred.resolve(x)
            if not self.fuses_upsample(x, scale, shift):
                raise ValueError("Gather(upsample2x=True) needs the fused channels-last gather -> conv path "
                                 "(sparse mode, channels-last fp32 GPU tensor, per-channel affine); upsample in the model instead")
        if self.mode == "sparse":
            act_name = self.activation_name
            if preactivated:
                if scale is not None or shift is not None:
                    raise ValueError("Gather(preactivated=True) takes no scale / shift: the input already carries them")
                act_name = "identity"
            x2 = None
            if isinstance(x, deferred.LazyCat) and x.spec is not None:
                a, b = x.parts
                from .. import hip

                if (hip.cat_fusable(a.shape[0], a.shape[1], self.kernel_size) and a.shape[1] % 4 == 0 and b.shape[1] % 4 == 0
                        and deferred.defer_ok(a, scale, shift, self.activation_first, self.sparse_update, act_name)
                        and hip.is_cl(a) and hip.is_cl(b)):
                    x, x2 = a, b
            fn = self.native(self.runtime, x)
            x = deferred.resolve(x)
            cl = x2 is not None or deferred.channels_last_ok(x, scale, shift, self.activation_first)
            if not cl:
                x = x.contiguous()
            idx = self.indices_on(x.device)
            scale = None if scale is None else scale.contiguous()
            shift = None if shift is None else shift.contiguous()
            bh, bw = self.block_size
            act, first = act_name, self.activation_first

            def run():
                xx = x if x2 is None else torch.cat([x, x2], dim=1)
                if upsample2x:
                    xx = torch.nn.functional.interpolate(xx, scale_factor=2.0, mode="nearest")
                if cl:
                    from .. import hip

                    return hip.gather_cl(xx, bh, bw, idx, scale, shift, act)
                return fn(xx, bh, bw, idx, scale, shift, act, first)

            if deferred.defer_ok(x, scale, shift, first, self.sparse_update, act):
                channels = x.shape[1] + (0 if x2 is None else x2.shape[1])
                return deferred.DeferredTiles(
                    (x.shape[0] * idx.shape[0], channels, bh, bw), x.dtype, x.device, run,
                    dict(kind="gather", x=x, x2=x2, block=(bh, bw), idx=idx, scale=scale, shift=shift, act=act, cl=cl,
                         up=upsample2x))
            return run()
        if self.mode == "full":
            self.note_full_input(x.shape[2:])
            assert scale is None
            assert shift is None
            return x
        if self.mode == "profile":
            b, c = x.shape[:2]
            output = torch.full((b * self.active_indices.size(0), c, *self.block_size), fill_value=x[0, 0, 0, 0],
                                dtype=x.dtype, device=x.device)
            if scale is not None:
                output = output * scale[0, 0, 0, 0]
            if shift is not None:
                output = output + shift[0, 0, 0, 0]
            return activation(output, self.activation_name)
        raise NotImplementedError("Unknown mode: [%s]!!!" % self.mode)

    def set_mask(self, masks: Dict, cache: Dict, timestamp: int):
        if self.timestamp == timestamp:
            return
        super(Gather, self).set_mask(masks, cache, timestamp)
        assert self.input_res is not None
        res = tuple(self.input_res)
        self.mask = masks[res]
        key = self.index_key(res)
        if key not in cache:
            cache[key] = reduce_mask(self.mask, self.block_size, self.block_stride, self.offset, verbose=self.verbose)
        self.active_indices = cache[key]
        self._tables = cache.setdefault(("tile_tables", *key[1:], *self.model_stride, *self.out_tile), {})

    def fuses_upsample(self, x: torch.Tensor, scale=None, shift=None) -> bool:
        return (self.mode == "sparse" and not isinstance(x, deferred.LazyCat)
                and deferred.channels_last_ok(deferred.resolve(x), scale, shift, self.activation_first)
                and deferred.defer_ok(deferred.resolve(x), scale, shift, self.activation_first, self.sparse_update,
                                      self.activation_name))

    def index_key(self, res) -> tuple:
        return ("active_indices", *res, *self.block_size, *self.block_stride, *self.offset)

    def indices_on(self, device: torch.device) -> torch.Tensor:
        idx = self.active_indices
        if idx.device != device:
            idx = self._tables.get(("idx", device))
            if idx is None:
                idx = self.active_indices.to(device)
                self._tables[("idx", device)] = idx
        return idx if idx.is_contiguous() else idx.contiguous()

    def tile_table(self, out_res: Tuple[int, int], device: torch.device) -> torch.Tensor:
        key = ("table", tuple(out_res), device)
        table = self._tables.get(key)
        if table is None:
            from .. import hip

            table = hip.tile_table(self.indices_on(device), self.offset, self.model_stride, self.out_tile, out_res)
            self._tables[key] = table
        return table
```

### sige_amd/nn/scatter.py

```python
from typing import Optional

import torch

from . import deferred
from .base import SIGEModule, SIGEModuleWrapper
from .gather import Gather


def _fused_ok(x: torch.Tensor) -> bool:
    return x.is_cuda


def hip_is_cl(t: torch.Tensor) -> bool:
    from .. import hip

    return hip.is_cl(t)


def _cl_ok(cached: torch.Tensor, *others) -> bool:
    if not cached.is_cuda or cached.dtype not in (torch.float32, torch.float16):
        return False
    from .. import hip

    if not (hip.is_cl(cached) and cached.shape[1] % 4 == 0):
# ... 138 lines not shown
    def refresh_outputs(self, new_mask: bool = False):
        stamp = self.gather.module.timestamp if new_mask else None
        self._out_bufs.refresh(self.original_outputs, stamp)
        self.twins.refresh(self.original_outputs, stamp)

    def plan_tables(self):
        g: Gather = self.gather.module
        for cached in self.original_outputs.values():
            if cached.is_cuda and g.active_indices is not None:
                g.tile_table(cached.shape[2:], cached.device)

    def forward_fused(self, conv, tiles: torch.Tensor, residual: Optional[torch.Tensor] = None) -> torch.Tensor:
        if self.mode == "sparse" and self.inplace and not self.sparse_update:
            g: Gather = self.gather.module
            cached = self.original_outputs[self.cache_id]
            if _cl_ok(cached, residual) and isinstance(tiles, deferred.DeferredTiles) and tiles.spec is not None:
                out = self._out_bufs.get(self.cache_id, cached, g.timestamp)
                tw = self.twins.launch_args(self.cache_id, cached, g.timestamp)
                done = _fused_conv_into(conv, tiles, out, g, residual=residual, twins=[(b, sc, sh) for _, b, sc, sh in tw])
                if done is not None:
                    return tag_twins(done, {k: b for k, b, _, _ in tw})
        return self.forward(conv(tiles), residual)

    def forward(self, x: torch.Tensor, residual: Optional[torch.Tensor] = None) -> torch.Tensor:
        self.check_dtype(x, residual)
        self.check_dim(x, residual)
        if self.mode == "sparse":
            x = deferred.resolve(x)
            g: Gather = self.gather.module
            cached = self.original_outputs[self.cache_id]
            if _cl_ok(cached, residual):
                from .. import hip

                out = self._out_bufs.get(self.cache_id, cached, g.timestamp) if (self.inplace and not self.sparse_update) else None
                output = hip.scatter_cl(x, cached, g.offset, g.model_stride, g.indices_on(x.device),
                                        g.tile_table(cached.shape[2:], x.device), residual, out=out)
            elif _fused_ok(x):
                from .. import hip

                output = hip.scatter_fused(
                    x.contiguous(), deferred.from_cache(cached), g.tile_table(cached.shape[2:], x.device), g.active_indices.size(0),
                    None if residual is None else residual.contiguous())
            else:
                fn = self.native(self.runtime, x)
                output = fn(x.contiguous(), deferred.from_cache(cached).contiguous(), g.offset[0], g.offset[1],
                            g.model_stride[0], g.model_stride[1], g.indices_on(x.device),
                            None if residual is None else residual.contiguous())
            if self.sparse_update:
                cached.copy_(output)
                self._out_bufs.invalidate(self.cache_id)
                self.twins.invalidate(self.cache_id)
            return tag_twins(output, emulated_twins(output, twins_for(self.twins.regs, self.cache_id)) if EMULATE_TWINS else {})
        if self.mode == "full":
            output = x if residual is None else x + residual
            self.output_res = output.shape[2:]
            self.original_outputs[self.cache_id] = deferred.to_cache(output, self.cache_dtype)
            self._out_bufs.invalidate(self.cache_id)
            self.twins.invalidate(self.cache_id)
            return output
        if self.mode == "profile":
            c = x.shape[1]
            output = torch.full((self.original_outputs[self.cache_id].size(0), c, *self.output_res),
                                fill_value=x[0, 0, 0, 0], dtype=x.dtype, device=x.device)
            if residual is not None:
                output = output + residual
            return output
        raise NotImplementedError("Unknown mode: [%s]!!!" % self.mode)


def _fused_conv_into(conv, tiles, out, g: Gather, residual=None, x1=None, table1=None, twins=None):
    from .. import hip

    spec = tiles.spec if isinstance(tiles, deferred.DeferredTiles) else None
    if spec is None or not spec.get("cl", False) or conv.groups != 1 or tuple(conv.dilation) != (1, 1):
        return None
    if conv.out_channels % 4 or tuple(conv.stride) != tuple(g.model_stride):
        return None
    packed = conv._packed_weights(tiles, True)
    if packed is None:
        return None
    if spec["kind"] == "gather":
        if x1 is not None:
            return None
        return hip.gather_conv_cl(spec["x"], spec.get("x2"), spec["block"], spec["idx"], spec["scale"], spec["shift"], spec["act"],
                                  packed, conv.bias, conv.out_channels, conv.kernel_size, conv.stride,
                                  full=dict(offset=g.offset, out_res=tuple(out.shape[2:]), residual=residual),
                                  upsample2x=spec.get("up", False), out=out, twins=twins)
    if tuple(conv.kernel_size) != (3, 3) or tuple(conv.stride) != (1, 1):
        return None
    return hip.scatter_gather_conv_scatter_cl(spec["x"], spec["y"], spec["block"], spec["idx"], spec["map"], spec["scale"],
                                              spec["shift"], spec["act"], packed, conv.bias, conv.out_channels,
                                              conv.kernel_size, g.offset, out, residual=residual, x1=x1, table1=table1,
                                              twins=twins)


class ScatterWithBlockResidual(SIGEModule):

    def __init__(self, main_gather: Gather, shortcut_gather: Gather):
        super(ScatterWithBlockResidual, self).__init__()
        self.main_gather = SIGEModuleWrapper(main_gather)
        self.shortcut_gather = SIGEModuleWrapper(shortcut_gather)

        self.load_runtime("scatter_with_block_residual")
        self.scatter_runtime = None
        self.output_res = None
        self.original_outputs = {}
        self.original_residuals = {}
        self.inplace = False
        self._out_bufs = _OutputBuffers()
        self.twins = _TwinBuffers()

    def clear_cache(self):
        self.original_outputs = {}
        self.original_residuals = {}
        self._out_bufs.clear()
        self.twins.clear()

    def refresh_outputs(self, new_mask: bool = False):
        stamp = (self.main_gather.module.timestamp, self.shortcut_gather.module.timestamp) if new_mask else None
        self._out_bufs.refresh(self.original_outputs, stamp)
        self.twins.refresh(self.original_outputs, stamp)

    def plan_tables(self):
        for cached in self.original_outputs.values():
            if cached.is_cuda:
                for g in (self.main_gather.module, self.shortcut_gather.module):
                    if g.active_indices is not None:
                        g.tile_table(cached.shape[2:], cached.device)

    def forward_fused(self, conv, tiles: torch.Tensor, residual: torch.Tensor) -> torch.Tensor:
        if self.mode == "sparse" and self.inplace and not self.sparse_update:
            mg: Gather = self.main_gather.module
            sg: Gather = self.shortcut_gather.module
            y0 = self.original_outputs[self.cache_id]
            y1 = self.original_residuals[self.cache_id]
            if (_cl_ok(y0, y1) and hip_is_cl(y1) and isinstance(tiles, deferred.DeferredTiles) and tiles.spec is not None
                    and sg.active_indices.size(0) <= mg.active_indices.size(0)):
                out = self._out_bufs.get(self.cache_id, y0, (mg.timestamp, sg.timestamp))
                x1 = deferred.resolve(residual)
                tw = self.twins.launch_args(self.cache_id, y0, (mg.timestamp, sg.timestamp))
                done = _fused_conv_into(conv, tiles, out, mg, residual=y1, x1=x1, table1=sg.tile_table(y0.shape[2:], y0.device),
                                        twins=[(b, sc, sh) for _, b, sc, sh in tw])
                if done is not None:
                    return tag_twins(done, {k: b for k, b, _, _ in tw})
        return self.forward(conv(tiles), residual)

    def forward(self, x: torch.Tensor, residual: torch.Tensor, x_is_sum: bool = False) -> torch.Tensor:
        self.check_dtype(x, residual)
        self.check_dim(x, residual)
        assert not x_is_sum or self.mode == "full"
        if self.mode == "sparse":
            x, residual = deferred.resolve(x), deferred.resolve(residual)
            mg: Gather = self.main_gather.module
            sg: Gather = self.shortcut_gather.module
            y0 = self.original_outputs[self.cache_id]
            y1 = self.original_residuals[self.cache_id]
            res = y0.shape[2:]
            if _cl_ok(y0, y1) and hip_is_cl(y1):
                from .. import hip

                out = self._out_bufs.get(self.cache_id, y0, (mg.timestamp, sg.timestamp)) \
                    if (self.inplace and not self.sparse_update) else None
                output = hip.scatter_with_block_residual_cl(
                    x, y0, residual, y1, mg.offset, mg.model_stride, mg.indices_on(x.device), mg.tile_table(res, x.device),
                    sg.indices_on(x.device), sg.tile_table(res, x.device), out=out)
            elif _fused_ok(x):
                from .. import hip

                output = hip.scatter_with_block_residual_fused(
                    x.contiguous(), deferred.from_cache(y0), residual.contiguous(), deferred.from_cache(y1),
# ... 40 lines not shown
```

Baseline: 848.7 forward/s.

## Replace upsample+3x3 conv with four 2x2 phase convolutions on the low-res input

Adds a polyphase form of the nearest-upsample followed by a 3x3 convolution. The 3x3 weights are collapsed into four 2x2 kernels, one per output phase, and a new MFMA kernel variant (grid y = phase) reads the low-resolution input directly. This cuts the multiply-accumulates per output from 9 to 4 taps and avoids reading upsampled duplicates. In exchange it adds extra packed weight storage and a new kernel path. It falls back to the old path when the tile3 9-tap kernel would be chosen, or when the conditions (fp32, no affine, edit batch 1) are not met.

```diff
diff --git a/include/sige_hip.h b/include/sige_hip.h
--- a/include/sige_hip.h
+++ b/include/sige_hip.h
@@ -198,6 +198,8 @@
                               float *twin1, const float *twin1_scale, const float *twin1_shift,
                               const float *packed_tile3, int min_blocks,
                               float *out, void *stream);
+size_t sige_hip_upsample_phase_packed_size(int Cout, int Cin);
+int sige_hip_upsample_phase_pack_f32(const float *w_phases, int Cout, int Cin, float *packed, void *stream);
 int sige_hip_conv_ksplit_hint(int T, int Cin, int Cout, int kH, int kW, int strideH, int strideW);
 int sige_hip_scatter_gather_conv_nhwc(int compute, const float *x, const void *y, int y_f16, int B, int Cin, int H, int W,
                                       int Rx, int Sx, int bH, int bW,
diff --git a/sige_amd/build.py b/sige_amd/build.py
--- a/sige_amd/build.py
+++ b/sige_amd/build.py
@@ -9,7 +9,7 @@
 LIB = os.path.join(LIB_DIR, "libsige_hip.so")
 SOURCES = ["api.hip", "plan.hip", "gather.hip", "scatter.hip", "reduce_mask.hip", "mask_pipeline.hip", "block_conv.hip", "conv_k3s1.hip", "conv_k1.hip",
            "conv_k3s2.hip", "conv_k3s1_nhwc.hip", "conv_k1_nhwc.hip", "conv_k3s2_nhwc.hip", "conv_k3s1_nhwc_w8.hip", "conv_k1_nhwc_w8.hip", "conv_k3s1_nhwc_h.hip", "conv_k1_nhwc_h.hip", "conv_k3s1_nhwc_x.hip", "conv_k1_nhwc_x.hip", "conv_k3s1_nhwc_c16.hip", "conv_k3s1_nhwc_h_c16.hip", "conv_k3s1_nhwc_x_c16.hip", "conv_pair_nhwc_x_t4.hip", "conv_pair_nhwc_x_f4.hip",
-           "conv_pair_nhwc_t4.hip", "conv_pair_nhwc_t8.hip", "conv_pair_nhwc_f4.hip", "conv_pair_nhwc_f8.hip", "conv_pair_nhwc_h_t4.hip", "conv_pair_nhwc_h_f4.hip", "conv_wide.hip", "conv_wide_k3_p8.hip", "conv_wide_k3_f32.hip", "conv_wide_k1_p8.hip", "conv_wide_pair_f32.hip", "conv_wide_pair_x3.hip", "conv_wide_pair_f16.hip", "group_norm.hip", "attention.hip", "attention_fused.hip", "attention_tokens.hip", "nhwc_ops.hip", "conv_out.hip", "conv_in.hip", "spade_ops.hip", "conv_tile3.hip", "conv_tile3_f32.hip", "token_ops.hip", "conv_tile3_f16.hip", "token_linear.hip", "resample_tiles.hip", "attention_wide.hip", "conv_side_nhwc_f4.hip", "conv_latent_head.hip", "spade_separable.hip"]
+           "conv_pair_nhwc_t4.hip", "conv_pair_nhwc_t8.hip", "conv_pair_nhwc_f4.hip", "conv_pair_nhwc_f8.hip", "conv_pair_nhwc_h_t4.hip", "conv_pair_nhwc_h_f4.hip", "conv_wide.hip", "conv_wide_k3_p8.hip", "conv_wide_k3_f32.hip", "conv_wide_k1_p8.hip", "conv_wide_pair_f32.hip", "conv_wide_pair_x3.hip", "conv_wide_pair_f16.hip", "group_norm.hip", "attention.hip", "attention_fused.hip", "attention_tokens.hip", "nhwc_ops.hip", "conv_out.hip", "conv_in.hip", "spade_ops.hip", "conv_tile3.hip", "conv_tile3_f32.hip", "token_ops.hip", "conv_tile3_f16.hip", "token_linear.hip", "resample_tiles.hip", "attention_wide.hip", "conv_side_nhwc_f4.hip", "conv_latent_head.hip", "spade_separable.hip", "conv_up_phase_nhwc.hip"]
 FLAGS = ["--offload-arch=gfx950", "-O3", "-std=c++17", "-fPIC", "-ffp-contract=off", "-Wno-unused-result"]
 
 
diff --git a/sige_amd/csrc/block_conv.hip b/sige_amd/csrc/block_conv.hip
--- a/sige_amd/csrc/block_conv.hip
+++ b/sige_amd/csrc/block_conv.hip
@@ -199,6 +199,14 @@
 SIGE_CONV_DECLARE_C16(H31_16, 1) SIGE_CONV_DECLARE_C16(H31_16, 2) SIGE_CONV_DECLARE_C16(H31_32, 1) SIGE_CONV_DECLARE_C16(H31_32, 2)
 SIGE_CONV_DECLARE_C16(X31_16, 1) SIGE_CONV_DECLARE_C16(X31_32, 1)
 
+using P22_16 = ConvGeo<2, 1, 3, 16>;
+using P22_32 = ConvGeo<2, 1, 3, 32>;
+template <typename G, int NB>
+void launch_conv_phase(ConvArgs a, hipStream_t st);
+template <> void launch_conv_phase<P22_16, 1>(ConvArgs, hipStream_t);
+template <> void launch_conv_phase<P22_16, 2>(ConvArgs, hipStream_t);
+template <> void launch_conv_phase<P22_32, 1>(ConvArgs, hipStream_t);
+
 __global__ __launch_bounds__(256) void splitk_reduce_nhwc_kernel(const float *__restrict__ ws, int S, size_t stride, size_t n4, int C,
                                                                 const float *__restrict__ bias, const float *__restrict__ residual,
                                                                 const float *__restrict__ oscale, const float *__restrict__ oshift, int oact,
@@ -670,6 +678,38 @@
     return SIGE_HIP_OK;
 }
 
+static int launch_phase_up(ConvArgs a, hipStream_t st) {
+    int rc = flush_held();
+    if (rc != SIGE_HIP_OK) return rc;
+    if (!g_side.empty() && (g_side.front().st != st || side_hazard(a))) {
+        rc = flush_side();
+        if (rc != SIGE_HIP_OK) return rc;
+    }
+    ConvArgs q = a;
+    ConvPlan p;
+    rc = plan_conv<3, 1, 6, SRC_GATHER, LAYOUT_NHWC, 0>(q, 1, 0, false, p);
+    if (rc != SIGE_HIP_OK) return rc;
+    const int mt = p.mt, nb = (mt == 16 && p.nb == 2) ? 2 : 1;
+    const int cc = mt == 32 ? P22_32::CC : P22_16::CC;
+    a.mbk = ceil_div(a.T, mt / 4);
+    a.ngk = ceil_div(a.Cout, mt * nb);
+    a.nchunks = ceil_div(a.Cin, cc);
+    a.nblk = ((a.nchunks + 1) & ~1) * 4;
+    a.ksplit = 1;
+    a.chunks_per_split = a.nchunks;
+    a.counters = nullptr;
+    a.ng_fast = 4.0 * a.Cout * a.Cin > 9.0 * a.T * a.Cin ? 1 : ((a.mbk >= 16 && a.ngk > 1) ? 2 : 0);
+    if (mt == 16) a.packed += 4 * packed_floats(a.Cout, a.Cin, 4, 32);
+    a.phase_up = 1;
+#ifdef SIGE_CONV_PROBE
+    a.probe = nullptr;
+#endif
+    if (mt == 32) launch_conv_phase<P22_32, 1>(a, st);
+    else if (nb == 2) launch_conv_phase<P22_16, 2>(a, st);
+    else launch_conv_phase<P22_16, 1>(a, st);
+    return launch_status();
+}
+
 template <int SRC, int DST = DST_TILES, int LAY = LAYOUT_NCHW, int PREC = 0>
 static int launch_conv(const ConvArgs &a, int mode, int kH, int kW, int R, int S, int strH, int strW, hipStream_t st) {
     int rc;
@@ -758,6 +798,24 @@
         pack_weights_kernel<1, 16><<<blocks(n16), 256, 0, st>>>(w, Cout, Cin, packed + n32, n16);
     }
     return launch_status(2);
+}
+
+extern "C" size_t sige_hip_upsample_phase_packed_size(int Cout, int Cin) {
+    if (Cout <= 0 || Cin <= 0) return 0;
+    return 4 * (packed_floats(Cout, Cin, 4, 32) + packed_floats(Cout, Cin, 4, 16));
+}
+
+extern "C" int sige_hip_upsample_phase_pack_f32(const float *w_phases, int Cout, int Cin, float *packed, void *stream) {
+    if (!w_phases || !packed || Cout <= 0 || Cin <= 0) return SIGE_HIP_EINVAL;
+    hipStream_t st = as_stream(stream);
+    const long n32 = (long)packed_floats(Cout, Cin, 4, 32), n16 = (long)packed_floats(Cout, Cin, 4, 16);
+    auto blocks = [](long n) { return (int)((n + 255) / 256 < 4096 ? (n + 255) / 256 : 4096); };
+    for (int ph = 0; ph < 4; ++ph) {
+        const float *w = w_phases + (size_t)ph * Cout * Cin * 4;
+        pack_weights_kernel<4, 32><<<blocks(n32), 256, 0, st>>>(w, Cout, Cin, packed + ph * n32, n32);
+        pack_weights_kernel<4, 16><<<blocks(n16), 256, 0, st>>>(w, Cout, Cin, packed + 4 * n32 + ph * n16, n16);
+    }
+    return launch_status(8);
 }
 
 extern "C" size_t sige_hip_block_conv_packed_size_f16c(int Cout, int Cin, int kH, int kW, int R, int S,
@@ -1001,7 +1059,9 @@
                                              float *twin1, const float *twin1_scale, const float *twin1_shift,
                                              float *out, void *stream) {
     const int Cin = C1 + C2;
+    if (upsample2x < 0 || upsample2x > 2) return SIGE_HIP_EINVAL;
     if (upsample2x && ((H | W) & 1)) return SIGE_HIP_EINVAL;
+    if (upsample2x == 2 && PREC != 0) return SIGE_HIP_EUNSUPPORTED;
     if (B < 0 || C1 <= 0 || C2 < 0 || Cout <= 0 || H <= 0 || W <= 0 || N < 0) return SIGE_HIP_EINVAL;
     if (to_full && (Ho <= 0 || Wo <= 0)) return SIGE_HIP_EINVAL;
     if (activation != SIGE_HIP_ACT_IDENTITY && activation != SIGE_HIP_ACT_SWISH) return SIGE_HIP_EUNSUPPORTED;
@@ -1042,10 +1102,15 @@
     a.twin1 = twin1; a.tscale1 = twin1_scale; a.tshift1 = twin1_shift;
     if (to_full) {
         a.residual = residual; a.Ho = Ho; a.Wo = Wo; a.offH = offsetH; a.offW = offsetW; a.strH = strideH; a.strW = strideW;
+        if constexpr (PREC == 0) {
+            if (upsample2x == 2) return launch_phase_up(a, as_stream(stream));
+        }
         return launch_conv<SRC_GATHER, DST_NCHW, LAYOUT_NHWC, PREC>(a, mode, kH, kW, bH, bW, strideH, strideW, as_stream(stream));
     }
     return launch_conv<SRC_GATHER, DST_TILES, LAYOUT_NHWC, PREC>(a, mode, kH, kW, bH, bW, strideH, strideW, as_stream(stream));
 }
+
+extern "C" size_t sige_hip_upsample_phase_packed_size(int Cout, int Cin);
 
 constexpr int kTile3F16PairMin = 256;
 
@@ -1092,7 +1157,18 @@
     const int Cin = C1 + C2;
     const bool f16 = compute == 1;
     const bool aff_ok = (!scale && !shift) || (scale && shift && scaleC == Cin && shiftC == Cin && scaleB == shiftB && (scaleB == 1 || scaleB == B));
-    if ((compute == 0 || f16) && B > 0 && N > 0 && aff_ok && !(g_side_armed > 0 && compute == 0 && to_full) &&
+    if (upsample2x == 2) {
+        if (compute != 0 || C2 || kH != 3 || kW != 3 || bH != 6 || bW != 6 || strideH != 1 || strideW != 1 || !to_full || scale || shift ||
+            activation != SIGE_HIP_ACT_IDENTITY || stacked_shift(H) != 0 || g_side_armed > 0)
+            return SIGE_HIP_EUNSUPPORTED;
+        const bool nine_tap = B > 0 && N > 0 &&
+                              tile3_takes(packed_tile3, min_blocks, B, N, C1, C2, Cout, kH, kW, bH, bW, strideH, strideW, as_stream(stream));
+        if (nine_tap) {
+            upsample2x = 1;
+            packed += sige_hip_upsample_phase_packed_size(Cout, Cin);
+        }
+    }
+    if (upsample2x != 2 && (compute == 0 || f16) && B > 0 && N > 0 && aff_ok && !(g_side_armed > 0 && compute == 0 && to_full) &&
         tile3_takes(packed_tile3, min_blocks, B, N, C1, C2, Cout, kH, kW, bH, bW, strideH, strideW, as_stream(stream), f16, f16 ? H : 0, f16 ? W : 0)) {
         const int rc = tile_conv3_launch(T3_GATHER, x, x2, B, C1, C2, H, W, upsample2x, active_indices, N, nullptr, 0, 0, scale, shift,
                                          scale ? scaleB : 0, activation, packed_tile3, bias, Cout, to_full, offsetH, offsetW, Ho, Wo,
diff --git a/sige_amd/csrc/conv_mfma.hpp b/sige_amd/csrc/conv_mfma.hpp
--- a/sige_amd/csrc/conv_mfma.hpp
+++ b/sige_amd/csrc/conv_mfma.hpp
@@ -141,6 +141,7 @@
     const float *wscale_ptr;
     int y_f16, res_f16;
     int hp_shift;
+    int phase_up;
 #ifdef SIGE_CONV_PROBE
     unsigned long long *probe;
 #endif
@@ -247,9 +248,13 @@
     return cmax(2 * STAGE + 2 * TABF, W * NB * G::MT * (G::MT + 4));
 }
 
-template <typename G, int NB, int SRC, int MODE, int DST, int LAYOUT, int W, bool Y16 = false>
+template <typename G, int NB, int SRC, int MODE, int DST, int LAYOUT, int W, bool Y16 = false, bool PH = false>
 __device__ __forceinline__ void conv_mfma_body(const ConvArgs &a, const int bx, const int by, float *const smem) {
     static_assert(!Y16 || (SRC == SRC_SCATTER_GATHER && LAYOUT == LAYOUT_NHWC), "fp16-stored cache: the channels-last scatter_gather source");
+    static_assert(!PH || (SRC == SRC_GATHER && MODE == MODE_RAW && DST == DST_NCHW && LAYOUT == LAYOUT_NHWC && W == 4 && !G::F16 &&
+                          G::K == 2 && G::S == 1 && G::R == 3),
+                  "phase form: exact fp32, channels-last raw gather into a full tensor, 2x2 taps on a 3x3 window");
+    const int ph_a = PH ? (by >> 1) : 0, ph_b = PH ? (by & 1) : 0;
     constexpr unsigned YB = Y16 ? 2u : 4u;
     constexpr bool F16 = G::F16;
     using M = std::conditional_t<F16, MfmaH<G::MT>, Mfma<G::MT>>;
@@ -291,12 +296,13 @@
     SIGE_PROBE(6);
     const int Cin = a.Cin;
     const int HW = (SRC == SRC_GATHER) ? (a.H >> a.up) * (a.W >> a.up) : a.H * a.W;
-    const int split = by;
+    const int split = PH ? 0 : by;
     const int first = split * a.chunks_per_split;
     const int last = min(a.nchunks, first + a.chunks_per_split) - 1;
 
     const int ngtot = (a.Cout + G::MT - 1) / G::MT;
     const long packed_floats_total = (long)ngtot * a.nblk * G::F * 64 * 4;
+    const float *const packed = PH ? a.packed + (size_t)by * packed_floats_total : a.packed;
     int gsel[NB];
 #pragma unroll
     for (int nb = 0; nb < NB; ++nb) gsel[nb] = min(ng * NB + nb, ngtot - 1);
@@ -304,7 +310,7 @@
     auto set_b_chunk = [&](int chunk) {
 #pragma unroll
         for (int nb = 0; nb < NB; ++nb)
-            r_b[nb] = make_rsrc(a.packed, ((long)gsel[nb] * a.nblk + chunk * W + wave) * G::F * 64 * 4, packed_floats_total);
+            r_b[nb] = make_rsrc(packed, ((long)gsel[nb] * a.nblk + chunk * W + wave) * G::F * 64 * 4, packed_floats_total);
     };
     float4 bset[2][NB][G::F];
     auto b_load = [&](float4 &dst, int nb, int f) { dst = buf_f32x4(r_b[nb], lane * 16, f * 1024); };
@@ -368,7 +374,8 @@
                 const int pxo = m % G::PX;
                 const int t = mb * G::TPB + m / G::PX, co = (ng * NB + nb) * G::MT + 4 * n4;
                 const int b = min(t, a.T - 1) / a.N;
-                const int h = (a.offH + e_h[k]) / a.strH + pxo / G::RO, w = (a.offW + e_w[k]) / a.strW + pxo % G::RO;
+                const int h = PH ? a.offH + e_h[k] + 2 * (pxo / G::RO) + ph_a : (a.offH + e_h[k]) / a.strH + pxo / G::RO;
+                const int w = PH ? a.offW + e_w[k] + 2 * (pxo % G::RO) + ph_b : (a.offW + e_w[k]) / a.strW + pxo % G::RO;
                 const bool in = o < OUT_UNITS && t < a.T && co < a.Cout && h >= 0 && h < a.Ho && w >= 0 && w < a.Wo;
                 e_h[k] = h; e_w[k] = w; e_in[k] = in;
                 e_q[k] = in ? (((size_t)b * a.Ho + h) * a.Wo + w) * a.Cout + co : 0;
@@ -398,7 +405,11 @@
                 const int tt = min(z_t[i], a.T - 1);
                 const int b = tt / a.N, n = tt - b * a.N;
                 const int2 o = *reinterpret_cast<const int2 *>(a.idx + 2 * n);
-                z_b[i] = b; z_h[i] = o.x + z_p[i] / G::R; z_w[i] = o.y + z_p[i] % G::R;
+                if constexpr (PH) {
+                    z_b[i] = b; z_h[i] = ((o.x + 1) >> 1) - 1 + ph_a + z_p[i] / G::R; z_w[i] = ((o.y + 1) >> 1) - 1 + ph_b + z_p[i] % G::R;
+                } else {
+                    z_b[i] = b; z_h[i] = o.x + z_p[i] / G::R; z_w[i] = o.y + z_p[i] % G::R;
+                }
             });
         }
         if constexpr (EPRE) {
@@ -448,9 +459,10 @@
                     hlo = ((h - z_p[i] / G::R + 2) >> a.hp_shift) << a.hp_shift;
                     hhi = hlo + (1 << a.hp_shift);
                 }
-                const bool in = z_live[i] && h >= hlo && h < hhi && w >= 0 && w < a.W;
+                const bool in = PH ? (z_live[i] && h >= 0 && h < (a.H >> 1) && w >= 0 && w < (a.W >> 1))
+                                   : (z_live[i] && h >= hlo && h < hhi && w >= 0 && w < a.W);
                 z_live[i] = in;
-                const int hw = (SRC == SRC_GATHER) ? (h >> a.up) * (a.W >> a.up) + (w >> a.up) : h * a.W + w;
+                const int hw = PH ? h * (a.W >> 1) + w : (SRC == SRC_GATHER) ? (h >> a.up) * (a.W >> a.up) + (w >> a.up) : h * a.W + w;
                 if (SRC == SRC_GATHER) {
                     off = in ? (unsigned)((b * HW + hw) * a.Csplit + c_l) * 4u : kOOB;
                     off2 = in ? (unsigned)(hw * (Cin - a.Csplit) + c_l) * 4u : kOOB;
@@ -981,6 +993,20 @@
     conv_mfma_body<G, NB, SRC, MODE, DST, LAYOUT, W, Y16>(a, blockIdx.x, blockIdx.y, smem);
 }
 
+template <typename G, int NB>
+__global__ __launch_bounds__(256) void conv_phase_kernel(const ConvArgs a) {
+    kernarg_touch<sizeof(ConvArgs)>();
+    __shared__ __attribute__((aligned(16))) float smem[conv_lds_floats<G, NB, MODE_RAW, LAYOUT_NHWC, 4>()];
+    conv_mfma_body<G, NB, SRC_GATHER, MODE_RAW, DST_NCHW, LAYOUT_NHWC, 4, false, true>(a, blockIdx.x, blockIdx.y, smem);
+}
+
+template <typename G, int NB>
+void launch_conv_phase(ConvArgs a, hipStream_t st);
+#define SIGE_CONV_PHASE_INSTANTIATE(G, NB)                                                                \
+    template <> void launch_conv_phase<G, NB>(ConvArgs a, hipStream_t st) {                               \
+        conv_phase_kernel<G, NB><<<dim3(conv_grid_x(a), 4), 256, 0, st>>>(a);                             \
+    }
+
 template <typename GA, int NBA, typename GB, int DST, int W, int MODEA>
 __global__ __launch_bounds__(64 * W) void conv_pair_kernel(const ConvArgs a, const ConvArgs b, const int na) {
     kernarg_touch<2 * sizeof(ConvArgs)>();
diff --git a/sige_amd/csrc/conv_up_phase_nhwc.hip b/sige_amd/csrc/conv_up_phase_nhwc.hip
--- /dev/null
+++ b/sige_amd/csrc/conv_up_phase_nhwc.hip
@@ -0,0 +1,8 @@
+#include "conv_mfma.hpp"
+namespace sige {
+using G16 = ConvGeo<2, 1, 3, 16>;
+using G32 = ConvGeo<2, 1, 3, 32>;
+SIGE_CONV_PHASE_INSTANTIATE(G16, 1)
+SIGE_CONV_PHASE_INSTANTIATE(G16, 2)
+SIGE_CONV_PHASE_INSTANTIATE(G32, 1)
+}
diff --git a/sige_amd/hip.py b/sige_amd/hip.py
--- a/sige_amd/hip.py
+++ b/sige_amd/hip.py
@@ -47,6 +47,8 @@
     "sige_hip_block_conv_packed_size_f16c": (_c_sz, [_c_int] * 9),
     "sige_hip_block_conv_pack_f16c": (_c_int, [_c_vp] + [_c_int] * 4 + [_c_vp, _c_vp]),
     "sige_hip_block_conv_pack_f32": (_c_int, [_c_vp] + [_c_int] * 4 + [_c_vp, _c_vp]),
+    "sige_hip_upsample_phase_packed_size": (_c_sz, [_c_int] * 2),
+    "sige_hip_upsample_phase_pack_f32": (_c_int, [_c_vp] + [_c_int] * 2 + [_c_vp, _c_vp]),
     "sige_hip_block_conv_f32": (_c_int, [_c_vp] + [_c_int] * 4 + [_c_vp, _c_vp] + [_c_int] * 5 + [_c_vp, _c_vp]),
     "sige_hip_gather_conv_f32": (
         _c_int, [_c_vp] + [_c_int] * 6 + [_c_vp, _c_int] + _BC + _BC + [_c_int, _c_vp, _c_vp] + [_c_int] * 5 + [_c_vp, _c_vp]),
@@ -780,6 +782,37 @@
     return packed
 
 
+def upsample_phase_kernels(weight: torch.Tensor) -> torch.Tensor:
+    w = weight.detach().to(torch.float64)
+    if w.dim() != 4 or tuple(w.shape[2:]) != (3, 3):
+        raise ValueError("upsample_phase_kernels: a [Cout,Cin,3,3] weight")
+
+    def collapse(t, dim, p):
+        t0, t1, t2 = t.select(dim, 0), t.select(dim, 1), t.select(dim, 2)
+        return torch.stack([t0, t1 + t2] if p == 0 else [t0 + t1, t2], dim)
+
+    return torch.stack([collapse(collapse(w, 2, a), 3, b) for a in (0, 1) for b in (0, 1)], 0).to(weight.dtype).contiguous()
+
+
+def upsample_phase_pack(weight: torch.Tensor, kernels: Optional[torch.Tensor] = None, out: Optional[torch.Tensor] = None) -> torch.Tensor:
+    w = _req(weight.detach(), torch.float32, "weight")
+    Cout, Cin, kH, kW = w.shape
+    n = int(lib().sige_hip_upsample_phase_packed_size(Cout, Cin))
+    n9 = conv_packed_size(Cout, Cin, 3, 3, 6, 6, 1, 1, 1)
+    if (kH, kW) != (3, 3) or n == 0 or n9 == 0:
+        raise ValueError("upsample_phase_pack: a [Cout,Cin,3,3] weight")
+    if out is not None and (out.numel() != n + n9 or out.device != w.device):
+        raise ValueError("upsample_phase_pack: `out` is not a pack of this shape")
+    packed = torch.empty((n + n9,), dtype=torch.float32, device=w.device).as_subclass(PackedWeights) if out is None else out
+    packed.compute = "f32"
+    wp = _req(upsample_phase_kernels(w) if kernels is None else kernels, torch.float32, "kernels", 5)
+    if tuple(wp.shape) != (4, Cout, Cin, 2, 2):
+        raise ValueError("upsample_phase_pack: `kernels` must be [4,Cout,Cin,2,2]")
+    _check(lib().sige_hip_upsample_phase_pack_f32(wp.data_ptr(), Cout, Cin, packed.data_ptr(), _stream(w)), "upsample_phase_pack")
+    _check(lib().sige_hip_block_conv_pack_f32(w.data_ptr(), Cout, Cin, 3, 3, packed.data_ptr() + 4 * n, _stream(w)), "upsample_phase_pack")
+    return packed
+
+
 COMPUTE_DTYPES = ("f32", "f16", "f16x3")
 
 
@@ -1431,7 +1464,7 @@
 def gather_conv_cl(x, x2, block: Tuple[int, int], activeIndices, scale, shift, activationName: str,
                    packed, bias, Cout: int, kernel: Tuple[int, int], stride: Tuple[int, int],
                    full: Optional[dict] = None, out_affine: Optional[tuple] = None, upsample2x: bool = False,
-                   out: Optional[torch.Tensor] = None, twins=None):
+                   out: Optional[torch.Tensor] = None, twins=None, phase=None):
     bias_keep = _vec(bias, "bias")
     x = _req_cl(x, "x")
     B, C1, H, W = x.shape
@@ -1500,16 +1533,24 @@
     targs, twin_keep = _twin_args(twins if twins else None, out, Cout, "gather_conv_cl")
     fargs = fargs + (int(bool(upsample2x)), *targs)
     t3r = _tile3_packed(packed) if (TILE3 is None and compute in (0, 1)) else None
-    status = lib().sige_hip_gather_conv_nhwc(
-        compute, x.data_ptr(), None if x2 is None else x2.data_ptr(), B, C1, C2, H, W, block[0], block[1], idx.data_ptr(), N,
-        *sa, *ta, _act(activationName), packed.data_ptr(), _p(bias_keep), Cout, kernel[0], kernel[1],
-        stride[0], stride[1], *fargs, *_tile3_args(packed, t3r), out.data_ptr(), _stream(x))
+    status = UNSUPPORTED
+    if phase is not None and upsample2x and full is not None and compute == 0:
+        fargs2 = fargs[:-(1 + len(targs))] + (2, *targs)
+        status = lib().sige_hip_gather_conv_nhwc(
+            compute, x.data_ptr(), None if x2 is None else x2.data_ptr(), B, C1, C2, H, W, block[0], block[1], idx.data_ptr(), N,
+            *sa, *ta, _act(activationName), phase.data_ptr(), _p(bias_keep), Cout, kernel[0], kernel[1],
+            stride[0], stride[1], *fargs2, *_tile3_args(packed, t3r), out.data_ptr(), _stream(x))
+    if status == UNSUPPORTED:
+        status = lib().sige_hip_gather_conv_nhwc(
+            compute, x.data_ptr(), None if x2 is None else x2.data_ptr(), B, C1, C2, H, W, block[0], block[1], idx.data_ptr(), N,
+            *sa, *ta, _act(activationName), packed.data_ptr(), _p(bias_keep), Cout, kernel[0], kernel[1],
+            stride[0], stride[1], *fargs, *_tile3_args(packed, t3r), out.data_ptr(), _stream(x))
     if status == UNSUPPORTED:
         return None
     _check(status, "gather_conv_cl")
     keep = getattr(_pair_state, "keep", None)
     if keep is not None:
-        keep.append((x, x2, idx, s_keep, t_keep, packed, bias_keep, out, ws, out_affine, full, twin_keep))
+        keep.append((x, x2, idx, s_keep, t_keep, packed, phase, bias_keep, out, ws, out_affine, full, twin_keep))
     if getattr(_side_state, "armed", False):
         _side_state.armed = False
         _side_state.keep.append((x, x2, idx, s_keep, t_keep, packed, bias_keep, out, ws, out_affine, full, twin_keep))
diff --git a/sige_amd/nn/base.py b/sige_amd/nn/base.py
--- a/sige_amd/nn/base.py
+++ b/sige_amd/nn/base.py
@@ -98,6 +98,7 @@
         nn.Conv2d.__init__(self, *args, **kwargs)
         SIGEModule.__init__(self, call_super=False)
         self._packed = {}
+        self._phase = None
         self._tiles_runtime = self.load_runtime("conv2d_tiles", {})
         self.compute_dtype = "f32"
 
@@ -119,6 +120,41 @@
             entry = (key, hip.conv_pack_weights(w, x.shape[2], x.shape[3], self.stride, compute))
             self._packed[compute] = entry
         return entry[1]
+
+    def _phase_key(self):
+        w = self.weight
+        return (w.data_ptr(), w._version, tuple(w.shape), w.device, self.compute_dtype)
+
+    def phase_kernels(self):
+        from .. import hip
+
+        if (tuple(self.kernel_size) != (3, 3) or tuple(self.stride) != (1, 1) or tuple(self.padding) != (1, 1) or self.groups != 1
+                or tuple(self.dilation) != (1, 1) or self.compute_dtype != "f32"):
+            return None
+        key = self._phase_key()
+        if self._phase is None or self._phase[0] != key:
+            self._phase = [key, hip.upsample_phase_kernels(self.weight), None]
+        return self._phase[1]
+
+    def phase_packed(self):
+        from .. import hip
+
+        wp = self.phase_kernels()
+        if wp is None:
+            return None
+        if self._phase[2] is None:
+            self._phase[2] = hip.upsample_phase_pack(self.weight, wp)
+        return self._phase[2]
+
+    def clear_cache(self):
+        self._phase = None
+
+    def rebuild_derived_caches(self):
+        old, self._phase = self._phase, None
+        if old is not None and old[2] is not None and self.phase_kernels() is not None and old[0][2:4] == self._phase[0][2:4]:
+            from .. import hip
+
+            self._phase[2] = hip.upsample_phase_pack(self.weight, self._phase[1], out=old[2])
 
     def _block_conv(self, x: torch.Tensor, out_affine=None) -> torch.Tensor:
         from .. import hip
diff --git a/sige_amd/nn/gather.py b/sige_amd/nn/gather.py
--- a/sige_amd/nn/gather.py
+++ b/sige_amd/nn/gather.py
@@ -11,6 +11,8 @@
 
 
 class Gather(SIGEModule):
+    PHASE_UPSAMPLE = True
+
     def __init__(
         self,
         conv: nn.Conv2d,
@@ -103,7 +105,7 @@
                 return deferred.DeferredTiles(
                     (x.shape[0] * idx.shape[0], channels, bh, bw), x.dtype, x.device, run,
                     dict(kind="gather", x=x, x2=x2, block=(bh, bw), idx=idx, scale=scale, shift=shift, act=act, cl=cl,
-                         up=upsample2x))
+                         up=upsample2x, phase=bool(upsample2x and self.PHASE_UPSAMPLE)))
             return run()
         if self.mode == "full":
             self.note_full_input(x.shape[2:])
diff --git a/sige_amd/nn/scatter.py b/sige_amd/nn/scatter.py
--- a/sige_amd/nn/scatter.py
+++ b/sige_amd/nn/scatter.py
@@ -244,10 +244,14 @@
     if spec["kind"] == "gather":
         if x1 is not None:
             return None
+        phase = None
+        if (spec.get("phase") and spec.get("x2") is None and spec["scale"] is None and spec["shift"] is None and spec["act"] == "identity"
+                and getattr(packed, "compute", "f32") == "f32" and spec["x"].is_cuda and hip.get_edit_batch() == 1):
+            phase = conv.phase_packed()
         return hip.gather_conv_cl(spec["x"], spec.get("x2"), spec["block"], spec["idx"], spec["scale"], spec["shift"], spec["act"],
                                   packed, conv.bias, conv.out_channels, conv.kernel_size, conv.stride,
                                   full=dict(offset=g.offset, out_res=tuple(out.shape[2:]), residual=residual),
-                                  upsample2x=spec.get("up", False), out=out, twins=twins)
+                                  upsample2x=spec.get("up", False), out=out, twins=twins, phase=phase)
     if tuple(conv.kernel_size) != (3, 3) or tuple(conv.stride) != (1, 1):
         return None
     return hip.scatter_gather_conv_scatter_cl(spec["x"], spec["y"], spec["block"], spec["idx"], spec["map"], spec["scale"],
```

New measurement: 864.5 forward/s, median of 6. +1.9%, better.
